# ShenhanQian/GaussianAvatars

Measured on AMD Instinct MI355X. Metric: frames/sec fwd+bwd @100k SH-3 splats 802x550, higher is better.
Workload: dtype f32; 1 GPU; BASELINE configs[2]: 100000 mesh-bound SH-3 splats (synthetic stand-in for media/306), 802x550 (HxW), select_mesh_by_timestep + render + L1-vs-white + backward, no optimiser step; splats=100000, width=550, height=802, sh_degree=3, scene=ellipsoid, splat_order=morton (io.spatial_sort: the loaders' default), num_rendered=2322054, num_binned=1851307, tile_culling=True, binding=fused, parallelism=one process, one GPU, 300 frames in turn; no collective

## Files before the change

### gaussianavatars_amd/_lib.py

```python
from __future__ import annotations

import ctypes as C
import os

_HERE = os.path.dirname(os.path.abspath(__file__))


def raw_stream(dev):
    import torch

    try:
        return torch._C._cuda_getCurrentRawStream(dev.index if dev.index is not None else torch.cuda.current_device())
    except AttributeError:
        return torch.cuda.current_stream(dev).cuda_stream


class _NoCtx:
    def __enter__(self):
        return None

    def __exit__(self, *a):
        return False


# ... 21 lines not shown


class GsrSettings(C.Structure):
    _fields_ = [
        ("image_height", C.c_int32),
        ("image_width", C.c_int32),
        ("tanfovx", C.c_float),
        ("tanfovy", C.c_float),
        ("bg", C.c_void_p),
        ("scale_modifier", C.c_float),
        ("viewmatrix", C.c_void_p),
        ("projmatrix", C.c_void_p),
        ("sh_degree", C.c_int32),
        ("campos", C.c_void_p),
        ("prefiltered", C.c_int32),
        ("debug", C.c_int32),
        ("tile_culling", C.c_int32),
        ("forward_only", C.c_int32),
        ("deterministic", C.c_int32),
        ("exact_scale_grad", C.c_int32),
        ("deferred_count", C.c_int32),
        ("fast_blend", C.c_int32),
    ]


class GsrGeomLayout(C.Structure):
    _fields_ = [(n, C.c_size_t) for n in
                ("depths", "grec", "cov3D", "rect", "tiles_touched", "clamped", "visible", "brec", "acc64", "acc", "total")]


class GsrBinningLayout(C.Structure):
    _fields_ = [(n, C.c_size_t) for n in
                ("keys", "point_list", "qlist", "qpos", "qcount", "qstart", "ranges", "tile_count", "tile_start", "tile_cursor", "tile_order",
                 "block_hist", "dkeys", "dtmp", "order", "bcount", "bstart", "bcursor", "border", "bhist", "qhist", "qprefix", "qmask", "ranks", "rank", "rank_over", "srect", "sspan", "pstat", "tdesc", "obs", "bandcnt", "path", "chunks", "nb", "nbands", "band_rows",
                 "total")]


class GsrBound(C.Structure):
    _fields_ = [("binding", C.c_void_p), ("binding_is_i64", C.c_int32), ("F", C.c_int32), ("face_R", C.c_void_p), ("face_scale", C.c_void_p),
                ("face_center", C.c_void_p), ("face_quat", C.c_void_p), ("slot", C.c_void_p), ("rows", C.c_void_p)]


class GsrImageLayout(C.Structure):
    _fields_ = [(n, C.c_size_t) for n in ("final_T", "n_contrib", "n_contrib_q", "c_final", "ck", "gmax", "units", "total")]


GSR_SYMBOLS = {
    "gsr_abi_version": (C.c_int, []),
    "gsr_last_error": (C.c_char_p, []),
    "gsr_count_slot_read": (C.c_int, [C.c_int32, C.POINTER(C.c_int64), C.POINTER(C.c_int64)]),
    "gsr_count_slot_overflow": (C.c_int, [C.c_int32, C.POINTER(C.c_int64), C.c_int32]),
    "gsr_last_forward_seq": (C.c_int64, []),
    "gsr_count_slot_wait": (C.c_int, [C.c_int32, C.c_int64, C.c_void_p, C.POINTER(C.c_int64)]),
    "gsr_geom_layout": (C.c_int, [C.c_int32, C.POINTER(GsrGeomLayout)]),
    "gsr_binning_layout": (C.c_int, [C.c_int64, C.c_int32, C.c_int32, C.c_int32, C.c_int32, C.POINTER(GsrBinningLayout)]),
    "gsr_image_layout": (C.c_int, [C.c_int32, C.c_int32, C.POINTER(GsrImageLayout)]),
    "gsr_forward": (C.c_int, [C.POINTER(GsrSettings), C.c_int32, C.c_int32] + [C.c_void_p] * 7 +
                    [C.c_void_p, C.c_void_p, C.c_void_p, C.c_void_p, C.c_int64, C.c_void_p,
                     C.POINTER(C.c_int64), C.c_void_p]),
    "gsr_backward": (C.c_int, [C.POINTER(GsrSettings), C.c_int32, C.c_int32] + [C.c_void_p] * 6 +
                     [C.c_void_p, C.c_void_p, C.c_void_p, C.c_int64, C.c_void_p, C.c_int64, C.c_void_p] +
                     [C.c_void_p] * 8 + [C.c_void_p]),
    "gsr_forward_ex": (C.c_int, [C.POINTER(GsrSettings), C.c_int32, C.c_int32] + [C.c_void_p] * 8 +
                       [C.c_void_p, C.c_void_p, C.c_void_p, C.c_void_p, C.c_int64, C.c_void_p,
                        C.POINTER(C.c_int64), C.c_void_p]),
    "gsr_backward_ex": (C.c_int, [C.POINTER(GsrSettings), C.c_int32, C.c_int32] + [C.c_void_p] * 7 +
                        [C.c_void_p, C.c_void_p, C.c_void_p, C.c_int64, C.c_void_p, C.c_int64, C.c_void_p] +
                        [C.c_void_p] * 9 + [C.c_void_p]),
    "gsr_forward_bound": (C.c_int, [C.POINTER(GsrSettings), C.c_int32, C.c_int32, C.POINTER(GsrBound)] + [C.c_void_p] * 6 +
                          [C.c_void_p, C.c_void_p, C.c_void_p, C.c_void_p, C.c_int64, C.c_void_p, C.POINTER(C.c_int64), C.c_void_p]),
    "gsr_backward_bound": (C.c_int, [C.POINTER(GsrSettings), C.c_int32, C.c_int32, C.POINTER(GsrBound)] + [C.c_void_p] * 6 +
                           [C.c_void_p, C.c_void_p, C.c_void_p, C.c_int64, C.c_void_p, C.c_int64, C.c_void_p] +
                           [C.c_void_p] * 8 + [C.c_void_p]),
    "gsr_mark_visible": (C.c_int, [C.c_int32, C.c_void_p, C.c_void_p, C.c_void_p, C.c_void_p, C.c_void_p]),
    "gsr_profile_enable": (C.c_int, [C.c_int]),
    "gsr_profile_read": (C.c_int, [C.POINTER(C.c_double), C.POINTER(C.c_int64)]),
    "gsr_kernel_name": (C.c_char_p, [C.c_int]),
    "gsr_wait_stats": (C.c_int, [C.POINTER(C.c_double), C.POINTER(C.c_int64)]),
}
GSR_NUM_KERNELS = 12


def gsr_profile_enable(on: bool) -> None:
    gsr().gsr_profile_enable(1 if on else 0)


def gsr_profile_read() -> dict:
    ms = (C.c_double * GSR_NUM_KERNELS)()
    n = (C.c_int64 * GSR_NUM_KERNELS)()
    rc = gsr().gsr_profile_read(ms, n)
    if rc != GSR_OK:
        raise RuntimeError(f"gsr_profile_read failed: {gsr().gsr_last_error().decode()}")
    return {gsr().gsr_kernel_name(i).decode(): (ms[i], n[i]) for i in range(GSR_NUM_KERNELS)}

def gsr_wait_stats():
    ms, n = C.c_double(), C.c_int64()
    gsr().gsr_wait_stats(C.byref(ms), C.byref(n))
    return ms.value, n.value


_gsr = None


def _torch_first():
    import torch


def gsr():
    global _gsr
    if _gsr is None:
        if not os.path.exists(GSR_LIB_PATH):
            raise RuntimeError(
                f"{GSR_LIB_PATH} is missing: build it with `python -c 'import __graft_entry__ as g; g.build()'` "
                "(hipcc --offload-arch=gfx950).  There is no CPU fallback."
            )
        _torch_first()
        lib = C.CDLL(GSR_LIB_PATH)
        for name, (res, args) in GSR_SYMBOLS.items():
            fn = getattr(lib, name)
            fn.restype = res
            fn.argtypes = args
        if lib.gsr_abi_version() != GSR_ABI_VERSION:
            raise RuntimeError(f"gsr ABI version {lib.gsr_abi_version()} != {GSR_ABI_VERSION}")
        _gsr = lib
    return _gsr


GAB_LIB_PATH = os.environ.get("GAB_LIB") or os.path.join(_HERE, "libgab_hip.so")
GAB_FLAME_WS_FLOATS = 512
GAB_BIND_ROW_FLOATS = 20
_P = C.c_void_p


class GabRig(C.Structure):
    _fields_ = [("V", C.c_int32), ("n_shape", C.c_int32), ("n_expr", C.c_int32), ("v_template", _P), ("shapedirs", _P),
                ("posedirs", _P), ("J_regressor", _P), ("lbs_weights", _P), ("parents", C.c_int32 * 5)]


GAB_SYMBOLS = {
    "gab_abi_version": (C.c_int, []),
    "gab_last_error": (C.c_char_p, []),
    "gab_flame_forward": (C.c_int, [C.POINTER(GabRig)] + [_P] * 8 + [_P, _P, _P, _P]),
    "gab_flame_backward": (C.c_int, [C.POINTER(GabRig)] + [_P] * 8 + [_P, _P, _P, _P] + [_P] * 8 + [_P] +
                           [C.c_int32, C.POINTER(C.c_void_p), C.POINTER(C.c_int32), _P]),
    "gab_flame_prepared_floats": (C.c_int64, [C.POINTER(GabRig)]),
    "gab_flame_prepare": (C.c_int, [C.POINTER(GabRig), _P, _P, _P, _P]),
    "gab_flame_forward_prepared": (C.c_int, [C.POINTER(GabRig), _P] + [_P] * 6 + [_P, _P, _P, _P]),
    "gab_blend_sequence": (C.c_int, [C.POINTER(GabRig), _P, _P, C.c_int32, _P, _P]),
    "gab_flame_forward_sequence": (C.c_int, [C.POINTER(GabRig), _P, _P] + [_P] * 6 + [_P, _P, _P, _P]),
    "gab_flame_backward_prepared": (C.c_int, [C.POINTER(GabRig), _P] + [_P] * 4 + [_P, _P, _P] + [_P] * 6 + [_P] +
                                    [C.c_int32, C.POINTER(C.c_void_p), C.POINTER(C.c_int32), _P]),
    "gab_mesh_backward_prepared": (C.c_int, [C.POINTER(GabRig), _P] + [_P] * 4 + [_P, _P, _P, _P, _P] + [_P] * 5 + [_P] * 6 + [_P] +
                                   [C.c_int32, C.POINTER(C.c_void_p), C.POINTER(C.c_int32), _P]),
    "gab_face_frames_forward": (C.c_int, [C.c_int32, C.c_int32, _P, _P, C.c_int32, _P, _P, _P, _P, _P, _P]),
    "gab_face_frames_backward": (C.c_int, [C.c_int32, C.c_int32, _P, _P, C.c_int32, _P, _P, _P, _P, _P, C.c_int32, _P]),
    "gab_bind_forward": (C.c_int, [C.c_int32, C.c_int32, _P, _P, _P, _P, C.c_int32, _P, _P, _P, _P, _P, _P, _P, _P, _P, _P]),
    "gab_bind_backward": (C.c_int, [C.c_int32, C.c_int32, _P, _P, _P, _P, C.c_int32, _P, _P, _P, _P, _P, _P, _P, _P, _P, _P, _P, _P, _P, _P, _P]),
    "gab_bind_backward_csr": (C.c_int, [C.c_int32, C.c_int32] + [_P] * 22),
    "gab_bind_backward_faces": (C.c_int, [C.c_int32, _P, _P, _P, _P]),
    "gab_zero_buffers": (C.c_int, [C.c_int32, C.POINTER(C.c_void_p), C.POINTER(C.c_int32), _P]),
    "gab_feed_row": (C.c_int, [_P, C.c_int32, C.c_int32, _P, C.c_int32, _P, _P, _P]),
    "gab_profile_enable": (C.c_int, [C.c_int]),
    "gab_profile_collect": (C.c_int, []),
    "gab_profile_entry": (C.c_int, [C.c_int32, C.POINTER(C.c_char_p), C.POINTER(C.c_double), C.POINTER(C.c_int64)]),
    "gab_profile_reset": (C.c_int, []),
}
GAB_ABI_VERSION = 5

_gab = None


def gab():
    global _gab
    if _gab is None:
        if not os.path.exists(GAB_LIB_PATH):
            raise RuntimeError(f"{GAB_LIB_PATH} is missing: run __graft_entry__.build() (hipcc, gfx950).  There is no CPU fallback.")
        _torch_first()
        lib = C.CDLL(GAB_LIB_PATH)
        for name, (res, args) in GAB_SYMBOLS.items():
            fn = getattr(lib, name)
            fn.restype = res
            fn.argtypes = args
        if lib.gab_abi_version() != GAB_ABI_VERSION:
            raise RuntimeError(f"gab ABI version {lib.gab_abi_version()} != {GAB_ABI_VERSION}")
        _gab = lib
    return _gab


GLS_LIB_PATH = os.path.join(_HERE, "libgls_hip.so")
GLS_SYMBOLS = {
    "gls_abi_version": (C.c_int, []),
    "gls_last_error": (C.c_char_p, []),
    "gls_partial_floats": (C.c_int64, [C.c_int32] * 4),
    "gls_l1_ssim_forward": (C.c_int, [C.c_int32] * 4 + [_P, _P, C.c_float] + [_P] * 4),
    "gls_l1_ssim_backward": (C.c_int, [C.c_int32] * 4 + [_P] * 4 + [C.c_float, _P, _P]),
    "gls_l1_ssim_backward_split": (C.c_int, [C.c_int32] * 4 + [_P] * 5 + [C.c_int32, C.c_float, _P, _P]),
    "gls_l1_forward": (C.c_int, [C.c_int64, _P, _P, C.c_float, _P, _P, _P]),
    "gls_l1_forward_grad": (C.c_int, [C.c_int64, _P, _P, C.c_float, _P, _P, _P, _P]),
    "gls_l1_backward": (C.c_int, [C.c_int64, _P, _P, _P, C.c_float, _P, _P]),
    "gls_densification_stats": (C.c_int, [C.c_int32] + [_P] * 6),
    "gls_add_densification_stats": (C.c_int, [C.c_int32, _P, _P, C.c_int32, _P, _P, _P]),
    "gls_profile_enable": (C.c_int, [C.c_int]),
    "gls_profile_collect": (C.c_int, []),
    "gls_profile_entry": (C.c_int, [C.c_int32, C.POINTER(C.c_char_p), C.POINTER(C.c_double), C.POINTER(C.c_int64)]),
    "gls_profile_reset": (C.c_int, []),
}
GLS_ABI_VERSION = 4

_gls = None


def gls():
    global _gls
    if _gls is None:
        if not os.path.exists(GLS_LIB_PATH):
            raise RuntimeError(f"{GLS_LIB_PATH} is missing: run __graft_entry__.build() (hipcc, gfx950).  There is no CPU fallback.")
        _torch_first()
        lib = C.CDLL(GLS_LIB_PATH)
        for name, (res, args) in GLS_SYMBOLS.items():
            fn = getattr(lib, name)
            fn.restype = res
            fn.argtypes = args
        if lib.gls_abi_version() != GLS_ABI_VERSION:
            raise RuntimeError(f"gls ABI version {lib.gls_abi_version()} != {GLS_ABI_VERSION}")
        _gls = lib
    return _gls


def launch_profile_enable(on: bool) -> None:
    for lib, tag in ((gab(), "gab"), (gls(), "gls")):
        getattr(lib, tag + "_profile_enable")(1 if on else 0)
        if on:
            getattr(lib, tag + "_profile_reset")()


def launch_profile_read() -> dict:
    out = {}
    for lib, tag in ((gab(), "gab"), (gls(), "gls")):
        n = getattr(lib, tag + "_profile_collect")()
        for i in range(n):
            name, ms, k = C.c_char_p(), C.c_double(), C.c_int64()
            if getattr(lib, tag + "_profile_entry")(i, C.byref(name), C.byref(ms), C.byref(k)) == 0:
                out[name.value.decode()] = (ms.value, k.value)
    return out


def gls_error() -> str:
    return gls().gls_last_error().decode("utf-8", "replace")


def gab_error() -> str:
    return gab().gab_last_error().decode("utf-8", "replace")


def gsr_error() -> str:
    return gsr().gsr_last_error().decode("utf-8", "replace")


GMR_LIB_PATH = os.path.join(_HERE, "libgmr_hip.so")
GMR_SYMBOLS = {
    "gmr_abi_version": (C.c_int, []),
    "gmr_last_error": (C.c_char_p, []),
    "gmr_workspace_bytes": (C.c_int64, [C.c_int32, C.c_int32]),
    "gmr_rasterize": (C.c_int, [C.c_int32] * 5 + [_P, _P, _P, _P, _P]),
    "gmr_antialias": (C.c_int, [C.c_int32] * 6 + [_P] * 7),
}
GMR_ABI_VERSION = 1
GMR_MAX_TRIANGLES = (1 << 24) - 1

_gmr = None


def gmr():
    global _gmr
    if _gmr is None:
        if not os.path.exists(GMR_LIB_PATH):
            raise RuntimeError(f"{GMR_LIB_PATH} is missing: run __graft_entry__.build() (hipcc, gfx950).  There is no CPU fallback.")
        _torch_first()
        lib = C.CDLL(GMR_LIB_PATH)
        for name, (res, args) in GMR_SYMBOLS.items():
            fn = getattr(lib, name)
            fn.restype = res
            fn.argtypes = args
        if lib.gmr_abi_version() != GMR_ABI_VERSION:
            raise RuntimeError(f"gmr ABI version {lib.gmr_abi_version()} != {GMR_ABI_VERSION}")
        _gmr = lib
    return _gmr


def gmr_error() -> str:
    return gmr().gmr_last_error().decode("utf-8", "replace")


GOP_LIB_PATH = os.path.join(_HERE, "libgop_hip.so")
GOP_ABI_VERSION = 1
GOP_MAX_TENSORS = 32
GOP_SLAB = 2048


class GopAdamTensor(C.Structure):
    _fields_ = [("param", _P), ("grad", _P), ("exp_avg", _P), ("exp_avg_sq", _P), ("n", C.c_int64), ("step_size", C.c_float),
                ("bias_correction2_sqrt", C.c_float)]


GOP_SYMBOLS = {
    "gop_abi_version": (C.c_int, []),
    "gop_last_error": (C.c_char_p, []),
    "gop_adam_step": (C.c_int, [C.c_int32, C.POINTER(GopAdamTensor), C.c_float, C.c_float, C.c_float, _P]),
    "gop_adam_step_ex": (C.c_int, [C.c_int32, C.POINTER(GopAdamTensor)] + [C.c_float] * 5 + [_P]),
    "gop_profile_enable": (C.c_int, [C.c_int]),
    "gop_profile_collect": (C.c_int, []),
    "gop_profile_entry": (C.c_int, [C.c_int32, C.POINTER(C.c_char_p), C.POINTER(C.c_double), C.POINTER(C.c_int64)]),
    "gop_profile_reset": (C.c_int, []),
}

_gop = None


def gop():
    global _gop
# ... 33 lines not shown
```

### gaussianavatars_amd/binding.py

```python
from __future__ import annotations

import ctypes as C
import os

import torch

from . import _host, _lib


def _p(t):
    return None if t is None else t.data_ptr()


def _stream(dev):
    return _lib.raw_stream(dev)


def _chk(rc, what):
    if rc != 0:
        raise RuntimeError(f"{what} failed ({rc}): {_lib.gab_error()}")


def _need_cuda(t, name):
    if not t.is_cuda:
# ... 51 lines not shown
        head._gab_rig = (key, s)
        r = head._gab_rig
    return r[1]


def _prepared_rig(head, rig, shape_flat, so_flat):
    key = (id(rig), shape_flat.data_ptr(), shape_flat._version, None if so_flat is None else (so_flat.data_ptr(), so_flat._version))
    c = getattr(head, "_gab_prepared", None)
    if c is None or c[0] != key:
        lib = _lib.gab()
        dev = head.v_template.device
        buf = torch.empty(int(lib.gab_flame_prepared_floats(C.byref(rig))), dtype=torch.float32, device=dev)
        with _lib.on_device(dev):
            _chk(lib.gab_flame_prepare(C.byref(rig), _p(shape_flat), _p(so_flat), _p(buf), _stream(dev)), "gab_flame_prepare")
        head._gab_prepared = c = (key, buf, shape_flat, so_flat)
    return c[1]


def _sequence_mode() -> str:
    return os.environ.get("GAA_MESH_SEQUENCE", "off")


def _sequence_table(head, rig, prepared, expr_tab):
    mode = _sequence_mode()
    if mode == "off" or getattr(head, "flame_sequence", True) is False or rig.n_expr <= 0:
        return None
    T = int(expr_tab.shape[0])
    if T < 2 or T * 3 * rig.V * 4 > (1 << 30):
        return None
    key = (prepared.data_ptr(), id(prepared), expr_tab.data_ptr(), expr_tab._version, T)
    c = getattr(head, "_gab_sequence", None)
    if c is not None and c[0] == key:
        if c[1] is not None:
            return c[1]
    elif mode != "eager":
        head._gab_sequence = (key, None, None, None)
        return None
    lib = _lib.gab()
    dev = expr_tab.device
    seq = torch.empty((T, 3 * rig.V), dtype=torch.float32, device=dev)
    with _lib.on_device(dev):
        _chk(lib.gab_blend_sequence(C.byref(rig), _p(prepared), _p(expr_tab), T, _p(seq), _stream(dev)), "gab_blend_sequence")
    head._gab_sequence = (key, seq, prepared, expr_tab)
    return seq


def _use_prepared(head, shape_needs_grad, so_needs_grad) -> bool:
    return not shape_needs_grad and not so_needs_grad and getattr(head, "flame_impl", "prepared") != "classic"


class _FlameForward(torch.autograd.Function):
    @staticmethod
    def forward(ctx, head, shape, expr, rotation, neck, jaw, eyes, translation, static_offset):
        ctx.set_materialize_grads(False)
        lib = _lib.gab()
        rig = _rig_struct(head)
        dev = head.v_template.device
        V = rig.V
        ins = [_f32(t).reshape(-1) for t in (shape, expr, rotation, neck, jaw, eyes, translation)]
        if ins[0].numel() != rig.n_shape or ins[1].numel() != rig.n_expr or ins[5].numel() != 6:
            raise RuntimeError("fused FLAME forward is batch-1: shape (1,n_shape), expr (1,n_expr), eyes (1,6)")
        so = None if static_offset is None else _f32(static_offset).reshape(-1)
        if so is not None and so.numel() != 3 * V:
            raise RuntimeError("static_offset must be (1,V,3)")
        verts = torch.empty((1, V, 3), dtype=torch.float32, device=dev)
        v_shaped = torch.empty((1, V, 3), dtype=torch.float32, device=dev)
        ws = torch.empty(_lib.GAB_FLAME_WS_FLOATS, dtype=torch.float32, device=dev)
        need = ctx.needs_input_grad
        ctx.prepared = _prepared_rig(head, rig, ins[0], so) if _use_prepared(head, need[1], static_offset is not None and need[8]) else None
        with _lib.on_device(dev):
            if ctx.prepared is not None:
                _chk(lib.gab_flame_forward_prepared(C.byref(rig), _p(ctx.prepared), *[_p(t) for t in ins[1:]], _p(verts), _p(v_shaped),
                                                    _p(ws), _stream(dev)), "gab_flame_forward_prepared")
            else:
                _chk(lib.gab_flame_forward(C.byref(rig), *[_p(t) for t in ins], _p(so), _p(verts), _p(v_shaped), _p(ws), _stream(dev)),
                     "gab_flame_forward")
        ctx.head = head
        ctx.has_so = static_offset is not None
        ctx.shapes = [t.shape for t in (shape, expr, rotation, neck, jaw, eyes, translation)]
        ctx.so_shape = None if static_offset is None else static_offset.shape
        ctx.save_for_backward(*ins, *( [so] if so is not None else []), v_shaped, ws)
        return verts, v_shaped

    @staticmethod
    def backward(ctx, g_verts, g_vshaped):
        lib = _lib.gab()
        head = ctx.head
        rig = _rig_struct(head)
        saved = ctx.saved_tensors
        ins = list(saved[:7])
        so = saved[7] if ctx.has_so else None
        v_shaped, ws = saved[-2], saved[-1]
        dev = v_shaped.device
        V = rig.V
        need = ctx.needs_input_grad
        f32 = dict(dtype=torch.float32, device=dev)
        d_shape = torch.empty(rig.n_shape, **f32) if need[1] else None
        d_expr = torch.empty(rig.n_expr, **f32)
        d_rot, d_neck, d_jaw = torch.empty(3, **f32), torch.empty(3, **f32), torch.empty(3, **f32)
        d_eyes, d_trans = torch.empty(6, **f32), torch.empty(3, **f32)
        d_so = torch.empty(3 * V, **f32) if (ctx.has_so and need[8]) else None
        scratch = torch.empty(3 * V, **f32)
        gv = torch.zeros((V, 3), **f32) if g_verts is None else _f32(g_verts)
        gvs = None if g_vshaped is None else _f32(g_vshaped)
        with _lib.on_device(dev):
            if ctx.prepared is not None and gvs is None and d_shape is None and d_so is None:
                _chk(lib.gab_flame_backward_prepared(C.byref(rig), _p(ctx.prepared), *[_p(t) for t in ins[2:6]], _p(v_shaped), _p(ws), _p(gv),
                                                     _p(d_expr), _p(d_rot), _p(d_neck), _p(d_jaw), _p(d_eyes), _p(d_trans), _p(scratch),
                                                     0, None, None, _stream(dev)), "gab_flame_backward_prepared")
            else:
                _chk(lib.gab_flame_backward(C.byref(rig), *[_p(t) for t in ins], _p(so), _p(v_shaped), _p(ws), _p(gv), _p(gvs),
                                            _p(d_shape), _p(d_expr), _p(d_rot), _p(d_neck), _p(d_jaw), _p(d_eyes), _p(d_trans), _p(d_so),
                                            _p(scratch), 0, None, None, _stream(dev)), "gab_flame_backward")
        sh = ctx.shapes
        outs = [None, None if d_shape is None else d_shape.view(sh[0]), d_expr.view(sh[1]), d_rot.view(sh[2]), d_neck.view(sh[3]),
                d_jaw.view(sh[4]), d_eyes.view(sh[5]), d_trans.view(sh[6]), None if d_so is None else d_so.view(ctx.so_shape)]
        return tuple(outs)


def flame_forward(head, shape, expr, rotation, neck, jaw, eyes, translation, static_offset=None):
    return _FlameForward.apply(head, shape, expr, rotation, neck, jaw, eyes, translation, static_offset)


class _FlameForwardTimestep(torch.autograd.Function):

    _ROWS = ("expr", "rotation", "neck_pose", "jaw_pose", "eyes_pose", "translation")

    @staticmethod
    def forward(ctx, head, t, shape, expr, rotation, neck, jaw, eyes, translation, static_offset):
        ctx.set_materialize_grads(False)
        lib = _lib.gab()
        rig = _rig_struct(head)
        dev = head.v_template.device
        V = rig.V
        tabs = [_f32(x) for x in (expr, rotation, neck, jaw, eyes, translation)]
        T = tabs[0].shape[0]
        widths = [int(x.shape[1]) for x in tabs]
        if widths != [rig.n_expr, 3, 3, 3, 6, 3] or any(x.shape[0] != T for x in tabs) or not (0 <= t < T):
            raise RuntimeError("flame_forward_timestep: expected (T,n_expr),(T,3),(T,3),(T,3),(T,6),(T,3) tables and 0 <= t < T")
        sh = _f32(shape).reshape(-1)
        so = None if static_offset is None else _f32(static_offset).reshape(-1)
        rows = [x.data_ptr() + 4 * t * w for x, w in zip(tabs, widths)]
        verts = torch.empty((1, V, 3), dtype=torch.float32, device=dev)
        v_shaped = torch.empty((1, V, 3), dtype=torch.float32, device=dev)
        ws = torch.empty(_lib.GAB_FLAME_WS_FLOATS, dtype=torch.float32, device=dev)
        need = ctx.needs_input_grad
        ctx.prepared = _prepared_rig(head, rig, sh, so) if _use_prepared(head, need[2], so is not None and need[9]) else None
        seq = _sequence_table(head, rig, ctx.prepared, tabs[0]) if (ctx.prepared is not None and not any(need[2:])) else None
        with _lib.on_device(dev):
            if seq is not None:
                _chk(lib.gab_flame_forward_sequence(C.byref(rig), _p(ctx.prepared), seq.data_ptr() + 4 * t * 3 * V, *rows, _p(verts), _p(v_shaped),
                                                    _p(ws), _stream(dev)), "gab_flame_forward_sequence")
            elif ctx.prepared is not None:
                _chk(lib.gab_flame_forward_prepared(C.byref(rig), _p(ctx.prepared), *rows, _p(verts), _p(v_shaped), _p(ws), _stream(dev)),
                     "gab_flame_forward_prepared")
            else:
                _chk(lib.gab_flame_forward(C.byref(rig), _p(sh), *rows, _p(so), _p(verts), _p(v_shaped), _p(ws), _stream(dev)),
                     "gab_flame_forward")
        ctx.head, ctx.t, ctx.T, ctx.widths = head, t, T, widths
        ctx.has_so = so is not None
        ctx.shape_shape = shape.shape
        ctx.so_shape = None if static_offset is None else static_offset.shape
        ctx.keep = _Keep(sh, *tabs, *([so] if so is not None else []), v_shaped, ws)
        return verts, v_shaped

    @staticmethod
    def backward(ctx, g_verts, g_vshaped):
        lib = _lib.gab()
        rig = _rig_struct(ctx.head)
        saved = ctx.keep.get()
        sh, tabs = saved[0], list(saved[1:7])
        so = saved[7] if ctx.has_so else None
        v_shaped, ws = saved[-2], saved[-1]
        dev = v_shaped.device
        V, T, t, widths = rig.V, ctx.T, ctx.t, ctx.widths
        need = ctx.needs_input_grad
        f32 = dict(dtype=torch.float32, device=dev)
        tables = [torch.empty((T, w), **f32) for w in widths]
        ptrs = (C.c_void_p * len(tables))(*[x.data_ptr() for x in tables])
        sizes = (C.c_int32 * len(tables))(*[T * w for w in widths])
        outp = [x.data_ptr() + 4 * t * w for x, w in zip(tables, widths)]
        d_shape = torch.empty(rig.n_shape, **f32) if need[2] else None
        d_so = torch.empty(3 * V, **f32) if (ctx.has_so and need[9]) else None
        scratch = torch.empty(3 * V, **f32)
        gv = torch.zeros((V, 3), **f32) if g_verts is None else _f32(g_verts)
        gvs = None if g_vshaped is None else _f32(g_vshaped)
        rows = [x.data_ptr() + 4 * t * w for x, w in zip(tabs, widths)]
        with _lib.on_device(dev):
            if ctx.prepared is not None and gvs is None and d_shape is None and d_so is None:
                _chk(lib.gab_flame_backward_prepared(C.byref(rig), _p(ctx.prepared), *rows[1:5], _p(v_shaped), _p(ws), _p(gv), *outp,
                                                     _p(scratch), len(tables), ptrs, sizes, _stream(dev)), "gab_flame_backward_prepared")
            else:
                _chk(lib.gab_flame_backward(C.byref(rig), _p(sh), *rows, _p(so), _p(v_shaped), _p(ws), _p(gv), _p(gvs), _p(d_shape),
                                            *outp, _p(d_so), _p(scratch), len(tables), ptrs, sizes, _stream(dev)), "gab_flame_backward")
        grads = [tb if need[3 + i] else None for i, tb in enumerate(tables)]
        return (None, None, None if d_shape is None else d_shape.view(ctx.shape_shape), *grads,
                None if d_so is None else d_so.view(ctx.so_shape))


def flame_forward_timestep(head, flame_param: dict, t: int):
    fp = flame_param
    return _FlameForwardTimestep.apply(head, int(t), fp["shape"], fp["expr"], fp["rotation"], fp["neck_pose"], fp["jaw_pose"],
                                       fp["eyes_pose"], fp["translation"], fp.get("static_offset"))


class _FaceFrames(torch.autograd.Function):
    @staticmethod
    def forward(ctx, verts, faces):
        ctx.set_materialize_grads(False)
        lib = _lib.gab()
        _need_cuda(verts, "verts")
        dev = verts.device
        v = _f32(verts)
        fi, is64 = _idx(faces)
        V, F = v.shape[0], fi.shape[0]
        f32 = dict(dtype=torch.float32, device=dev)
        center, R = torch.empty((F, 3), **f32), torch.empty((F, 3, 3), **f32)
        scale, quat = torch.empty((F, 1), **f32), torch.empty((F, 4), **f32)
        ctx.d_verts = torch.empty((V, 3), **f32) if ctx.needs_input_grad[0] else None
        with _lib.on_device(dev):
            _chk(lib.gab_face_frames_forward(V, F, _p(v), _p(fi), is64, _p(center), _p(R), _p(scale), _p(quat), _p(ctx.d_verts),
                                             _stream(dev)), "gab_face_frames_forward")
        ctx.keep = _Keep(v, fi)
        ctx.is64 = is64
        return center, R, scale, quat

    @staticmethod
    def backward(ctx, g_center, g_R, g_scale, g_quat):
        lib = _lib.gab()
        v, fi = ctx.keep.get()
        dev = v.device
        V, F = v.shape[0], fi.shape[0]
        d_verts, ctx.d_verts = ctx.d_verts, None
        prepared = d_verts is not None
        if not prepared:
            d_verts = torch.empty((V, 3), dtype=torch.float32, device=dev)
        gs = [None if g is None else _f32(g) for g in (g_center, g_R, g_scale, g_quat)]
        with _lib.on_device(dev):
            _chk(lib.gab_face_frames_backward(V, F, _p(v), _p(fi), ctx.is64, _p(gs[0]), _p(gs[1]), _p(gs[2]), _p(gs[3]), _p(d_verts),
                                              1 if prepared else 0, _stream(dev)), "gab_face_frames_backward")
        return d_verts, None


def face_frames(verts, faces):
    return _FaceFrames.apply(verts, faces)


class _SubCtx:

    def __init__(self, needs_input_grad):
        self.needs_input_grad = needs_input_grad

    def set_materialize_grads(self, flag):
        pass


def vertex_corner_csr(faces: torch.Tensor, num_verts: int):
    hit = getattr(faces, "_gaa_vertex_corners", None)
    if hit is not None and hit[0] == faces._version and hit[1] == num_verts:
        return hit[2]
    f = faces.detach().long()
    flat = f.reshape(-1)
    order = torch.sort(flat, stable=True).indices
    fo, co = order // 3, order % 3
    vf_list = torch.cat([(4 * fo + co)[:, None], f[fo]], 1).to(torch.int32).contiguous()
    vf_begin = torch.zeros(num_verts + 1, dtype=torch.int32, device=flat.device)
    vf_begin[1:] = torch.cumsum(torch.bincount(flat, minlength=num_verts), 0).to(torch.int32)
    faces._gaa_vertex_corners = (faces._version, num_verts, (vf_begin, vf_list))
    return vf_begin, vf_list


def _mesh_backward_mode() -> str:
    return os.environ.get("GAA_MESH_BWD", "merged")


class _MeshFramesTimestep(torch.autograd.Function):
    @staticmethod
    def forward(ctx, head, t, faces, shape, expr, rotation, neck, jaw, eyes, translation, static_offset):
        ctx.set_materialize_grads(False)
        need = ctx.needs_input_grad
        c1 = _SubCtx((False, False) + tuple(need[3:]))
        verts, v_shaped = _FlameForwardTimestep.forward(c1, head, t, shape, expr, rotation, neck, jaw, eyes, translation, static_offset)
        ctx.merged = c1.prepared is not None and _mesh_backward_mode() == "merged"
        if ctx.merged and faces.device != verts.device:
            raise RuntimeError(f"select_mesh_by_timestep: faces live on {faces.device}, the vertices on {verts.device}")
        if ctx.merged and any(need):
            ctx.corners = vertex_corner_csr(faces, int(verts.shape[1]))
        c2 = _SubCtx((any(need) and not ctx.merged, False))
        center, R, scale, quat = _FaceFrames.forward(c2, verts[0], faces)
        ctx.c1, ctx.c2 = c1, c2
        ctx.faces = faces
        return verts, v_shaped, center, R, scale, quat

    @staticmethod
    def _backward_merged(ctx, g_verts, g_center, g_R, g_scale, g_quat):
        c1, c2 = ctx.c1, ctx.c2
        lib = _lib.gab()
        rig = _rig_struct(c1.head)
        saved = c1.keep.get()
        tabs = list(saved[1:7])
        v_shaped, ws = saved[-2], saved[-1]
        v, _ = c2.keep.get()
        dev = v.device
        V, T, t, widths = rig.V, c1.T, c1.t, c1.widths
        need = c1.needs_input_grad
        f32 = dict(dtype=torch.float32, device=dev)
        tables = [torch.empty((T, w), **f32) for w in widths]
        ptrs = (C.c_void_p * len(tables))(*[x.data_ptr() for x in tables])
        sizes = (C.c_int32 * len(tables))(*[T * w for w in widths])
        outp = [x.data_ptr() + 4 * t * w for x, w in zip(tables, widths)]
        rows = [x.data_ptr() + 4 * t * w for x, w in zip(tabs, widths)]
        vf_begin, vf_list = ctx.corners
        scratch = torch.empty(3 * V, **f32)
        gs = [None if g is None else _f32(g) for g in (g_center, g_R, g_scale, g_quat)]
        gv = None if g_verts is None else _f32(g_verts)
        with _lib.on_device(dev):
            _chk(lib.gab_mesh_backward_prepared(C.byref(rig), _p(c1.prepared), *rows[1:5], _p(v_shaped), _p(ws), _p(v),
                                                _p(vf_begin), _p(vf_list), _p(gs[0]), _p(gs[1]), _p(gs[2]), _p(gs[3]), _p(gv), *outp,
                                                _p(scratch), len(tables), ptrs, sizes, _stream(dev)), "gab_mesh_backward_prepared")
        grads = [tb if need[3 + i] else None for i, tb in enumerate(tables)]
        return (None, None, None, None, *grads, None)

    @staticmethod
    def backward(ctx, g_verts, g_vshaped, g_center, g_R, g_scale, g_quat):
        if ctx.merged and g_vshaped is None:
            return _MeshFramesTimestep._backward_merged(ctx, g_verts, g_center, g_R, g_scale, g_quat)
        d_verts, _ = _FaceFrames.backward(ctx.c2, g_center, g_R, g_scale, g_quat)
        if g_verts is not None:
            d_verts = d_verts + g_verts.reshape(d_verts.shape)
        grads = _FlameForwardTimestep.backward(ctx.c1, d_verts.view(1, -1, 3), g_vshaped)
        return (None, None, None) + tuple(grads[2:])


_RIG_BUFFERS = ("v_template", "shapedirs", "posedirs", "J_regressor", "lbs_weights")


def _plain(t) -> bool:
    return t.is_cuda and t.dtype is torch.float32 and t.is_contiguous()


def _mesh_plan(H, head, fp: dict, faces):
    shape, so = fp["shape"], fp.get("static_offset")
    bufs = head.__dict__.get("_buffers")
    if bufs is None or any(n not in bufs for n in _RIG_BUFFERS):
        bufs = {n: getattr(head, n) for n in _RIG_BUFFERS}
    env = (os.environ.get("GAA_MESH_BWD"), os.environ.get("GAA_MESH_SEQUENCE"))
    st = head.__dict__.get("_gaa_mesh_plan")
    if st is not None:
        (plan, k_shape, v_shape, k_so, v_so, k_faces, v_faces, k_bufs, k_env, k_flags) = st
        if (k_shape is shape and v_shape == shape._version and k_so is so and (so is None or v_so == so._version) and k_faces is faces and v_faces == faces._version
                and k_env == env and k_flags == (shape.requires_grad, so is not None and so.requires_grad, getattr(head, "flame_impl", "prepared"))
                and all(bufs[n] is b for n, b in zip(_RIG_BUFFERS, k_bufs))):
            return plan
    plan = None
    flags = (shape.requires_grad, so is not None and so.requires_grad, getattr(head, "flame_impl", "prepared"))
    ok = (not flags[0] and not flags[1] and flags[2] != "classic" and _mesh_backward_mode() == "merged" and _sequence_mode() == "off"
          and all(_plain(bufs[n]) for n in _RIG_BUFFERS) and faces.is_cuda and faces.is_contiguous() and faces.dtype in (torch.int32, torch.int64)
          and faces.device == bufs["v_template"].device)
    if ok:
        rig = _rig_struct(head)
        sh = _f32(shape).reshape(-1)
        sof = None if so is None else _f32(so).reshape(-1)
        if sh.numel() == rig.n_shape and (sof is None or sof.numel() == 3 * rig.V):
            prepared = _prepared_rig(head, rig, sh, sof)
            vf_begin, vf_list = vertex_corner_csr(faces, int(rig.V))
            plan = H.make_mesh_plan(*[bufs[n] for n in _RIG_BUFFERS], [int(x) for x in head.parents.tolist()], int(head.n_shape_params), prepared, faces, vf_begin, vf_list)
    head.__dict__["_gaa_mesh_plan"] = (plan, shape, shape._version, so, None if so is None else so._version, faces, faces._version, tuple(bufs[n] for n in _RIG_BUFFERS), env, flags)
    return plan


def mesh_frames_timestep(head, flame_param: dict, t: int, faces):
    fp = flame_param
    H = _host.get()
    if H is not None:
        expr, rot, neck, jaw, eyes, trans = fp["expr"], fp["rotation"], fp["neck_pose"], fp["jaw_pose"], fp["eyes_pose"], fp["translation"]
        if _plain(expr) and _plain(rot) and _plain(neck) and _plain(jaw) and _plain(eyes) and _plain(trans):
            plan = _mesh_plan(H, head, fp, faces)
            if plan is not None:
                return H.mesh_frames(plan, expr, rot, neck, jaw, eyes, trans, int(t))
    return _MeshFramesTimestep.apply(head, int(t), faces, fp["shape"], fp["expr"], fp["rotation"], fp["neck_pose"], fp["jaw_pose"],
                                     fp["eyes_pose"], fp["translation"], fp.get("static_offset"))


def binding_csr(binding: torch.Tensor, num_faces: int):
    b = binding.detach().long()
    order64 = torch.sort(b, stable=True).indices
    order = order64.to(torch.int32).contiguous()
    counts = torch.bincount(b, minlength=num_faces)
    face_begin = torch.zeros(num_faces + 1, dtype=torch.int32, device=b.device)
    face_begin[1:] = torch.cumsum(counts, 0).to(torch.int32)
    slot = torch.empty_like(order)
    slot[order64] = torch.arange(order.numel(), dtype=torch.int32, device=b.device)
    return order, face_begin, b.to(torch.int32).contiguous(), slot


class _BindSplats(torch.autograd.Function):
    @staticmethod
    def forward(ctx, xyz, log_scaling, rotation, binding, face_R, face_scale, face_center, face_quat, csr=None, opacity_logit=None):
        lib = _lib.gab()
        _need_cuda(xyz, "_xyz")
        dev = xyz.device
        x, ls, q = _f32(xyz), _f32(log_scaling), _f32(rotation)
        b, is64 = _idx(binding)
        fR, fs, fc, fq = _f32(face_R), _f32(face_scale), _f32(face_center), _f32(face_quat)
        N, F = x.shape[0], fc.shape[0]
        f32 = dict(dtype=torch.float32, device=dev)
        ox, osc, oq = torch.empty((N, 3), **f32), torch.empty((N, 3), **f32), torch.empty((N, 4), **f32)
        ol = None if opacity_logit is None else _f32(opacity_logit)
        oo = None if ol is None else torch.empty_like(ol)
        with _lib.on_device(dev):
            _chk(lib.gab_bind_forward(N, F, _p(x), _p(ls), _p(q), _p(b), is64, _p(fc), _p(fR), _p(fs), _p(fq), _p(ox), _p(osc), _p(oq),
                                      _p(ol), _p(oo), _stream(dev)), "gab_bind_forward")
        ctx.keep = _Keep(x, ls, q, b, fR, fs, fc, fq, oo)
        ctx.is64 = is64
        if csr is not None and (csr[0].numel() != N or csr[1].numel() != F + 1 or any(t.numel() != N for t in csr[2:4])):
            raise RuntimeError(f"binding CSR does not match this call: {csr[0].numel()} ordered splats / {csr[1].numel() - 1} faces, "
                               f"expected {N} / {F} (rebuild it with binding_csr after the binding changed)")
        ctx.csr = csr
        if oo is None:
            return ox, osc, oq
        return ox, osc, oq, oo

    @staticmethod
    def backward(ctx, g_xyz, g_scaling, g_rot, g_opacity=None):
        lib = _lib.gab()
        x, ls, q, b, fR, fs, fc, fq, oo = ctx.keep.get()
        dev = x.device
        N, F = x.shape[0], fc.shape[0]
        f32 = dict(dtype=torch.float32, device=dev)
        d_x, d_ls, d_q = torch.empty((N, 3), **f32), torch.empty((N, 3), **f32), torch.empty((N, 4), **f32)
        d_face = torch.empty(17 * F, **f32)
        gs = [None if g is None else _f32(g) for g in (g_xyz, g_scaling, g_rot)]
        go = None if (oo is None or g_opacity is None) else _f32(g_opacity)
        d_ol = None if oo is None else torch.empty_like(oo)
        with _lib.on_device(dev):
            if ctx.csr is not None:
                order, face_begin = ctx.csr[0], ctx.csr[1]
                splat_face, slot = (ctx.csr[2], ctx.csr[3]) if len(ctx.csr) >= 4 else (None, None)
                rows = torch.empty(_lib.GAB_BIND_ROW_FLOATS * N, **f32) if slot is not None else None
                _chk(lib.gab_bind_backward_csr(N, F, _p(x), _p(ls), _p(q), _p(fR), _p(fs), _p(fq), _p(gs[0]), _p(gs[1]), _p(gs[2]),
                                               _p(order), _p(face_begin), _p(d_x), _p(d_ls), _p(d_q), _p(d_face), _p(oo), _p(go), _p(d_ol),
                                               _p(splat_face), _p(slot), _p(rows), _stream(dev)), "gab_bind_backward_csr")
            else:
                _chk(lib.gab_bind_backward(N, F, _p(x), _p(ls), _p(q), _p(b), ctx.is64, _p(fc), _p(fR), _p(fs), _p(fq), _p(gs[0]),
                                           _p(gs[1]), _p(gs[2]), _p(d_x), _p(d_ls), _p(d_q), _p(d_face), _p(oo), _p(go), _p(d_ol),
                                           _stream(dev)), "gab_bind_backward")
        return (d_x, d_ls, d_q, None, d_face[3 * F: 12 * F].view(F, 3, 3), d_face[12 * F: 13 * F].view(F, 1), d_face[: 3 * F].view(F, 3),
                d_face[13 * F:].view(F, 4), None, d_ol)


def bind_splats(xyz, log_scaling, rotation, binding, face_R, face_scale, face_center, face_quat, csr=None, opacity_logit=None):
    return _BindSplats.apply(xyz, log_scaling, rotation, binding, face_R, face_scale, face_center, face_quat, csr, opacity_logit)
```

### gaussianavatars_amd/csrc/build_host.py

```python
#!/usr/bin/env python3
import os
import subprocess
import sys
import sysconfig

HERE = os.path.dirname(os.path.abspath(__file__))
OUT = os.path.join(os.path.dirname(HERE), "gaa_host.so")
SRC = os.path.join(HERE, "gaa_host.cpp")
STAMP = OUT + ".stamp"
DEPS = [SRC, __file__] + [os.path.join(HERE, "..", "..", "include", h) for h in ("gsr.h", "gab.h", "gls.h")]


def build_stamp() -> str:
    import torch

    return "torch=%s cxx11abi=%d python=%s soabi=%s" % (torch.__version__, int(torch._C._GLIBCXX_USE_CXX11_ABI), sys.version.split()[0],
                                                       sysconfig.get_config_var("SOABI"))


def stamp_matches() -> bool:
    try:
        return open(STAMP).read().strip() == build_stamp()
    except OSError:
        return False


def up_to_date() -> bool:
    return os.path.exists(OUT) and all(os.path.getmtime(OUT) >= os.path.getmtime(d) for d in DEPS) and stamp_matches()


def main() -> int:
    if up_to_date() and "--force" not in sys.argv:
        return 0
    import torch
    from torch.utils import cpp_extension as ce

    tl = ce.library_paths()[0]
    rocm = os.environ.get("ROCM_PATH", "/opt/rocm")
    cmd = ["g++", "-O2", "-std=c++17", "-fPIC", "-shared", "-Wall", "-Wno-unused-function", "-Wno-sign-compare",
           "-D__HIP_PLATFORM_AMD__=1", "-DUSE_ROCM=1", "-DTORCH_EXTENSION_NAME=gaa_host", "-DTORCH_API_INCLUDE_EXTENSION_H",
           f"-D_GLIBCXX_USE_CXX11_ABI={int(torch._C._GLIBCXX_USE_CXX11_ABI)}"]
    cmd += [f"-I{p}" for p in ce.include_paths()] + [f"-I{rocm}/include", f"-I{sysconfig.get_paths()['include']}"]
    cmd += [SRC, "-o", OUT, f"-L{tl}", "-lc10", "-lc10_hip", "-ltorch_cpu", "-ltorch_hip", "-ltorch", "-ltorch_python", "-ldl", f"-Wl,-rpath,{tl}"]
    print("building gaa_host.so (g++, torch %s) ..." % torch.__version__, flush=True)
    r = subprocess.run(cmd)
    if r.returncode == 0:
        with open(STAMP, "w") as fh:
            fh.write(build_stamp() + "\n")
    return r.returncode


if __name__ == "__main__":
    sys.exit(main())
```

### gaussianavatars_amd/csrc/gaa_host.cpp

```cpp
#include <torch/extension.h>

#include <ATen/hip/impl/HIPGuardImplMasqueradingAsCUDA.h>
#include <c10/hip/HIPStream.h>
#include <dlfcn.h>
#include <torch/csrc/autograd/function.h>
#include <torch/csrc/autograd/functions/utils.h>

#include <atomic>
#include <map>
#include <mutex>
#include <tuple>

#include "../../include/gab.h"
#include "../../include/gls.h"
#include "../../include/gsr.h"

namespace {

using at::Tensor;
using torch::autograd::Node;
using torch::autograd::variable_list;

#define GAA_API(X)                                                                                                                      \
    X(gsr_abi_version) X(gsr_last_error) X(gsr_geom_layout) X(gsr_binning_layout) X(gsr_image_layout) X(gsr_forward_bound)             \
    X(gsr_backward_bound) X(gsr_last_forward_seq) X(gsr_count_slot_wait) X(gsr_count_slot_overflow)                                     \
    X(gab_abi_version) X(gab_last_error) X(gab_flame_forward_prepared) X(gab_face_frames_forward) X(gab_mesh_backward_prepared)         \
    X(gab_bind_backward_faces)                                                                                                           \
    X(gls_abi_version) X(gls_last_error) X(gls_partial_floats) X(gls_l1_forward) X(gls_l1_forward_grad) X(gls_l1_backward)               \
    X(gls_l1_ssim_forward) X(gls_l1_ssim_backward_split)

struct Api {
#define GAA_DECL(name) decltype(&::name) name = nullptr;
    GAA_API(GAA_DECL)
#undef GAA_DECL
    bool ready = false;
} api;

void* open_loaded(const std::string& path)
{
    void* h = dlopen(path.c_str(), RTLD_NOW | RTLD_NOLOAD);
    if (!h) h = dlopen(path.c_str(), RTLD_NOW);
    TORCH_CHECK(h, "gaa_host: cannot open ", path, ": ", dlerror());
    return h;
}

void init(const std::string& gsr_path, const std::string& gab_path, const std::string& gls_path)
{
    void* hs[3] = {open_loaded(gsr_path), open_loaded(gab_path), open_loaded(gls_path)};
#define GAA_LOAD(name)                                                                                       \
    {                                                                                                        \
        void* s = nullptr;                                                                                   \
        for (void* h : hs)                                                                                   \
            if (!s) s = dlsym(h, #name);                                                                     \
        TORCH_CHECK(s, "gaa_host: the libraries do not export ", #name);                                     \
        api.name = reinterpret_cast<decltype(api.name)>(s);                                                  \
    }
    GAA_API(GAA_LOAD)
#undef GAA_LOAD
    TORCH_CHECK(api.gsr_abi_version() == GSR_ABI_VERSION, "gaa_host was built for gsr ABI ", GSR_ABI_VERSION, ", the library is ", api.gsr_abi_version());
    TORCH_CHECK(api.gab_abi_version() == GAB_ABI_VERSION, "gaa_host was built for gab ABI ", GAB_ABI_VERSION, ", the library is ", api.gab_abi_version());
    TORCH_CHECK(api.gls_abi_version() == GLS_ABI_VERSION, "gaa_host was built for gls ABI ", GLS_ABI_VERSION, ", the library is ", api.gls_abi_version());
    api.ready = true;
}

inline void need_api() { TORCH_CHECK(api.ready, "gaa_host.init() has not been called"); }

inline void* cur_stream(const Tensor& t) { return (void*)c10::hip::getCurrentHIPStream(t.device().index()).stream(); }
using DeviceGuard = c10::hip::HIPGuardMasqueradingAsCUDA;

inline const float* fptr(const Tensor& t) { return t.defined() && t.numel() ? t.data_ptr<float>() : nullptr; }
inline float* fptr_mut(Tensor& t) { return t.defined() && t.numel() ? t.data_ptr<float>() : nullptr; }

inline void check_f32(const Tensor& t, const char* name)
{
    TORCH_CHECK(t.defined() && t.is_cuda(), name, " must be a device tensor; the MI355X path has no CPU implementation");
    TORCH_CHECK(t.scalar_type() == at::kFloat && t.is_contiguous(), name, " must be contiguous float32 (the native host does not copy: take the Python entry)");
}

inline Tensor empty_f32(at::IntArrayRef sizes, const Tensor& like) { return at::empty(sizes, like.options().dtype(at::kFloat)); }

inline Tensor grad_f32(const Tensor& g)
{
    if (!g.defined()) return g;
    if (g.scalar_type() == at::kFloat && g.is_contiguous()) return g;
    return g.to(at::kFloat).contiguous();
}

struct Kept {
    Tensor t;
    uint32_t version = 0;
    Kept() = default;
    explicit Kept(const Tensor& x, bool alias = false) : t(x.defined() ? (alias ? x.detach() : x) : x), version(x.defined() ? x._version() : 0) {}
    const Tensor& get(const char* what) const
    {
        TORCH_CHECK(!t.defined() || t._version() == version, "one of the variables needed for gradient computation has been modified by an inplace operation (",
                    what, " saved by the native host is at version ", t.defined() ? t._version() : 0, ", expected ", version, ")");
        return t;
    }
};

inline bool any_requires_grad(std::initializer_list<std::reference_wrapper<const Tensor>> ts)
{
    if (!at::GradMode::is_enabled()) return false;
    for (const Tensor& t : ts)
        if (t.defined() && t.requires_grad()) return true;
    return false;
}

struct MeshPlan {
    GabRig rig{};
    Tensor keep[5];
    Tensor prepared;
    Tensor faces;
    int faces_i64 = 0;
    Tensor vf_begin, vf_list;
    int64_t F = 0;
};

struct MeshNode : public Node {
    std::shared_ptr<MeshPlan> plan;
    Kept tabs[6];
    Kept verts, v_shaped;
    Tensor ws;
    int64_t t = 0, T = 0;
    int64_t widths[6] = {0, 3, 3, 3, 6, 3};

    variable_list apply(variable_list&& grads) override
    {
        std::lock_guard<std::mutex> lock(mutex_);
        need_api();
        TORCH_CHECK(grads.size() == 6, "MeshNode: expected 6 gradients");
        TORCH_CHECK(!grads[1].defined(), "the native mesh node has no path for a gradient w.r.t. verts_cano (v_shaped): take GAA_NATIVE_HOST=0");
        const MeshPlan& p = *plan;
        static const char* names[6] = {"expr", "rotation", "neck_pose", "jaw_pose", "eyes_pose", "translation"};
        const Tensor& v = verts.get("verts");
        const Tensor& vs = v_shaped.get("verts_cano");
        DeviceGuard guard(v.device().index());
        void* stream = cur_stream(v);
        const int V = p.rig.V;
        Tensor tables[6];
        float* zero_ptrs[6];
        int32_t zero_sizes[6];
        float* outp[6];
        const float* rows[6];
        for (int i = 0; i < 6; ++i) {
            const Tensor& tab = tabs[i].get(names[i]);
            tables[i] = empty_f32({T, widths[i]}, v);
            zero_ptrs[i] = tables[i].data_ptr<float>();
            zero_sizes[i] = (int32_t)(T * widths[i]);
            outp[i] = zero_ptrs[i] + t * widths[i];
            rows[i] = tab.data_ptr<float>() + t * widths[i];
        }
        Tensor scratch = empty_f32({3 * (int64_t)V}, v);
        Tensor gc = grad_f32(grads[2]), gR = grad_f32(grads[3]), gs = grad_f32(grads[4]), gq = grad_f32(grads[5]), gv = grad_f32(grads[0]);
        int rc = api.gab_mesh_backward_prepared(&p.rig, p.prepared.data_ptr<float>(), rows[1], rows[2], rows[3], rows[4], vs.data_ptr<float>(), ws.data_ptr<float>(),
                                                v.data_ptr<float>(), p.vf_begin.data_ptr<int32_t>(), p.vf_list.data_ptr<int32_t>(), fptr(gc), fptr(gR), fptr(gs), fptr(gq),
                                                fptr(gv), outp[0], outp[1], outp[2], outp[3], outp[4], outp[5], scratch.data_ptr<float>(), 6, zero_ptrs, zero_sizes, stream);
        TORCH_CHECK(rc == 0, "gab_mesh_backward_prepared failed (", rc, "): ", api.gab_last_error());
        variable_list out(6);
        for (int i = 0; i < 6; ++i)
            if (task_should_compute_output(i)) out[i] = tables[i];
        return out;
    }
    void release_variables() override {}
};

std::vector<Tensor> mesh_frames(const std::shared_ptr<MeshPlan>& plan, const Tensor& expr, const Tensor& rotation, const Tensor& neck, const Tensor& jaw,
                                const Tensor& eyes, const Tensor& translation, int64_t t)
{
    need_api();
    const MeshPlan& p = *plan;
    const Tensor* tabs[6] = {&expr, &rotation, &neck, &jaw, &eyes, &translation};
    const int64_t widths[6] = {p.rig.n_expr, 3, 3, 3, 6, 3};
    static const char* names[6] = {"expr", "rotation", "neck_pose", "jaw_pose", "eyes_pose", "translation"};
    const int64_t T = expr.dim() == 2 ? expr.size(0) : -1;
    TORCH_CHECK(T > 0 && t >= 0 && t < T, "flame_forward_timestep: expected (T,n_expr),(T,3),(T,3),(T,3),(T,6),(T,3) tables and 0 <= t < T");
    for (int i = 0; i < 6; ++i) {
        check_f32(*tabs[i], names[i]);
        TORCH_CHECK(tabs[i]->dim() == 2 && tabs[i]->size(0) == T && tabs[i]->size(1) == widths[i],
                    "flame_forward_timestep: expected (T,n_expr),(T,3),(T,3),(T,3),(T,6),(T,3) tables and 0 <= t < T");
    }
    const Tensor& like = p.prepared;
    DeviceGuard guard(like.device().index());
    void* stream = cur_stream(like);
    const int64_t V = p.rig.V, F = p.F;
    Tensor verts = empty_f32({1, V, 3}, like), v_shaped = empty_f32({1, V, 3}, like), ws = empty_f32({GAB_FLAME_WS_FLOATS}, like);
    Tensor center = empty_f32({F, 3}, like), R = empty_f32({F, 3, 3}, like), scale = empty_f32({F, 1}, like), quat = empty_f32({F, 4}, like);
    const float* rows[6];
    for (int i = 0; i < 6; ++i) rows[i] = tabs[i]->data_ptr<float>() + t * widths[i];
    int rc = api.gab_flame_forward_prepared(&p.rig, p.prepared.data_ptr<float>(), rows[0], rows[1], rows[2], rows[3], rows[4], rows[5], verts.data_ptr<float>(),
                                            v_shaped.data_ptr<float>(), ws.data_ptr<float>(), stream);
    TORCH_CHECK(rc == 0, "gab_flame_forward_prepared failed (", rc, "): ", api.gab_last_error());
    rc = api.gab_face_frames_forward((int32_t)V, (int32_t)F, verts.data_ptr<float>(), p.faces.data_ptr(), p.faces_i64, center.data_ptr<float>(), R.data_ptr<float>(),
                                     scale.data_ptr<float>(), quat.data_ptr<float>(), nullptr , stream);
    TORCH_CHECK(rc == 0, "gab_face_frames_forward failed (", rc, "): ", api.gab_last_error());
    if (any_requires_grad({expr, rotation, neck, jaw, eyes, translation})) {
        auto node = std::shared_ptr<MeshNode>(new MeshNode(), torch::autograd::deleteNode);
        node->set_next_edges(torch::autograd::collect_next_edges(expr, rotation, neck, jaw, eyes, translation));
        node->plan = plan;
        for (int i = 0; i < 6; ++i) {
            node->tabs[i] = Kept(*tabs[i]);
            node->widths[i] = widths[i];
        }
        node->verts = Kept(verts, true);
        node->v_shaped = Kept(v_shaped, true);
        node->ws = ws;
        node->t = t;
        node->T = T;
        torch::autograd::set_history({verts, v_shaped, center, R, scale, quat}, node);
    }
    return {verts, v_shaped, center, R, scale, quat};
}

struct Layouts {
    GsrGeomLayout geom;
    GsrImageLayout img;
};
std::mutex layout_mutex;
std::map<std::tuple<int64_t, int, int>, Layouts> layout_cache;
std::map<std::tuple<int64_t, int, int, int64_t, int>, GsrBinningLayout> binning_cache;

Layouts layouts(int64_t P, int W, int H)
{
    std::lock_guard<std::mutex> lock(layout_mutex);
    auto key = std::make_tuple(P, W, H);
    auto it = layout_cache.find(key);
    if (it == layout_cache.end()) {
        if (layout_cache.size() > 64) layout_cache.clear();
        Layouts l{};
        TORCH_CHECK(api.gsr_geom_layout((int32_t)P, &l.geom) == 0 && api.gsr_image_layout(W, H, &l.img) == 0, "gsr layout: ", api.gsr_last_error());
        it = layout_cache.emplace(key, l).first;
    }
    return it->second;
}
GsrBinningLayout binning_layout(int64_t cap, int W, int H, int64_t P, int mode)
{
    std::lock_guard<std::mutex> lock(layout_mutex);
    auto key = std::make_tuple(cap, W, H, P, mode);
    auto it = binning_cache.find(key);
    if (it == binning_cache.end()) {
        if (binning_cache.size() > 64) binning_cache.clear();
        GsrBinningLayout b{};
        TORCH_CHECK(api.gsr_binning_layout(cap, W, H, (int32_t)P, mode, &b) == 0, "gsr_binning_layout: ", api.gsr_last_error());
        it = binning_cache.emplace(key, b).first;
    }
    return it->second;
}

struct RasterNode : public Node {
    GsrSettings s{};
    Tensor bg, viewmatrix, projmatrix, campos;
    Kept xyz, dc, rest, opacity, scaling, rotation;
    Kept fR, fs, fc, fq;
    Tensor binding, csr_slot, face_begin;
    int binding_i64 = 0;
    Tensor radii, state;
    size_t off_img = 0, off_binning = 0;
    int64_t P = 0, M = 0, F = 0, capacity = 0, num_rendered = 0;
    bool bound = false;

    variable_list apply(variable_list&& grads) override
    {
        std::lock_guard<std::mutex> lock(mutex_);
        need_api();
        variable_list out(11);
        if (grads.empty() || !grads[0].defined()) return out;
        TORCH_CHECK(state.defined(), "the rasterizer state of this frame has been released (backward through the graph a second time without retain_graph)");
        const Tensor& x = xyz.get("_xyz");
        DeviceGuard guard(x.device().index());
        void* stream = cur_stream(x);
        Tensor g = grad_f32(grads[0]);
        TORCH_CHECK(g.is_cuda() && g.numel() == 3 * (int64_t)s.image_height * s.image_width, "grad_out_color must be a (3,H,W) device tensor");
        Tensor g_xyz = empty_f32({P, 3}, x), g_m2 = empty_f32({P, 3}, x), g_dc = empty_f32({P, 1, 3}, x), g_rest = empty_f32({P, M - 1, 3}, x);
        Tensor g_op = empty_f32({P, 1}, x), g_ls = empty_f32({P, 3}, x), g_rot = empty_f32({P, 4}, x);
        GsrBound b{};
        Tensor scratch, d_face;
        if (!bound) {
            scratch = empty_f32({9 * P}, x);
        } else {
            const int64_t rows_at = (9 * P + 3) / 4 * 4;
            scratch = empty_f32({rows_at + (int64_t)GAB_BIND_ROW_FLOATS * P}, x);
            d_face = empty_f32({17 * F}, x);
            b.binding = binding.data_ptr();
            b.binding_is_i64 = binding_i64;
            b.F = (int32_t)F;
            b.face_R = fR.get("face_orien_mat").data_ptr<float>();
            b.face_scale = fs.get("face_scaling").data_ptr<float>();
            b.face_center = fc.get("face_center").data_ptr<float>();
            b.face_quat = fq.get("face_orien_quat").data_ptr<float>();
            b.slot = csr_slot.data_ptr<int32_t>();
            b.rows = scratch.data_ptr<float>() + rows_at;
        }
        GsrSettings sb = s;
        sb.forward_only = 0;
        sb.deferred_count = 0;
        uint8_t* st = state.data_ptr<uint8_t>();
        int rc = api.gsr_backward_bound(&sb, (int32_t)P, (int32_t)M, &b, x.data_ptr<float>(), dc.get("_features_dc").data_ptr<float>(), rest.get("_features_rest").data_ptr<float>(),
                                        opacity.get("_opacity").data_ptr<float>(), scaling.get("_scaling").data_ptr<float>(), rotation.get("_rotation").data_ptr<float>(),
                                        radii.data_ptr<int32_t>(), st, st + off_binning, capacity, st + off_img, num_rendered, g.data_ptr<float>(), g_xyz.data_ptr<float>(),
                                        g_m2.data_ptr<float>(), g_dc.data_ptr<float>(), g_rest.data_ptr<float>(), g_op.data_ptr<float>(), g_ls.data_ptr<float>(),
                                        g_rot.data_ptr<float>(), scratch.data_ptr<float>(), stream);
        TORCH_CHECK(rc == 0, "gsr_backward_bound failed (", rc, "): ", api.gsr_last_error());
        if (bound) {
            rc = api.gab_bind_backward_faces((int32_t)F, face_begin.data_ptr<int32_t>(), b.rows, d_face.data_ptr<float>(), stream);
            TORCH_CHECK(rc == 0, "gab_bind_backward_faces failed (", rc, "): ", api.gab_last_error());
        }
        out[0] = g_xyz, out[1] = g_m2, out[2] = g_dc, out[3] = g_rest, out[4] = g_op, out[5] = g_ls, out[6] = g_rot;
        if (bound) {
            if (task_should_compute_output(7)) out[7] = d_face.as_strided({F, 3, 3}, {9, 3, 1}, 3 * F);
            if (task_should_compute_output(8)) out[8] = d_face.as_strided({F, 1}, {1, 1}, 12 * F);
            if (task_should_compute_output(9)) out[9] = d_face.as_strided({F, 3}, {3, 1}, 0);
            if (task_should_compute_output(10)) out[10] = d_face.as_strided({F, 4}, {4, 1}, 13 * F);
        }
        for (int i = 0; i < 7; ++i)
            if (!task_should_compute_output(i)) out[i] = Tensor();
        return out;
    }
    void release_variables() override
    {
        std::lock_guard<std::mutex> lock(mutex_);
        state = Tensor();
    }
};

struct RasterResult {
    Tensor color, radii, visible, state;
    int64_t num_rendered = 0, capacity = 0, off_binning = 0;
    int forward_only = 0, path = 0, nbands = 0, fitted = 1;
};

RasterResult rasterize_bound(const Tensor& xyz, const Tensor& means2D, const Tensor& dc, const Tensor& rest, const Tensor& opacity, const Tensor& scaling,
                             const Tensor& rotation, const c10::optional<Tensor>& face_R, const c10::optional<Tensor>& face_scale,
                             const c10::optional<Tensor>& face_center, const c10::optional<Tensor>& face_quat, const c10::optional<Tensor>& binding,
                             const c10::optional<Tensor>& csr_slot, const c10::optional<Tensor>& face_begin, const Tensor& bg, const Tensor& viewmatrix,
                             const Tensor& projmatrix, const Tensor& campos, int64_t H, int64_t W, double tanfovx, double tanfovy, double scale_modifier,
                             int64_t sh_degree, int64_t debug, int64_t tile_culling, int64_t exact_scale_grad, int64_t deterministic, int64_t fast_blend,
                             int64_t capacity, int64_t late_slot)
{
    need_api();
    check_f32(xyz, "_xyz"), check_f32(dc, "_features_dc"), check_f32(rest, "_features_rest"), check_f32(opacity, "_opacity");
    check_f32(scaling, "_scaling"), check_f32(rotation, "_rotation");
    check_f32(bg, "bg"), check_f32(viewmatrix, "viewmatrix"), check_f32(projmatrix, "projmatrix"), check_f32(campos, "campos");
    const int64_t P = xyz.size(0);
    TORCH_CHECK(P > 0 && xyz.dim() == 2 && xyz.size(1) == 3, "_xyz must be (P,3) with P > 0");
    TORCH_CHECK(rest.dim() == 3 && rest.size(0) == P && rest.size(1) >= 1 && dc.numel() == 3 * P, "split SH: _features_dc must be (P,1,3) and _features_rest (P,M-1,3)");
    const int64_t M = 1 + rest.size(1);
    const bool bound = binding.has_value() && binding->defined();
    GsrBound b{};
// ... 114 lines not shown
        need_api();
        variable_list out(2);
        if (grads.empty() || !grads[0].defined()) return out;
        Tensor pre = da;
        da = Tensor();
        if (pre.defined()) {
            if (is_unit_seed(grads[0])) {
                g_l1_misses = 0;
                out[0] = pre;
                return out;
            }
            if (++g_l1_misses >= 2) g_l1_emit = 0;
        }
        const Tensor& x = a.get("network_output");
        const Tensor& y = b.get("gt");
        DeviceGuard guard(x.device().index());
        void* stream = cur_stream(x);
        Tensor g = grad_f32(grads[0]);
        const int64_t n = x.numel();
        if (task_should_compute_output(0)) {
            out[0] = at::empty_like(x);
            int rc = api.gls_l1_backward(n, x.data_ptr<float>(), y.data_ptr<float>(), g.data_ptr<float>(), (float)scale, out[0].data_ptr<float>(), stream);
            TORCH_CHECK(rc == 0, "gls_l1_backward failed (", rc, "): ", api.gls_last_error());
        }
        if (task_should_compute_output(1)) {
            out[1] = at::empty_like(y);
            int rc = api.gls_l1_backward(n, y.data_ptr<float>(), x.data_ptr<float>(), g.data_ptr<float>(), (float)scale, out[1].data_ptr<float>(), stream);
            TORCH_CHECK(rc == 0, "gls_l1_backward failed (", rc, "): ", api.gls_last_error());
        }
        return out;
    }
    void release_variables() override
    {
        std::lock_guard<std::mutex> lock(mutex_);
        da = Tensor();
    }
};

Tensor l1_loss(const Tensor& a, const Tensor& b, int64_t emit, bool seeded)
{
    need_api();
    check_f32(a, "network_output"), check_f32(b, "gt");
    TORCH_CHECK(a.numel() == b.numel(), "l1_loss: the two images differ in size");
    DeviceGuard guard(a.device().index());
    void* stream = cur_stream(a);
    const int64_t n = a.numel();
    const double scale = 1.0 / (double)std::max<int64_t>(n, 1);
    Tensor out = empty_f32({}, a), partial = empty_f32({api.gls_partial_floats(1, 1, 1, 1)}, a);
    const bool ga = at::GradMode::is_enabled() && a.requires_grad(), gb = at::GradMode::is_enabled() && b.requires_grad();
    Tensor da;
    const bool want = emit < 0 ? g_l1_emit.load() != 0 : emit != 0;
    if (ga && !gb && seeded && want) {
        da = at::empty_like(a);
        int rc = api.gls_l1_forward_grad(n, a.data_ptr<float>(), b.data_ptr<float>(), (float)scale, out.data_ptr<float>(), partial.data_ptr<float>(), da.data_ptr<float>(), stream);
        TORCH_CHECK(rc == 0, "gls_l1_forward_grad failed (", rc, "): ", api.gls_last_error());
    } else {
        int rc = api.gls_l1_forward(n, a.data_ptr<float>(), b.data_ptr<float>(), (float)scale, out.data_ptr<float>(), partial.data_ptr<float>(), stream);
        TORCH_CHECK(rc == 0, "gls_l1_forward failed (", rc, "): ", api.gls_last_error());
    }
    if (ga || gb) {
        auto node = std::shared_ptr<L1Node>(new L1Node(), torch::autograd::deleteNode);
        node->set_next_edges(torch::autograd::collect_next_edges(a, b));
        node->a = Kept(a), node->b = Kept(b), node->da = da, node->scale = scale;
        torch::autograd::set_history(out, node);
    }
    return out;
}

struct L1SsimNode : public Node {
    Kept img1, img2;
    Tensor maps;
    int C = 0, H = 0, W = 0;
    double scale = 0;
    variable_list apply(variable_list&& grads) override
    {
        std::lock_guard<std::mutex> lock(mutex_);
        need_api();
        variable_list out(2);
        if (grads.size() != 2 || (!grads[0].defined() && !grads[1].defined())) return out;
        TORCH_CHECK(maps.defined(), "the SSIM derivative planes of this frame have been released (backward through the graph a second time without retain_graph)");
        const Tensor& x = img1.get("img1");
        const Tensor& y = img2.get("img2");
        DeviceGuard guard(x.device().index());
        void* stream = cur_stream(x);
        Tensor g1 = grad_f32(grads[0]), g2 = grad_f32(grads[1]);
        out[0] = at::empty_like(x);
        int rc = api.gls_l1_ssim_backward_split(1, C, H, W, x.data_ptr<float>(), y.data_ptr<float>(), maps.data_ptr<float>(), fptr(g1), fptr(g2), 0, (float)scale,
                                                out[0].data_ptr<float>(), stream);
        TORCH_CHECK(rc == 0, "gls_l1_ssim_backward_split failed (", rc, "): ", api.gls_last_error());
        return out;
    }
    void release_variables() override
    {
        std::lock_guard<std::mutex> lock(mutex_);
        maps = Tensor();
    }
};

std::vector<Tensor> l1_ssim(const Tensor& img1, const Tensor& img2)
{
    need_api();
    check_f32(img1, "image"), check_f32(img2, "gt");
    TORCH_CHECK(img1.dim() == 3 && img1.sizes() == img2.sizes(), "the native l1_ssim takes one (C,H,W) pair");
    TORCH_CHECK(!(at::GradMode::is_enabled() && img2.requires_grad()), "the native l1_ssim has no gradient for the second image");
    const int C = (int)img1.size(0), H = (int)img1.size(1), W = (int)img1.size(2);
    DeviceGuard guard(img1.device().index());
    void* stream = cur_stream(img1);
    const bool need = at::GradMode::is_enabled() && img1.requires_grad();
    const double scale = 1.0 / ((double)C * H * W);
    Tensor sums = empty_f32({2}, img1), partial = empty_f32({api.gls_partial_floats(1, C, H, W)}, img1);
    Tensor maps = need ? empty_f32({3, 1, C, H, W}, img1) : Tensor();
    int rc = api.gls_l1_ssim_forward(1, C, H, W, img1.data_ptr<float>(), img2.data_ptr<float>(), (float)scale, sums.data_ptr<float>(), fptr_mut(maps), partial.data_ptr<float>(), stream);
    TORCH_CHECK(rc == 0, "gls_l1_ssim_forward failed (", rc, "): ", api.gls_last_error());
    Tensor l1 = at::empty({0}, sums.options()).set_(sums.storage(), 0, {}, {});
    Tensor ss = at::empty({0}, sums.options()).set_(sums.storage(), 1, {}, {});
    if (need) {
        auto node = std::shared_ptr<L1SsimNode>(new L1SsimNode(), torch::autograd::deleteNode);
        node->set_next_edges(torch::autograd::collect_next_edges(img1, img2));
        node->img1 = Kept(img1), node->img2 = Kept(img2), node->maps = maps;
        node->C = C, node->H = H, node->W = W, node->scale = scale;
        torch::autograd::set_history({l1, ss}, node);
    }
    return {l1, ss};
}

std::shared_ptr<MeshPlan> make_mesh_plan(const Tensor& v_template, const Tensor& shapedirs, const Tensor& posedirs, const Tensor& J_regressor, const Tensor& lbs_weights,
                                         std::vector<int64_t> parents, int64_t n_shape, const Tensor& prepared, const Tensor& faces, const Tensor& vf_begin,
                                         const Tensor& vf_list)
{
    auto p = std::make_shared<MeshPlan>();
    const Tensor* rig[5] = {&v_template, &shapedirs, &posedirs, &J_regressor, &lbs_weights};
    static const char* names[5] = {"v_template", "shapedirs", "posedirs", "J_regressor", "lbs_weights"};
    for (int i = 0; i < 5; ++i) {
        check_f32(*rig[i], names[i]);
        p->keep[i] = *rig[i];
    }
    check_f32(prepared, "prepared rig");
    TORCH_CHECK(parents.size() == GAB_NUM_JOINTS, "the fused FLAME kernels are built for the 5-joint FLAME skeleton");
    p->rig.V = (int32_t)v_template.size(0);
    p->rig.n_shape = (int32_t)n_shape;
    p->rig.n_expr = (int32_t)(shapedirs.size(2) - n_shape);
    p->rig.v_template = v_template.data_ptr<float>(), p->rig.shapedirs = shapedirs.data_ptr<float>(), p->rig.posedirs = posedirs.data_ptr<float>();
    p->rig.J_regressor = J_regressor.data_ptr<float>(), p->rig.lbs_weights = lbs_weights.data_ptr<float>();
    for (int j = 0; j < GAB_NUM_JOINTS; ++j) p->rig.parents[j] = (int32_t)parents[j];
    p->prepared = prepared;
    TORCH_CHECK(faces.is_cuda() && faces.is_contiguous() && faces.dim() == 2 && faces.size(1) == 3 && (faces.scalar_type() == at::kInt || faces.scalar_type() == at::kLong),
                "faces must be a contiguous (F,3) int32 / int64 device tensor");
    TORCH_CHECK(faces.device() == prepared.device(), "select_mesh_by_timestep: faces live on ", faces.device(), ", the vertices on ", prepared.device());
    p->faces = faces, p->faces_i64 = faces.scalar_type() == at::kLong, p->F = faces.size(0);
    TORCH_CHECK(vf_begin.scalar_type() == at::kInt && vf_list.scalar_type() == at::kInt && vf_begin.is_contiguous() && vf_list.is_contiguous() && vf_begin.numel() == p->rig.V + 1 &&
                    vf_list.numel() == 12 * p->F,
                "vertex -> corner table does not match this topology");
    p->vf_begin = vf_begin, p->vf_list = vf_list;
    return p;
}

}

PYBIND11_MODULE(TORCH_EXTENSION_NAME, m)
{
    m.doc() = "compiled host side of gaussianavatars_amd's autograd nodes (include/gsr.h, gab.h, gls.h underneath)";
    m.def("init", &init, "resolve the C ABI from the three loaded libraries");
    py::class_<MeshPlan, std::shared_ptr<MeshPlan>>(m, "MeshPlan");
    m.def("make_mesh_plan", &make_mesh_plan);
    m.def("mesh_frames", &mesh_frames, py::call_guard<py::gil_scoped_release>());
    py::class_<RasterResult>(m, "RasterResult")
        .def_readonly("color", &RasterResult::color)
        .def_readonly("radii", &RasterResult::radii)
        .def_readonly("visible", &RasterResult::visible)
        .def_readonly("state", &RasterResult::state)
        .def_readonly("num_rendered", &RasterResult::num_rendered)
        .def_readonly("capacity", &RasterResult::capacity)
        .def_readonly("off_binning", &RasterResult::off_binning)
        .def_readonly("forward_only", &RasterResult::forward_only)
        .def_readonly("path", &RasterResult::path)
        .def_readonly("nbands", &RasterResult::nbands)
        .def_readonly("fitted", &RasterResult::fitted);
    m.def("rasterize_bound", &rasterize_bound, py::call_guard<py::gil_scoped_release>());
    m.def("set_unit_seed", &set_unit_seed);
    m.def("l1_emit_state", &l1_emit_state);
    m.def("l1_loss", &l1_loss, py::call_guard<py::gil_scoped_release>());
    m.def("l1_ssim", &l1_ssim, py::call_guard<py::gil_scoped_release>());
    m.attr("GSR_ABI") = GSR_ABI_VERSION;
    m.attr("GAB_ABI") = GAB_ABI_VERSION;
    m.attr("GLS_ABI") = GLS_ABI_VERSION;
}
```

### gaussianavatars_amd/csrc/gab_kernels.hip

```cpp
#include <hip/hip_runtime.h>
#include <hip/amd_detail/amd_hip_unsafe_atomics.h>

#include <cstdarg>
#include <cstdio>

#include "../../include/gab.h"
#include "launch_prof.h"
#include "bind_math.h"

namespace gab {

struct Rig {
    int V, n_shape, n_expr;
    const float* __restrict__ v_template;
    const float* __restrict__ shapedirs;
    const float* __restrict__ posedirs;
    const float* __restrict__ J_regressor;
    const float* __restrict__ lbs_weights;
    int parents[GAB_NUM_JOINTS];
};

constexpr int WS_J = 0;
constexpr int WS_R = 16;
constexpr int WS_PF = 64;
constexpr int WS_A = 128;
constexpr int WS_DA = 256;
constexpr int WS_DT = 320;
constexpr int WS_DPF = 324;
constexpr int WS_DJ = 384;

template <int CTRL, int ROW_MASK>
__device__ __forceinline__ float dpp_f(float v)
{
    return __int_as_float(__builtin_amdgcn_update_dpp(0, __float_as_int(v), CTRL, ROW_MASK, 0xf, false));
}
__device__ __forceinline__ float wave_sum_hi(float v)
{
    v += dpp_f<0xB1, 0xf>(v);
    v += dpp_f<0x4E, 0xf>(v);
    v += dpp_f<0x141, 0xf>(v);
    v += dpp_f<0x140, 0xf>(v);
    v += dpp_f<0x142, 0xa>(v);
    v += dpp_f<0x143, 0xc>(v);
    return v;
}

__device__ __forceinline__ float beta_at(const float* shape, const float* expr, int n_shape, int l)
{
    return l < n_shape ? shape[l] : expr[l - n_shape];
}

__global__ __launch_bounds__(256) void k_blend(Rig rig, const float* __restrict__ shape, const float* __restrict__ expr,
                                                const float* __restrict__ static_offset, float* __restrict__ v_shaped)
{
    const int lane = threadIdx.x & 63;
    const int e = blockIdx.x * 4 + (threadIdx.x >> 6);
    const int E = 3 * rig.V;
    if (e >= E) return;
    const int NB = rig.n_shape + rig.n_expr;
    const float* row = rig.shapedirs + (size_t)e * NB;
    float acc = 0.f;
    if ((NB & 3) == 0 && (rig.n_shape & 3) == 0) {
        const float4* row4 = reinterpret_cast<const float4*>(row);
        for (int c = lane; c < NB / 4; c += 64) {
            const float4 r = row4[c];
            const int l = 4 * c;
            const float4 b = l < rig.n_shape ? reinterpret_cast<const float4*>(shape)[c]
                                             : reinterpret_cast<const float4*>(expr)[c - rig.n_shape / 4];
            acc += r.x * b.x + r.y * b.y + r.z * b.z + r.w * b.w;
        }
    } else {
        for (int l = lane; l < NB; l += 64) acc += row[l] * beta_at(shape, expr, rig.n_shape, l);
    }
    acc = wave_sum_hi(acc);
    if (lane == 63) v_shaped[e] = rig.v_template[e] + acc + (static_offset ? static_offset[e] : 0.f);
}

__device__ __forceinline__ void rodrigues(const float* r, float* R )
{
    const float ux = r[0] + 1e-8f, uy = r[1] + 1e-8f, uz = r[2] + 1e-8f;
    const float th = sqrtf(ux * ux + uy * uy + uz * uz);
    const float dx = r[0] / th, dy = r[1] / th, dz = r[2] / th;
    const float s = sinf(th), c = cosf(th);
    const float K[9] = {0.f, -dz, dy, dz, 0.f, -dx, -dy, dx, 0.f};
    float KK[9];
#pragma unroll
    for (int i = 0; i < 3; ++i)
#pragma unroll
        for (int j = 0; j < 3; ++j) KK[3 * i + j] = K[3 * i] * K[j] + K[3 * i + 1] * K[3 + j] + K[3 * i + 2] * K[6 + j];
#pragma unroll
    for (int i = 0; i < 9; ++i) R[i] = ((i % 4) == 0 ? 1.f : 0.f) + s * K[i] + (1.f - c) * KK[i];
}

__device__ __forceinline__ void rodrigues_bwd(const float* r, const float* dR , float* dr )
{
    const float u[3] = {r[0] + 1e-8f, r[1] + 1e-8f, r[2] + 1e-8f};
    const float th = sqrtf(u[0] * u[0] + u[1] * u[1] + u[2] * u[2]);
    const float d[3] = {r[0] / th, r[1] / th, r[2] / th};
    const float s = sinf(th), c = cosf(th);
    const float K[9] = {0.f, -d[2], d[1], d[2], 0.f, -d[0], -d[1], d[0], 0.f};
    float KK[9];
#pragma unroll
    for (int i = 0; i < 3; ++i)
#pragma unroll
        for (int j = 0; j < 3; ++j) KK[3 * i + j] = K[3 * i] * K[j] + K[3 * i + 1] * K[3 + j] + K[3 * i + 2] * K[6 + j];
    float g_s = 0.f, g_c = 0.f;
#pragma unroll
    for (int i = 0; i < 9; ++i) { g_s += dR[i] * K[i]; g_c -= dR[i] * KK[i]; }
    float dK[9];
#pragma unroll
    for (int i = 0; i < 3; ++i)
#pragma unroll
        for (int j = 0; j < 3; ++j) {
            float a = 0.f, b = 0.f;
#pragma unroll
            for (int k = 0; k < 3; ++k) {
                a += dR[3 * i + k] * K[3 * j + k];
                b += K[3 * k + i] * dR[3 * k + j];
            }
            dK[3 * i + j] = s * dR[3 * i + j] + (1.f - c) * (a + b);
        }
    const float gd[3] = {dK[7] - dK[5], dK[2] - dK[6], dK[3] - dK[1]};
    float g_th = g_s * c - g_c * s;
    g_th -= (gd[0] * r[0] + gd[1] * r[1] + gd[2] * r[2]) / (th * th);
#pragma unroll
    for (int k = 0; k < 3; ++k) dr[k] = gd[k] / th + g_th * u[k] / th;
}

__device__ constexpr int kFlameParents[GAB_NUM_JOINTS] = {-1, 0, 1, 1, 1};
template <bool FLAME_TREE>
__device__ __forceinline__ int parent_of(const int* parents, int i) { return FLAME_TREE ? kFlameParents[i] : parents[i]; }

template <bool FLAME_TREE>
__device__ __forceinline__ void chain_forward(const int* parents, const float* R , const float* J , float* Rg ,
                                              float* tg )
{
#pragma unroll
    for (int i = 0; i < GAB_NUM_JOINTS; ++i) {
        if (i == 0) {
#pragma unroll
            for (int k = 0; k < 9; ++k) Rg[k] = R[k];
#pragma unroll
            for (int k = 0; k < 3; ++k) tg[k] = J[k];
            continue;
        }
        const int p = parent_of<FLAME_TREE>(parents, i);
        const float rel[3] = {J[3 * i] - J[3 * p], J[3 * i + 1] - J[3 * p + 1], J[3 * i + 2] - J[3 * p + 2]};
#pragma unroll
        for (int r = 0; r < 3; ++r) {
#pragma unroll
            for (int c = 0; c < 3; ++c)
                Rg[9 * i + 3 * r + c] = Rg[9 * p + 3 * r] * R[9 * i + c] + Rg[9 * p + 3 * r + 1] * R[9 * i + 3 + c] +
                                        Rg[9 * p + 3 * r + 2] * R[9 * i + 6 + c];
            tg[3 * i + r] = Rg[9 * p + 3 * r] * rel[0] + Rg[9 * p + 3 * r + 1] * rel[1] + Rg[9 * p + 3 * r + 2] * rel[2] + tg[3 * p + r];
        }
    }
}

template <bool FLAME_TREE>
__global__ __launch_bounds__(1024) void k_joints_chain(Rig rig, const float* __restrict__ v_shaped, const float* __restrict__ rotation,
                                                        const float* __restrict__ neck, const float* __restrict__ jaw,
                                                        const float* __restrict__ eyes, float* __restrict__ ws)
{
    __shared__ float red[16][16];
    __shared__ float out[WS_DA];
    const int tid = threadIdx.x, lane = tid & 63, wid = tid >> 6;
    if (tid < GAB_FLAME_WS_FLOATS - WS_DA) ws[WS_DA + tid] = 0.f;
    if (tid < WS_DA) out[tid] = 0.f;
    float acc[15];
#pragma unroll
    for (int k = 0; k < 15; ++k) acc[k] = 0.f;
    for (int v = tid; v < rig.V; v += 1024) {
        const float x = v_shaped[3 * v], y = v_shaped[3 * v + 1], z = v_shaped[3 * v + 2];
#pragma unroll
        for (int j = 0; j < GAB_NUM_JOINTS; ++j) {
            const float w = rig.J_regressor[(size_t)j * rig.V + v];
            acc[3 * j] += w * x;
            acc[3 * j + 1] += w * y;
            acc[3 * j + 2] += w * z;
        }
    }
#pragma unroll
    for (int k = 0; k < 15; ++k) {
        const float s = wave_sum_hi(acc[k]);
        if (lane == 63) red[wid][k] = s;
    }
    __syncthreads();
    if (tid < 15) {
        float sum = 0.f;
#pragma unroll
        for (int w = 0; w < 16; ++w) sum += red[w][tid];
        out[WS_J + tid] = sum;
    } else if (tid >= 64 && tid < 64 + GAB_NUM_JOINTS) {
        const int j = tid - 64;
        const float* pj = j == 0 ? rotation : j == 1 ? neck : j == 2 ? jaw : eyes + 3 * (j - 3);
        const float pose[3] = {pj[0], pj[1], pj[2]};
        float R[9];
        rodrigues(pose, R);
#pragma unroll
        for (int k = 0; k < 9; ++k) {
            out[WS_R + 9 * j + k] = R[k];
            if (j >= 1) out[WS_PF + 9 * (j - 1) + k] = R[k] - ((k % 4) == 0 ? 1.f : 0.f);
        }
    }
    __syncthreads();
    if (tid == 0) {
        float J[15], R[45], Rg[45], tg[15];
#pragma unroll
        for (int k = 0; k < 15; ++k) J[k] = out[WS_J + k];
#pragma unroll
        for (int k = 0; k < 45; ++k) R[k] = out[WS_R + k];
        chain_forward<FLAME_TREE>(rig.parents, R, J, Rg, tg);
#pragma unroll
        for (int j = 0; j < GAB_NUM_JOINTS; ++j)
#pragma unroll
            for (int r = 0; r < 3; ++r) {
#pragma unroll
                for (int c = 0; c < 3; ++c) out[WS_A + 12 * j + 4 * r + c] = Rg[9 * j + 3 * r + c];
                out[WS_A + 12 * j + 4 * r + 3] = tg[3 * j + r] - (Rg[9 * j + 3 * r] * J[3 * j] + Rg[9 * j + 3 * r + 1] * J[3 * j + 1] +
                                                                  Rg[9 * j + 3 * r + 2] * J[3 * j + 2]);
            }
    }
    __syncthreads();
    if (tid < WS_DA) ws[tid] = out[tid];
}

template <bool DEEP>
__device__ __forceinline__ void vertex_posed_and_T(const Rig& rig, const float* __restrict__ ws, const float* __restrict__ v_shaped,
                                                   int v, float* vp , float* T )
{
    const int E = 3 * rig.V;
    float po[3] = {0.f, 0.f, 0.f};
    if (DEEP) {
#pragma unroll
        for (int p = 0; p < GAB_POSE_FEATURES; ++p) {
            const float f = ws[WS_PF + p];
            const float* row = rig.posedirs + (size_t)p * E + 3 * v;
            po[0] += f * row[0];
            po[1] += f * row[1];
            po[2] += f * row[2];
        }
    } else {
        for (int p = 0; p < GAB_POSE_FEATURES; ++p) {
            const float f = ws[WS_PF + p];
            const float* row = rig.posedirs + (size_t)p * E + 3 * v;
            po[0] += f * row[0];
            po[1] += f * row[1];
            po[2] += f * row[2];
        }
    }
#pragma unroll
    for (int k = 0; k < 3; ++k) vp[k] = po[k] + v_shaped[3 * v + k];
#pragma unroll
    for (int k = 0; k < 12; ++k) T[k] = 0.f;
#pragma unroll
    for (int j = 0; j < GAB_NUM_JOINTS; ++j) {
        const float w = rig.lbs_weights[(size_t)v * GAB_NUM_JOINTS + j];
#pragma unroll
        for (int k = 0; k < 12; ++k) T[k] += w * ws[WS_A + 12 * j + k];
    }
}

__global__ __launch_bounds__(256) void k_skin(Rig rig, const float* __restrict__ ws, const float* __restrict__ v_shaped,
                                               const float* __restrict__ translation, float* __restrict__ verts)
{
    const int v = blockIdx.x * blockDim.x + threadIdx.x;
    if (v >= rig.V) return;
    float vp[3], T[12];
    vertex_posed_and_T<false>(rig, ws, v_shaped, v, vp, T);
    for (int r = 0; r < 3; ++r)
        verts[3 * v + r] = T[4 * r] * vp[0] + T[4 * r + 1] * vp[1] + T[4 * r + 2] * vp[2] + T[4 * r + 3] + translation[r];
}

__host__ __device__ inline int prep_joint_offset(int V) { return (3 * V + 3) & ~3; }

__global__ __launch_bounds__(256) void k_prep_rows(Rig rig, const float* __restrict__ shape, const float* __restrict__ static_offset,
                                                    float* __restrict__ prepared)
{
    const int lane = threadIdx.x & 63;
    const int e = blockIdx.x * 4 + (threadIdx.x >> 6);
    if (e >= 3 * rig.V) return;
    const float* row = rig.shapedirs + (size_t)e * (rig.n_shape + rig.n_expr);
    float acc = 0.f;
    for (int l = lane; l < rig.n_shape; l += 64) acc += row[l] * shape[l];
    acc = wave_sum_hi(acc);
    if (lane == 63) prepared[e] = rig.v_template[e] + acc + (static_offset ? static_offset[e] : 0.f);
}
__global__ __launch_bounds__(256) void k_prep_joints(Rig rig, float* __restrict__ prepared)
{
    const int lane = threadIdx.x & 63;
    const int o = blockIdx.x * 4 + (threadIdx.x >> 6);
    if (o >= 15 + 15 * rig.n_expr) return;
    const int NB = rig.n_shape + rig.n_expr;
    const int k = o < 15 ? o : (o - 15) / rig.n_expr, l = o < 15 ? 0 : (o - 15) % rig.n_expr;
    const int j = k / 3, c = k - 3 * j;
    float acc = 0.f;
    for (int v = lane; v < rig.V; v += 64) {
        const float w = rig.J_regressor[(size_t)j * rig.V + v];
        if (w != 0.f) acc += w * (o < 15 ? prepared[3 * v + c] : rig.shapedirs[(size_t)(3 * v + c) * NB + rig.n_shape + l]);
    }
    acc = wave_sum_hi(acc);
    const int jo = prep_joint_offset(rig.V);
    if (lane == 63) prepared[o < 15 ? jo + o : jo + 16 + (o - 15)] = acc;
}

#ifndef GAB_FUSED_VERTS
#define GAB_FUSED_VERTS 8
#endif
template <bool FLAME_TREE>
__global__ __launch_bounds__(256) void k_flame_fused(Rig rig, const float* __restrict__ prepared, const float* __restrict__ expr,
                                                      const float* __restrict__ rotation, const float* __restrict__ neck,
                                                      const float* __restrict__ jaw, const float* __restrict__ eyes,
                                                      const float* __restrict__ translation, float* __restrict__ verts,
                                                      float* __restrict__ v_shaped, float* __restrict__ ws, const float* __restrict__ vs_pre)
{
    constexpr int VW = GAB_FUSED_VERTS, ROWS = 3 * VW, PER = ROWS / 8;
    __shared__ float out[WS_DA];
    __shared__ float vs[ROWS];
    __shared__ float po[ROWS];
    const int tid = threadIdx.x, lane = tid & 63, wid = tid >> 6;
    const int E = 3 * rig.V, NB = rig.n_shape + rig.n_expr;
    const int e0 = blockIdx.x * ROWS;
    const int jo = prep_joint_offset(rig.V);
    const int hw = 2 * wid + (lane >> 5), hl = lane & 31;
    const int nq = rig.n_expr >> 2;
    const bool vec = (rig.n_expr & 3) == 0 && (rig.n_shape & 3) == 0 && (NB & 3) == 0 && nq <= 32;
    float acc[PER];
#pragma unroll
    for (int r = 0; r < PER; ++r) acc[r] = 0.f;
    if (vs_pre) {
    } else if (vec) {
        float4 rw[PER];
        const float4 b = hl < nq ? reinterpret_cast<const float4*>(expr)[hl] : make_float4(0.f, 0.f, 0.f, 0.f);
#pragma unroll
        for (int r = 0; r < PER; ++r) {
            const int e = e0 + hw * PER + r;
            rw[r] = (e < E && hl < nq) ? reinterpret_cast<const float4*>(rig.shapedirs + (size_t)e * NB + rig.n_shape)[hl]
                                       : make_float4(0.f, 0.f, 0.f, 0.f);
        }
#pragma unroll
        for (int r = 0; r < PER; ++r) acc[r] = rw[r].x * b.x + rw[r].y * b.y + rw[r].z * b.z + rw[r].w * b.w;
    } else {
#pragma unroll
        for (int r = 0; r < PER; ++r) {
            const int e = e0 + hw * PER + r;
            if (e < E)
                for (int l = hl; l < rig.n_expr; l += 32) acc[r] += rig.shapedirs[(size_t)e * NB + rig.n_shape + l] * expr[l];
        }
    }
    if (tid < WS_DA) out[tid] = 0.f;
    __syncthreads();
    if (tid < 240) {
        const int k = tid >> 4, q = tid & 15;
        const float* mrow = prepared + jo + 16 + (size_t)k * rig.n_expr;
        float a = 0.f;
        for (int l = q; l < rig.n_expr; l += 16) a += mrow[l] * expr[l];
        a += dpp_f<0xB1, 0xf>(a);
        a += dpp_f<0x4E, 0xf>(a);
        a += dpp_f<0x141, 0xf>(a);
        a += dpp_f<0x140, 0xf>(a);
        if (q == 0) out[WS_J + k] = prepared[jo + k] + a;
    } else if (tid < 240 + GAB_NUM_JOINTS) {
        const int j = tid - 240;
        const float* pj = j == 0 ? rotation : j == 1 ? neck : j == 2 ? jaw : eyes + 3 * (j - 3);
        const float pose[3] = {pj[0], pj[1], pj[2]};
        float R[9];
        rodrigues(pose, R);
#pragma unroll
        for (int k = 0; k < 9; ++k) {
            out[WS_R + 9 * j + k] = R[k];
            if (j >= 1) out[WS_PF + 9 * (j - 1) + k] = R[k] - ((k % 4) == 0 ? 1.f : 0.f);
        }
    }
#pragma unroll
    for (int r = 0; r < PER; ++r) {
        float a = acc[r];
        a += dpp_f<0xB1, 0xf>(a);
        a += dpp_f<0x4E, 0xf>(a);
        a += dpp_f<0x141, 0xf>(a);
        a += dpp_f<0x140, 0xf>(a);
        a += dpp_f<0x142, 0xa>(a);
        const int e = e0 + hw * PER + r;
        if (hl == 31 && e < E) {
            const float x = vs_pre ? vs_pre[e] : prepared[e] + a;
            vs[hw * PER + r] = x;
            v_shaped[e] = x;
        }
    }
    __syncthreads();
    if (tid == 0) {
        float J[15], R[45], Rg[45], tg[15];
#pragma unroll
        for (int k = 0; k < 15; ++k) J[k] = out[WS_J + k];
#pragma unroll
        for (int k = 0; k < 45; ++k) R[k] = out[WS_R + k];
        chain_forward<FLAME_TREE>(rig.parents, R, J, Rg, tg);
#pragma unroll
        for (int j = 0; j < GAB_NUM_JOINTS; ++j)
#pragma unroll
            for (int r = 0; r < 3; ++r) {
#pragma unroll
                for (int c = 0; c < 3; ++c) out[WS_A + 12 * j + 4 * r + c] = Rg[9 * j + 3 * r + c];
                out[WS_A + 12 * j + 4 * r + 3] = tg[3 * j + r] - (Rg[9 * j + 3 * r] * J[3 * j] + Rg[9 * j + 3 * r + 1] * J[3 * j + 1] +
                                                                  Rg[9 * j + 3 * r + 2] * J[3 * j + 2]);
            }
    } else if (tid >= 64) {
        for (int vl = (tid - 64) >> 4; vl < VW; vl += 12) {
            const int v = blockIdx.x * VW + vl, q = tid & 15;
            float o[3] = {0.f, 0.f, 0.f};
            if (v < rig.V)
                for (int p = q; p < GAB_POSE_FEATURES; p += 16) {
                    const float f = out[WS_PF + p];
                    const float* row = rig.posedirs + (size_t)p * E + 3 * v;
                    o[0] += f * row[0]; o[1] += f * row[1]; o[2] += f * row[2];
                }
#pragma unroll
            for (int k = 0; k < 3; ++k) {
                float a = o[k];
                a += dpp_f<0xB1, 0xf>(a);
                a += dpp_f<0x4E, 0xf>(a);
                a += dpp_f<0x141, 0xf>(a);
                a += dpp_f<0x140, 0xf>(a);
                if (q == 0) po[3 * vl + k] = a;
            }
        }
    }
    __syncthreads();
    if (blockIdx.x == 0) {
        if (tid < WS_DA) ws[tid] = out[tid];
        for (int k = WS_DA + tid; k < GAB_FLAME_WS_FLOATS; k += 256) ws[k] = 0.f;
    }
    if (tid < VW) {
        const int v = blockIdx.x * VW + tid;
        if (v < rig.V) {
            float T[12];
#pragma unroll
            for (int k = 0; k < 12; ++k) T[k] = 0.f;
#pragma unroll
            for (int j = 0; j < GAB_NUM_JOINTS; ++j) {
                const float w = rig.lbs_weights[(size_t)v * GAB_NUM_JOINTS + j];
#pragma unroll
                for (int k = 0; k < 12; ++k) T[k] += w * out[WS_A + 12 * j + k];
            }
            const float vp[3] = {po[3 * tid] + vs[3 * tid], po[3 * tid + 1] + vs[3 * tid + 1], po[3 * tid + 2] + vs[3 * tid + 2]};
#pragma unroll
            for (int r = 0; r < 3; ++r)
                verts[3 * v + r] = T[4 * r] * vp[0] + T[4 * r + 1] * vp[1] + T[4 * r + 2] * vp[2] + T[4 * r + 3] + translation[r];
        }
    }
}

struct ZeroSpec { float* p[8]; int n[8]; int count; };

__global__ __launch_bounds__(256) void k_skin_bwd(Rig rig, float* __restrict__ ws, const float* __restrict__ v_shaped,
                                                   const float* __restrict__ dL_dverts, float* __restrict__ g_vs , ZeroSpec zero)
{
    __shared__ float red[4][100];
    const int tid = threadIdx.x, lane = tid & 63, wid = tid >> 6;
    const int v = blockIdx.x * blockDim.x + tid;
    for (int b = 0; b < zero.count; ++b)
        for (int i = v; i < zero.n[b]; i += (int)(gridDim.x * blockDim.x)) zero.p[b][i] = 0.f;
    const bool ok = v < rig.V;
    const int E = 3 * rig.V;
    float g[3] = {0.f, 0.f, 0.f}, vp[3] = {0.f, 0.f, 0.f}, T[12], gvp[3] = {0.f, 0.f, 0.f};
    float w[GAB_NUM_JOINTS] = {0.f, 0.f, 0.f, 0.f, 0.f};
    float pf[GAB_POSE_FEATURES];
#pragma unroll
    for (int p = 0; p < GAB_POSE_FEATURES; ++p) pf[p] = 0.f;
    if (ok) {
        vertex_posed_and_T<true>(rig, ws, v_shaped, v, vp, T);
#pragma unroll
        for (int k = 0; k < 3; ++k) g[k] = dL_dverts[3 * v + k];
#pragma unroll
        for (int c = 0; c < 3; ++c) gvp[c] = T[c] * g[0] + T[4 + c] * g[1] + T[8 + c] * g[2];
#pragma unroll
        for (int k = 0; k < 3; ++k) g_vs[3 * v + k] = gvp[k];
#pragma unroll
        for (int j = 0; j < GAB_NUM_JOINTS; ++j) w[j] = rig.lbs_weights[(size_t)v * GAB_NUM_JOINTS + j];
#pragma unroll
        for (int p = 0; p < GAB_POSE_FEATURES; ++p) {
            const float* row = rig.posedirs + (size_t)p * E + 3 * v;
            pf[p] = row[0] * gvp[0] + row[1] * gvp[1] + row[2] * gvp[2];
        }
    }
    const float vph[4] = {vp[0], vp[1], vp[2], ok ? 1.f : 0.f};
#pragma unroll
    for (int j = 0; j < GAB_NUM_JOINTS; ++j)
#pragma unroll
        for (int r = 0; r < 3; ++r)
#pragma unroll
            for (int c = 0; c < 4; ++c) {
                const float s = wave_sum_hi(w[j] * g[r] * vph[c]);
                if (lane == 63) red[wid][12 * j + 4 * r + c] = s;
            }
#pragma unroll
    for (int r = 0; r < 3; ++r) {
        const float s = wave_sum_hi(g[r]);
        if (lane == 63) red[wid][60 + r] = s;
    }
#pragma unroll
    for (int p = 0; p < GAB_POSE_FEATURES; ++p) {
        const float s = wave_sum_hi(pf[p]);
        if (lane == 63) red[wid][63 + p] = s;
    }
    __syncthreads();
    if (tid < 99) {
        const float s = (red[0][tid] + red[1][tid]) + (red[2][tid] + red[3][tid]);
        float* dst = tid < 60 ? &ws[WS_DA + tid] : (tid < 63 ? &ws[WS_DT + tid - 60] : &ws[WS_DPF + tid - 63]);
        unsafeAtomicAdd(dst, s);
    }
}

template <bool FLAME_TREE, int NT>
__device__ __forceinline__ void chain_bwd_body(Rig rig, float* __restrict__ ws, const float* __restrict__ rotation, const float* __restrict__ neck,
                            const float* __restrict__ jaw, const float* __restrict__ eyes, float* __restrict__ d_rotation,
                            float* __restrict__ d_neck, float* __restrict__ d_jaw, float* __restrict__ d_eyes,
                            float* __restrict__ d_translation, float* __restrict__ d_expr, float* __restrict__ d_shape,
                            const float* __restrict__ Mmat)
{
    __shared__ float sw[GAB_FLAME_WS_FLOATS];
    __shared__ float sdJ[16];
    for (int kk = threadIdx.x; kk < GAB_FLAME_WS_FLOATS; kk += NT) sw[kk] = ws[kk];
    __syncthreads();
    for (int kk = WS_DA + (int)threadIdx.x; kk < WS_DJ; kk += NT) ws[kk] = 0.f;
    if (!Mmat) {
        for (int kk = threadIdx.x; kk < rig.n_expr; kk += NT) d_expr[kk] = 0.f;
        if (d_shape)
            for (int kk = threadIdx.x; kk < rig.n_shape; kk += NT) d_shape[kk] = 0.f;
    }
    __shared__ float sdR[45];
    if (threadIdx.x == 0) {
    float J[15], R[45], Rg[45], tg[15];
#pragma unroll
    for (int k = 0; k < 15; ++k) J[k] = sw[WS_J + k];
#pragma unroll
    for (int k = 0; k < 45; ++k) R[k] = sw[WS_R + k];
    chain_forward<FLAME_TREE>(rig.parents, R, J, Rg, tg);
    float dRg[45], dtg[15], dJ[15], dR[45];
#pragma unroll
    for (int k = 0; k < 45; ++k) { dRg[k] = 0.f; dR[k] = 0.f; }
#pragma unroll
    for (int k = 0; k < 15; ++k) { dtg[k] = 0.f; dJ[k] = 0.f; }
#pragma unroll
    for (int i = 0; i < GAB_NUM_JOINTS; ++i) {
        const float* dA = sw + WS_DA + 12 * i;
#pragma unroll
        for (int r = 0; r < 3; ++r) {
            const float dAt = dA[4 * r + 3];
#pragma unroll
            for (int c = 0; c < 3; ++c) {
                dRg[9 * i + 3 * r + c] += dA[4 * r + c] - dAt * J[3 * i + c];
                dJ[3 * i + c] -= Rg[9 * i + 3 * r + c] * dAt;
            }
            dtg[3 * i + r] += dAt;
        }
    }
#pragma unroll
    for (int i = GAB_NUM_JOINTS - 1; i >= 1; --i) {
        const int p = parent_of<FLAME_TREE>(rig.parents, i);
        const float rel[3] = {J[3 * i] - J[3 * p], J[3 * i + 1] - J[3 * p + 1], J[3 * i + 2] - J[3 * p + 2]};
        float drel[3] = {0.f, 0.f, 0.f};
#pragma unroll
        for (int r = 0; r < 3; ++r) {
#pragma unroll
            for (int c = 0; c < 3; ++c) {
                dRg[9 * p + 3 * r + c] += dtg[3 * i + r] * rel[c];
                drel[c] += Rg[9 * p + 3 * r + c] * dtg[3 * i + r];
            }
            dtg[3 * p + r] += dtg[3 * i + r];
        }
#pragma unroll
        for (int c = 0; c < 3; ++c) { dJ[3 * i + c] += drel[c]; dJ[3 * p + c] -= drel[c]; }
#pragma unroll
        for (int r = 0; r < 3; ++r)
#pragma unroll
            for (int c = 0; c < 3; ++c) {
                float a = 0.f, b = 0.f;
#pragma unroll
                for (int k = 0; k < 3; ++k) {
                    a += dRg[9 * i + 3 * r + k] * R[9 * i + 3 * c + k];
                    b += Rg[9 * p + 3 * k + r] * dRg[9 * i + 3 * k + c];
                }
                dRg[9 * p + 3 * r + c] += a;
                dR[9 * i + 3 * r + c] += b;
            }
    }
#pragma unroll
    for (int k = 0; k < 9; ++k) dR[k] += dRg[k];
#pragma unroll
    for (int c = 0; c < 3; ++c) dJ[c] += dtg[c];
#pragma unroll
    for (int j = 1; j < GAB_NUM_JOINTS; ++j)
#pragma unroll
        for (int k = 0; k < 9; ++k) dR[9 * j + k] += sw[WS_DPF + 9 * (j - 1) + k];
#pragma unroll
    for (int k = 0; k < 45; ++k) sdR[k] = dR[k];
#pragma unroll
    for (int k = 0; k < 15; ++k) { ws[WS_DJ + k] = dJ[k]; sdJ[k] = dJ[k]; }
    }
    __syncthreads();
    if (Mmat)
        for (int l = threadIdx.x; l < rig.n_expr; l += NT) {
            float a = 0.f;
#pragma unroll
            for (int k = 0; k < 15; ++k) a += Mmat[(size_t)k * rig.n_expr + l] * sdJ[k];
            unsafeAtomicAdd(&d_expr[l], a);
        }
    const int j = threadIdx.x;
    if (j < GAB_NUM_JOINTS) {
        const float* pj = j == 0 ? rotation : j == 1 ? neck : j == 2 ? jaw : eyes + 3 * (j - 3);
        float* dj = j == 0 ? d_rotation : j == 1 ? d_neck : j == 2 ? d_jaw : d_eyes + 3 * (j - 3);
        const float pose[3] = {pj[0], pj[1], pj[2]};
        float dRj[9], dpose[3];
#pragma unroll
        for (int k = 0; k < 9; ++k) dRj[k] = sdR[9 * j + k];
        rodrigues_bwd(pose, dRj, dpose);
        dj[0] = dpose[0]; dj[1] = dpose[1]; dj[2] = dpose[2];
    } else if (j >= 8 && j < 11) {
        d_translation[j - 8] = sw[WS_DT + j - 8];
    }
}
template <bool FLAME_TREE>
__global__ __launch_bounds__(64) void k_chain_bwd(Rig rig, float* __restrict__ ws, const float* __restrict__ rotation, const float* __restrict__ neck,
                            const float* __restrict__ jaw, const float* __restrict__ eyes, float* __restrict__ d_rotation,
                            float* __restrict__ d_neck, float* __restrict__ d_jaw, float* __restrict__ d_eyes,
                            float* __restrict__ d_translation, float* __restrict__ d_expr, float* __restrict__ d_shape)
{
    chain_bwd_body<FLAME_TREE, 64>(rig, ws, rotation, neck, jaw, eyes, d_rotation, d_neck, d_jaw, d_eyes, d_translation, d_expr, d_shape, nullptr);
}

#define GAB_BLEND_BWD_ROWS 128
__device__ __forceinline__ void blend_bwd_body(Rig rig, const float* __restrict__ ws, const float* __restrict__ g_vs,
                                               const float* __restrict__ dL_dv_shaped, float* __restrict__ d_static_offset,
                                               float* __restrict__ d_shape, float* __restrict__ d_expr, int block)
{
    __shared__ float g[GAB_BLEND_BWD_ROWS];
    const int tid = threadIdx.x;
    const int E = 3 * rig.V;
    const int e0 = block * GAB_BLEND_BWD_ROWS;
    if (tid < GAB_BLEND_BWD_ROWS) {
        const int e = e0 + tid;
        float x = 0.f;
        if (e < E) {
            const int v = e / 3, k = e - 3 * v;
            x = g_vs[e];
            if (ws)
                for (int j = 0; j < GAB_NUM_JOINTS; ++j) x += rig.J_regressor[(size_t)j * rig.V + v] * ws[WS_DJ + 3 * j + k];
            if (dL_dv_shaped) x += dL_dv_shaped[e];
            if (d_static_offset) d_static_offset[e] = x;
        }
        g[tid] = x;
    }
    __syncthreads();
    const int NB = rig.n_shape + rig.n_expr;
    const int rows = min(GAB_BLEND_BWD_ROWS, E - e0);
    const int c0 = d_shape ? 0 : rig.n_shape, nC = NB - c0;
    __shared__ float part[128];
    const int cl = tid & 127, half = tid >> 7;
    const int r0 = half * (GAB_BLEND_BWD_ROWS / 2), r1 = min(rows, r0 + GAB_BLEND_BWD_ROWS / 2);
    for (int cb = 0; cb < nC; cb += 128) {
        const int c = cb + cl;
        float acc = 0.f;
        if (c < nC) {
            const float* col = rig.shapedirs + (size_t)e0 * NB + c0 + c;
            int r = r0;
            for (; r + 8 <= r1; r += 8) {
                float x[8];
#pragma unroll
                for (int k = 0; k < 8; ++k) x[k] = col[(size_t)(r + k) * NB];
#pragma unroll
                for (int k = 0; k < 8; ++k) acc += x[k] * g[r + k];
            }
            for (; r < r1; ++r) acc += col[(size_t)r * NB] * g[r];
        }
        if (half == 1) part[cl] = acc;
        __syncthreads();
        if (half == 0 && c < nC) {
            const int l = c0 + c;
            float* dst = l < rig.n_shape ? d_shape + l : d_expr + (l - rig.n_shape);
            unsafeAtomicAdd(dst, acc + part[cl]);
        }
        __syncthreads();
    }
}
__global__ __launch_bounds__(256) void k_blend_bwd(Rig rig, const float* __restrict__ ws, const float* __restrict__ g_vs,
                                                    const float* __restrict__ dL_dv_shaped, float* __restrict__ d_static_offset,
                                                    float* __restrict__ d_shape, float* __restrict__ d_expr)
{
    blend_bwd_body(rig, ws, g_vs, dL_dv_shaped, d_static_offset, d_shape, d_expr, (int)blockIdx.x);
}
template <bool FLAME_TREE>
__global__ __launch_bounds__(256) void k_chain_blend_bwd(Rig rig, float* __restrict__ ws, const float* __restrict__ g_vs, const float* __restrict__ Mmat,
                                                          const float* __restrict__ rotation, const float* __restrict__ neck,
                                                          const float* __restrict__ jaw, const float* __restrict__ eyes,
                                                          float* __restrict__ d_rotation, float* __restrict__ d_neck, float* __restrict__ d_jaw,
                                                          float* __restrict__ d_eyes, float* __restrict__ d_translation, float* __restrict__ d_expr)
{
    if (blockIdx.x == 0)
        chain_bwd_body<FLAME_TREE, 256>(rig, ws, rotation, neck, jaw, eyes, d_rotation, d_neck, d_jaw, d_eyes, d_translation, d_expr, nullptr, Mmat);
    else
        blend_bwd_body(rig, nullptr, g_vs, nullptr, nullptr, nullptr, d_expr, (int)blockIdx.x - 1);
}

struct Vec3 { float x, y, z; };
__device__ __forceinline__ Vec3 operator-(Vec3 a, Vec3 b) { return {a.x - b.x, a.y - b.y, a.z - b.z}; }
__device__ __forceinline__ Vec3 operator+(Vec3 a, Vec3 b) { return {a.x + b.x, a.y + b.y, a.z + b.z}; }
__device__ __forceinline__ Vec3 operator*(Vec3 a, float s) { return {a.x * s, a.y * s, a.z * s}; }
__device__ __forceinline__ float dot(Vec3 a, Vec3 b) { return a.x * b.x + a.y * b.y + a.z * b.z; }
__device__ __forceinline__ Vec3 cross(Vec3 a, Vec3 b) { return {a.y * b.z - a.z * b.y, a.z * b.x - a.x * b.z, a.x * b.y - a.y * b.x}; }
__device__ __forceinline__ Vec3 ld3(const float* p, long long i) { return {p[3 * i], p[3 * i + 1], p[3 * i + 2]}; }

__device__ __forceinline__ long long index_at(const void* idx, int is64, long long i)
{
    return is64 ? ((const long long*)idx)[i] : (long long)((const int*)idx)[i];
}

struct Frame {
    Vec3 e1, e2, a0, a1, a2, n, m;
    float l1, ln, lm, d;
    bool c1, cn, cm;
};
__device__ __forceinline__ Frame make_frame(Vec3 v0, Vec3 v1, Vec3 v2)
{
    Frame f;
    const float eps = 1e-20f;
    f.e1 = v1 - v0;
    f.e2 = v2 - v0;
    float q = dot(f.e1, f.e1);
    f.c1 = q < eps; f.l1 = sqrtf(f.c1 ? eps : q);
    f.a0 = f.e1 * (1.f / f.l1);
    f.n = cross(f.a0, f.e2);
    q = dot(f.n, f.n);
    f.cn = q < eps; f.ln = sqrtf(f.cn ? eps : q);
    f.a1 = f.n * (1.f / f.ln);
    f.m = cross(f.a1, f.a0);
    q = dot(f.m, f.m);
    f.cm = q < eps; f.lm = sqrtf(f.cm ? eps : q);
    f.a2 = f.m * (-1.f / f.lm);
    f.d = dot(f.a2, f.e2);
    return f;
}

__device__ __forceinline__ int quat_raw(const float* R, float* q)
{
    const float tr = R[0] + R[4] + R[8];
    const float dec[4] = {R[0], R[4], R[8], tr};
    int c = 0;
    for (int k = 1; k < 4; ++k) if (dec[k] > dec[c]) c = k;
    if (c < 3) {
        const int i = c, j = (i + 1) % 3, k = (j + 1) % 3;
        q[i] = 1.f - tr + 2.f * R[4 * i];
        q[j] = R[3 * j + i] + R[3 * i + j];
        q[k] = R[3 * k + i] + R[3 * i + k];
        q[3] = R[3 * k + j] - R[3 * j + k];
    } else {
        q[0] = R[7] - R[5];
        q[1] = R[2] - R[6];
        q[2] = R[3] - R[1];
        q[3] = 1.f + tr;
    }
    return c;
}

__global__ __launch_bounds__(256) void k_face_frames(int F, const float* __restrict__ verts, const void* __restrict__ faces, int is64,
                                                      float* __restrict__ center, float* __restrict__ Rm, float* __restrict__ scaling,
                                                      float* __restrict__ quat, float* __restrict__ zero_fill, int zero_count)
{
    const int f = blockIdx.x * blockDim.x + threadIdx.x;
    if (zero_fill)
        for (int k = f; k < zero_count; k += (int)(gridDim.x * blockDim.x)) zero_fill[k] = 0.f;
    if (f >= F) return;
    const Vec3 v0 = ld3(verts, index_at(faces, is64, 3ll * f)), v1 = ld3(verts, index_at(faces, is64, 3ll * f + 1)),
               v2 = ld3(verts, index_at(faces, is64, 3ll * f + 2));
    const Frame fr = make_frame(v0, v1, v2);
    const Vec3 c = (v0 + v1 + v2) * (1.f / 3.f);
    center[3 * f] = c.x; center[3 * f + 1] = c.y; center[3 * f + 2] = c.z;
    const float R[9] = {fr.a0.x, fr.a1.x, fr.a2.x, fr.a0.y, fr.a1.y, fr.a2.y, fr.a0.z, fr.a1.z, fr.a2.z};
    for (int k = 0; k < 9; ++k) Rm[9 * f + k] = R[k];
    scaling[f] = (fr.l1 + fabsf(fr.d)) * 0.5f;
    float q[4];
    quat_raw(R, q);
    const float inv = 1.f / sqrtf(q[0] * q[0] + q[1] * q[1] + q[2] * q[2] + q[3] * q[3]);
    quat[4 * f] = q[3] * inv;
    quat[4 * f + 1] = q[0] * inv;
    quat[4 * f + 2] = q[1] * inv;
    quat[4 * f + 3] = q[2] * inv;
}

__device__ __forceinline__ Vec3 unit_bwd(Vec3 g_unit, Vec3 unit, float len, bool clamped)
{
    if (clamped) return g_unit * (1.f / len);
    return (g_unit - unit * dot(unit, g_unit)) * (1.f / len);
}

__device__ __forceinline__ void face_frame_bwd(int f, Vec3 v0, Vec3 v1, Vec3 v2, const float* __restrict__ d_center, const float* __restrict__ d_R,
                                               const float* __restrict__ d_scaling, const float* __restrict__ d_quat, Vec3& g0, Vec3& g1, Vec3& g2)
{
    const Frame fr = make_frame(v0, v1, v2);
    const float R[9] = {fr.a0.x, fr.a1.x, fr.a2.x, fr.a0.y, fr.a1.y, fr.a2.y, fr.a0.z, fr.a1.z, fr.a2.z};
    float gR[9];
    for (int k = 0; k < 9; ++k) gR[k] = d_R ? d_R[9 * f + k] : 0.f;
    if (d_quat) {
        float q[4];
        const int c = quat_raw(R, q);
        const float len = sqrtf(q[0] * q[0] + q[1] * q[1] + q[2] * q[2] + q[3] * q[3]);
        const float qn[4] = {q[0] / len, q[1] / len, q[2] / len, q[3] / len};
        const float g[4] = {d_quat[4 * f + 1], d_quat[4 * f + 2], d_quat[4 * f + 3], d_quat[4 * f]};
        const float gd = qn[0] * g[0] + qn[1] * g[1] + qn[2] * g[2] + qn[3] * g[3];
        float gq[4];
        for (int k = 0; k < 4; ++k) gq[k] = (g[k] - qn[k] * gd) / len;
        if (c < 3) {
            const int i = c, j = (i + 1) % 3, k = (j + 1) % 3;
            gR[0] -= gq[i]; gR[4] -= gq[i]; gR[8] -= gq[i];
            gR[4 * i] += 2.f * gq[i];
            gR[3 * j + i] += gq[j]; gR[3 * i + j] += gq[j];
            gR[3 * k + i] += gq[k]; gR[3 * i + k] += gq[k];
            gR[3 * k + j] += gq[3]; gR[3 * j + k] -= gq[3];
        } else {
            gR[7] += gq[0]; gR[5] -= gq[0];
            gR[2] += gq[1]; gR[6] -= gq[1];
            gR[3] += gq[2]; gR[1] -= gq[2];
            gR[0] += gq[3]; gR[4] += gq[3]; gR[8] += gq[3];
        }
    }
    Vec3 g_a0 = {gR[0], gR[3], gR[6]}, g_a1 = {gR[1], gR[4], gR[7]}, g_a2 = {gR[2], gR[5], gR[8]};
    Vec3 g_e2 = {0.f, 0.f, 0.f};
    float g_l1 = 0.f;
    if (d_scaling) {
        const float gs = d_scaling[f] * 0.5f;
        g_l1 = gs;
        const float sg = fr.d > 0.f ? 1.f : (fr.d < 0.f ? -1.f : 0.f);
        g_a2 = g_a2 + fr.e2 * (gs * sg);
        g_e2 = g_e2 + fr.a2 * (gs * sg);
    }
    const Vec3 u = fr.a2 * -1.f;
    const Vec3 g_m = unit_bwd(g_a2 * -1.f, u, fr.lm, fr.cm);
    g_a1 = g_a1 + cross(fr.a0, g_m);
    g_a0 = g_a0 + cross(g_m, fr.a1);
    const Vec3 g_n = unit_bwd(g_a1, fr.a1, fr.ln, fr.cn);
    g_a0 = g_a0 + cross(fr.e2, g_n);
    g_e2 = g_e2 + cross(g_n, fr.a0);
    Vec3 g_e1 = unit_bwd(g_a0, fr.a0, fr.l1, fr.c1);
    if (!fr.c1) g_e1 = g_e1 + fr.a0 * g_l1;
    Vec3 gc = {0.f, 0.f, 0.f};
    if (d_center) gc = Vec3{d_center[3 * f], d_center[3 * f + 1], d_center[3 * f + 2]} * (1.f / 3.f);
    g0 = gc - g_e1 - g_e2; g1 = gc + g_e1; g2 = gc + g_e2;
}

__global__ __launch_bounds__(256) void k_face_frames_bwd(int F, const float* __restrict__ verts, const void* __restrict__ faces, int is64,
                                                          const float* __restrict__ d_center, const float* __restrict__ d_R,
                                                          const float* __restrict__ d_scaling, const float* __restrict__ d_quat,
                                                          float* __restrict__ d_verts)
{
    const int f = blockIdx.x * blockDim.x + threadIdx.x;
    if (f >= F) return;
    const long long i0 = index_at(faces, is64, 3ll * f), i1 = index_at(faces, is64, 3ll * f + 1), i2 = index_at(faces, is64, 3ll * f + 2);
    Vec3 g0, g1, g2;
    face_frame_bwd(f, ld3(verts, i0), ld3(verts, i1), ld3(verts, i2), d_center, d_R, d_scaling, d_quat, g0, g1, g2);
    unsafeAtomicAdd(&d_verts[3 * i0], g0.x); unsafeAtomicAdd(&d_verts[3 * i0 + 1], g0.y); unsafeAtomicAdd(&d_verts[3 * i0 + 2], g0.z);
    unsafeAtomicAdd(&d_verts[3 * i1], g1.x); unsafeAtomicAdd(&d_verts[3 * i1 + 1], g1.y); unsafeAtomicAdd(&d_verts[3 * i1 + 2], g1.z);
    unsafeAtomicAdd(&d_verts[3 * i2], g2.x); unsafeAtomicAdd(&d_verts[3 * i2 + 1], g2.y); unsafeAtomicAdd(&d_verts[3 * i2 + 2], g2.z);
}

#ifndef GAB_MESH_VPB
#define GAB_MESH_VPB 32
#endif
struct GatherSkinArgs {
    const float* v_shaped; float* ws;
    const float* verts;
    const int* vf_begin; const int4* vf_list;
    const float* d_center; const float* d_R; const float* d_scaling; const float* d_quat;
    const float* g_verts;
    float* g_vs;
};
__global__ __launch_bounds__(256) void k_gather_skin_bwd(Rig rig, GatherSkinArgs a, ZeroSpec zero)
{
    constexpr int VPB = GAB_MESH_VPB, ROWS = 3 * VPB;
    static_assert(VPB == 16 || VPB == 32 || VPB == 64, "a wave holds the workgroup's vertices");
    __shared__ float gv[ROWS];
    __shared__ float red[100];
    constexpr int PDN = GAB_POSE_FEATURES * ROWS, PDK = (PDN + 255) / 256;
    __shared__ float pd[GAB_POSE_FEATURES][ROWS];
    const int tid = threadIdx.x, lane = tid & 63, wid = __builtin_amdgcn_readfirstlane(tid >> 6);
    const int gid = blockIdx.x * 256 + tid;
    for (int b = 0; b < zero.count; ++b)
        for (int i = gid; i < zero.n[b]; i += (int)(gridDim.x * 256)) zero.p[b][i] = 0.f;
    const int vbase = blockIdx.x * VPB, vend = min(vbase + VPB, rig.V);
    const int E = 3 * rig.V;
    const int p0 = a.vf_begin[vbase], p1 = a.vf_begin[vend];
    float pdr[PDK];
#pragma unroll
    for (int i = 0; i < PDK; ++i) {
        const int k = tid + 256 * i, p = k / ROWS, c = k - p * ROWS;
        pdr[i] = (k < PDN && 3 * vbase + c < E) ? rig.posedirs[(size_t)p * E + 3 * vbase + c] : 0.f;
    }
    const int v = vbase + lane;
    const bool ok = lane < VPB && v < rig.V;
    float vs[3] = {0.f, 0.f, 0.f}, gx[3] = {0.f, 0.f, 0.f};
    float w[GAB_NUM_JOINTS] = {0.f, 0.f, 0.f, 0.f, 0.f};
    if (ok) {
#pragma unroll
        for (int k = 0; k < 3; ++k) { vs[k] = a.v_shaped[3 * v + k]; gx[k] = a.g_verts ? a.g_verts[3 * v + k] : 0.f; }
#pragma unroll
        for (int j = 0; j < GAB_NUM_JOINTS; ++j) w[j] = rig.lbs_weights[(size_t)v * GAB_NUM_JOINTS + j];
    }
    for (int k = tid; k < ROWS; k += 256) gv[k] = 0.f;
    __syncthreads();
    float tc[3] = {0.f, 0.f, 0.f};
    for (int p = p0 + tid; p < p1; p += 256) {
        const int4 e = a.vf_list[p];
        const int f = e.x >> 2, c = e.x & 3;
        Vec3 g0, g1, g2;
        face_frame_bwd(f, ld3(a.verts, e.y), ld3(a.verts, e.z), ld3(a.verts, e.w), a.d_center, a.d_R, a.d_scaling, a.d_quat, g0, g1, g2);
        const Vec3 g = c == 0 ? g0 : (c == 1 ? g1 : g2);
        const int vl = (c == 0 ? e.y : (c == 1 ? e.z : e.w)) - vbase;
        atomicAdd(&gv[3 * vl], g.x); atomicAdd(&gv[3 * vl + 1], g.y); atomicAdd(&gv[3 * vl + 2], g.z);
        if (a.d_center) {
#pragma unroll
            for (int r = 0; r < 3; ++r) tc[r] += a.d_center[3 * f + r] * (1.0f / 3.0f);
        }
    }
    __shared__ float tcs[4][3];
#pragma unroll
    for (int r = 0; r < 3; ++r) {
        const float s = wave_sum_hi(tc[r]);
        if (lane == 63) tcs[wid][r] = s;
    }
#pragma unroll
    for (int i = 0; i < PDK; ++i) {
        const int k = tid + 256 * i;
        if (k < PDN) (&pd[0][0])[k] = pdr[i];
    }
    __syncthreads();
    float g[3] = {0.f, 0.f, 0.f}, vp[3] = {0.f, 0.f, 0.f}, T[12], gvp[3] = {0.f, 0.f, 0.f};
    float pf[GAB_POSE_FEATURES];
#pragma unroll
    for (int p = 0; p < GAB_POSE_FEATURES; ++p) pf[p] = 0.f;
    if (ok) {
        float po[3] = {0.f, 0.f, 0.f};
#pragma unroll
        for (int p = 0; p < GAB_POSE_FEATURES; ++p) {
            const float f = a.ws[WS_PF + p];
            po[0] += f * pd[p][3 * lane]; po[1] += f * pd[p][3 * lane + 1]; po[2] += f * pd[p][3 * lane + 2];
        }
#pragma unroll
        for (int k = 0; k < 3; ++k) vp[k] = po[k] + vs[k];
#pragma unroll
        for (int k = 0; k < 12; ++k) T[k] = 0.f;
#pragma unroll
        for (int j = 0; j < GAB_NUM_JOINTS; ++j)
#pragma unroll
            for (int k = 0; k < 12; ++k) T[k] += w[j] * a.ws[WS_A + 12 * j + k];
#pragma unroll
        for (int k = 0; k < 3; ++k) g[k] = gv[3 * lane + k] + gx[k];
#pragma unroll
        for (int c = 0; c < 3; ++c) gvp[c] = T[c] * g[0] + T[4 + c] * g[1] + T[8 + c] * g[2];
#pragma unroll
        for (int p = 0; p < GAB_POSE_FEATURES; ++p) pf[p] = pd[p][3 * lane] * gvp[0] + pd[p][3 * lane + 1] * gvp[1] + pd[p][3 * lane + 2] * gvp[2];
        if (wid == 0) { a.g_vs[3 * v] = gvp[0]; a.g_vs[3 * v + 1] = gvp[1]; a.g_vs[3 * v + 2] = gvp[2]; }
    }
    const float vph[4] = {vp[0], vp[1], vp[2], ok ? 1.f : 0.f};
#pragma unroll
    for (int j = 0; j < GAB_NUM_JOINTS; ++j) {
        if (wid != (j >> 1)) continue;
#pragma unroll
        for (int r = 0; r < 3; ++r)
#pragma unroll
            for (int c = 0; c < 4; ++c) {
                const float s = wave_sum_hi(w[j] * g[r] * vph[c]);
                if (lane == 63) red[12 * j + 4 * r + c] = s;
            }
    }
    if (wid == 2) {
#pragma unroll
        for (int r = 0; r < 3; ++r) {
            const float s = wave_sum_hi(gx[r]);
            if (lane == 63) red[60 + r] = s + ((tcs[0][r] + tcs[1][r]) + (tcs[2][r] + tcs[3][r]));
        }
    }
#pragma unroll
    for (int p = 0; p < GAB_POSE_FEATURES; ++p) {
        if (wid != (p < 9 ? 2 : 3)) continue;
        const float s = wave_sum_hi(pf[p]);
        if (lane == 63) red[63 + p] = s;
    }
    __syncthreads();
    if (tid < 99) {
        float* dst = tid < 60 ? &a.ws[WS_DA + tid] : (tid < 63 ? &a.ws[WS_DT + tid - 60] : &a.ws[WS_DPF + tid - 63]);
        unsafeAtomicAdd(dst, red[tid]);
    }
}

using bindm::qmul;
using bindm::qconj;
using bindm::qnorm_clamped;

__global__ __launch_bounds__(256) void k_bind(int N, const float* __restrict__ xyz, const float* __restrict__ log_scaling,
                                               const float* __restrict__ rotation, const void* __restrict__ binding, int is64,
                                               const float* __restrict__ fc, const float* __restrict__ fR, const float* __restrict__ fs,
                                               const float* __restrict__ fq, float* __restrict__ out_xyz, float* __restrict__ out_scaling,
                                               float* __restrict__ out_rotation, const float* __restrict__ opacity_logit,
                                               float* __restrict__ out_opacity)
{
    const int i = blockIdx.x * blockDim.x + threadIdx.x;
    if (i >= N) return;
    if (opacity_logit) out_opacity[i] = bindm::sigmoid(opacity_logit[i]);
    const long long f = index_at(binding, is64, i);
    const float s = fs[f];
    float w[3];
    bindm::world_xyz(fR + 9 * f, s, fc + 3 * f, xyz[3 * i], xyz[3 * i + 1], xyz[3 * i + 2], w);
    for (int r = 0; r < 3; ++r) out_xyz[3 * i + r] = w[r];
    for (int k = 0; k < 3; ++k) out_scaling[3 * i + k] = bindm::world_scaling(log_scaling[3 * i + k], s);
    reinterpret_cast<float4*>(out_rotation)[i] = bindm::world_rotation(reinterpret_cast<const float4*>(fq)[f], reinterpret_cast<const float4*>(rotation)[i]);
}

__global__ __launch_bounds__(256) void k_bind_bwd(int N, const float* __restrict__ xyz, const float* __restrict__ log_scaling,
                                                   const float* __restrict__ rotation, const void* __restrict__ binding, int is64,
                                                   const float* __restrict__ fR, const float* __restrict__ fs, const float* __restrict__ fq,
                                                   const float* __restrict__ g_xyz, const float* __restrict__ g_scaling,
                                                   const float* __restrict__ g_rot, float* __restrict__ d_xyz,
                                                   float* __restrict__ d_log_scaling, float* __restrict__ d_rotation, float* __restrict__ d_face, int F,
                                                   const float* __restrict__ out_opacity, const float* __restrict__ g_opacity,
                                                   float* __restrict__ d_opacity_logit)
{
    const int i = blockIdx.x * blockDim.x + threadIdx.x;
    if (i >= N) return;
    if (d_opacity_logit) {
        const float o = out_opacity[i];
        d_opacity_logit[i] = (g_opacity ? g_opacity[i] : 0.f) * o * (1.f - o);
    }
    const long long f = index_at(binding, is64, i);
    const float s = fs[f];
    const float* R = fR + 9 * f;
    float* dfc = d_face + 3 * f;
    float* dfR = d_face + (size_t)3 * F + 9 * f;
    float* dfs = d_face + (size_t)12 * F + f;
    float* dfq = d_face + (size_t)13 * F + 4 * f;
    float ds = 0.f;
    const float x[3] = {xyz[3 * i], xyz[3 * i + 1], xyz[3 * i + 2]};
    const float gx[3] = {g_xyz ? g_xyz[3 * i] : 0.f, g_xyz ? g_xyz[3 * i + 1] : 0.f, g_xyz ? g_xyz[3 * i + 2] : 0.f};
    for (int c = 0; c < 3; ++c) d_xyz[3 * i + c] = s * (R[c] * gx[0] + R[3 + c] * gx[1] + R[6 + c] * gx[2]);
    if (g_xyz) {
        for (int r = 0; r < 3; ++r) {
            unsafeAtomicAdd(&dfc[r], gx[r]);
            const float rx = R[3 * r] * x[0] + R[3 * r + 1] * x[1] + R[3 * r + 2] * x[2];
            ds += gx[r] * rx;
            for (int c = 0; c < 3; ++c) unsafeAtomicAdd(&dfR[3 * r + c], s * gx[r] * x[c]);
        }
    }
    for (int k = 0; k < 3; ++k) {
        const float e = expf(log_scaling[3 * i + k]);
        const float g = g_scaling ? g_scaling[3 * i + k] : 0.f;
        d_log_scaling[3 * i + k] = g * e * s;
        ds += g * e;
    }
    unsafeAtomicAdd(dfs, ds);
    const float4 qf = reinterpret_cast<const float4*>(fq)[f];
    const float4 q = reinterpret_cast<const float4*>(rotation)[i];
    const float na = qnorm_clamped(qf), nb = qnorm_clamped(q);
    const float4 a = make_float4(qf.x / na, qf.y / na, qf.z / na, qf.w / na);
    const float4 b = make_float4(q.x / nb, q.y / nb, q.z / nb, q.w / nb);
    const float4 g = g_rot ? reinterpret_cast<const float4*>(g_rot)[i] : make_float4(0.f, 0.f, 0.f, 0.f);
    const float4 da = qmul(g, qconj(b));
    const float4 db = qmul(qconj(a), g);
    const float ada = a.x * da.x + a.y * da.y + a.z * da.z + a.w * da.w;
    const float bdb = b.x * db.x + b.y * db.y + b.z * db.z + b.w * db.w;
    reinterpret_cast<float4*>(d_rotation)[i] = make_float4((db.x - b.x * bdb) / nb, (db.y - b.y * bdb) / nb, (db.z - b.z * bdb) / nb, (db.w - b.w * bdb) / nb);
    if (g_rot) {
        unsafeAtomicAdd(&dfq[0], (da.x - a.x * ada) / na);
        unsafeAtomicAdd(&dfq[1], (da.y - a.y * ada) / na);
        unsafeAtomicAdd(&dfq[2], (da.z - a.z * ada) / na);
        unsafeAtomicAdd(&dfq[3], (da.w - a.w * ada) / na);
    }
}

__global__ __launch_bounds__(256) void k_bind_bwd_csr(int F, const float* __restrict__ xyz, const float* __restrict__ log_scaling,
                                                       const float* __restrict__ rotation, const float* __restrict__ fR,
                                                       const float* __restrict__ fs, const float* __restrict__ fq,
                                                       const float* __restrict__ g_xyz, const float* __restrict__ g_scaling,
                                                       const float* __restrict__ g_rot, const int* __restrict__ order,
                                                       const int* __restrict__ face_begin, float* __restrict__ d_xyz,
                                                       float* __restrict__ d_log_scaling, float* __restrict__ d_rotation,
                                                       float* __restrict__ d_face, const float* __restrict__ out_opacity,
                                                       const float* __restrict__ g_opacity, float* __restrict__ d_opacity_logit)
{
    const int gtid = blockIdx.x * blockDim.x + threadIdx.x;
    const int f = gtid >> 4, sub = gtid & 15;
    const bool okf = f < F;
    float acc[17];
#pragma unroll
    for (int k = 0; k < 17; ++k) acc[k] = 0.f;
    if (okf) {
        const float s = fs[f];
        float R[9];
#pragma unroll
        for (int k = 0; k < 9; ++k) R[k] = fR[9 * f + k];
        const float4 qf = reinterpret_cast<const float4*>(fq)[f];
        const float na = qnorm_clamped(qf);
        const float4 a = make_float4(qf.x / na, qf.y / na, qf.z / na, qf.w / na);
        const int b0 = face_begin[f], b1 = face_begin[f + 1];
        for (int j = b0 + sub; j < b1; j += 16) {
            const int i = order[j];
            if (d_opacity_logit) {
                const float o = out_opacity[i];
                d_opacity_logit[i] = (g_opacity ? g_opacity[i] : 0.f) * o * (1.f - o);
            }
            const float x[3] = {xyz[3 * i], xyz[3 * i + 1], xyz[3 * i + 2]};
            const float gx[3] = {g_xyz ? g_xyz[3 * i] : 0.f, g_xyz ? g_xyz[3 * i + 1] : 0.f, g_xyz ? g_xyz[3 * i + 2] : 0.f};
#pragma unroll
            for (int c = 0; c < 3; ++c) d_xyz[3 * i + c] = s * (R[c] * gx[0] + R[3 + c] * gx[1] + R[6 + c] * gx[2]);
#pragma unroll
            for (int r = 0; r < 3; ++r) {
                acc[r] += gx[r];
                acc[12] += gx[r] * (R[3 * r] * x[0] + R[3 * r + 1] * x[1] + R[3 * r + 2] * x[2]);
#pragma unroll
                for (int c = 0; c < 3; ++c) acc[3 + 3 * r + c] += s * gx[r] * x[c];
            }
#pragma unroll
            for (int k = 0; k < 3; ++k) {
                const float e = expf(log_scaling[3 * i + k]);
                const float g = g_scaling ? g_scaling[3 * i + k] : 0.f;
                d_log_scaling[3 * i + k] = g * e * s;
                acc[12] += g * e;
            }
            const float4 q = reinterpret_cast<const float4*>(rotation)[i];
            const float nb = qnorm_clamped(q);
            const float4 b = make_float4(q.x / nb, q.y / nb, q.z / nb, q.w / nb);
            const float4 g = g_rot ? reinterpret_cast<const float4*>(g_rot)[i] : make_float4(0.f, 0.f, 0.f, 0.f);
            const float4 da = qmul(g, qconj(b));
            const float4 db = qmul(qconj(a), g);
            const float ada = a.x * da.x + a.y * da.y + a.z * da.z + a.w * da.w;
            const float bdb = b.x * db.x + b.y * db.y + b.z * db.z + b.w * db.w;
            reinterpret_cast<float4*>(d_rotation)[i] =
                make_float4((db.x - b.x * bdb) / nb, (db.y - b.y * bdb) / nb, (db.z - b.z * bdb) / nb, (db.w - b.w * bdb) / nb);
            acc[13] += (da.x - a.x * ada) / na;
            acc[14] += (da.y - a.y * ada) / na;
            acc[15] += (da.z - a.z * ada) / na;
            acc[16] += (da.w - a.w * ada) / na;
        }
    }
#pragma unroll
    for (int k = 0; k < 17; ++k) {
// ... 231 lines not shown
    const unsigned period = schedule ? (unsigned)n_sched : (unsigned)T;
    int t = schedule ? schedule[c % period] : (int)c;
    t = (int)((unsigned)t % (unsigned)T);
    for (int k = threadIdx.x; k < width; k += 256) row[k] = packed[(size_t)t * width + k];
    __syncthreads();
    if (threadIdx.x == 0) *cursor = (int)((c + 1u) % period);
}

__global__ __launch_bounds__(256) void k_zero_many(ZeroSpec z)
{
    const int b = blockIdx.y;
    if (b >= z.count) return;
    float* p = z.p[b];
    for (int i = blockIdx.x * blockDim.x + threadIdx.x; i < z.n[b]; i += gridDim.x * blockDim.x) p[i] = 0.f;
}

}

namespace {
thread_local char g_err[512] = "";
int fail(int code, const char* fmt, ...)
{
    va_list ap;
    va_start(ap, fmt);
    vsnprintf(g_err, sizeof(g_err), fmt, ap);
    va_end(ap);
    return code;
}
#define HIP_TRY(expr)                                                                                    \
    do {                                                                                                 \
        hipError_t e_ = (expr);                                                                          \
        if (e_ != hipSuccess) return fail(GAB_E_HIP, "%s failed: %s", #expr, hipGetErrorString(e_));     \
    } while (0)
#define LAUNCH_CHECK(name)                                                                               \
    do {                                                                                                 \
        hipError_t e_ = hipGetLastError();                                                               \
        if (e_ != hipSuccess) return fail(GAB_E_HIP, "launch of %s failed: %s", name, hipGetErrorString(e_)); \
    } while (0)

int to_rig(const GabRig* r, gab::Rig* o)
{
    if (!r) return fail(GAB_E_ARG, "rig is NULL");
    if (r->V <= 0 || r->n_shape < 0 || r->n_expr < 0 || r->n_shape + r->n_expr <= 0) return fail(GAB_E_ARG, "bad rig sizes");
    if (!r->v_template || !r->shapedirs || !r->posedirs || !r->J_regressor || !r->lbs_weights) return fail(GAB_E_ARG, "NULL rig buffer");
    if (r->parents[0] != -1) return fail(GAB_E_ARG, "parents[0] must be -1");
    for (int i = 1; i < GAB_NUM_JOINTS; ++i)
        if (r->parents[i] < 0 || r->parents[i] >= i) return fail(GAB_E_ARG, "parents must be topologically ordered");
    o->V = r->V; o->n_shape = r->n_shape; o->n_expr = r->n_expr;
    o->v_template = r->v_template; o->shapedirs = r->shapedirs; o->posedirs = r->posedirs;
    o->J_regressor = r->J_regressor; o->lbs_weights = r->lbs_weights;
    for (int i = 0; i < GAB_NUM_JOINTS; ++i) o->parents[i] = r->parents[i];
    return 0;
}
}

extern "C" {

int gab_abi_version(void) { return GAB_ABI_VERSION; }
const char* gab_last_error(void) { return g_err; }

int gab_flame_forward(const GabRig* rig_, const float* shape, const float* expr, const float* rotation, const float* neck,
                      const float* jaw, const float* eyes, const float* translation, const float* static_offset, float* verts,
                      float* v_shaped, float* ws, void* stream_)
{
    gab::Rig rig;
    if (int rc = to_rig(rig_, &rig)) return rc;
    if ((rig.n_shape && !shape) || (rig.n_expr && !expr) || !rotation || !neck || !jaw || !eyes || !translation || !verts || !v_shaped || !ws)
        return fail(GAB_E_ARG, "gab_flame_forward: NULL buffer");
    hipStream_t st = (hipStream_t)stream_;
    const int E = 3 * rig.V;
    PROF_LAUNCH(gab::k_blend, dim3((E + 3) / 4), dim3(256), 0, st, rig, shape, expr, static_offset, v_shaped);
    LAUNCH_CHECK("k_blend");
    const bool flame_tree = rig.parents[1] == 0 && rig.parents[2] == 1 && rig.parents[3] == 1 && rig.parents[4] == 1;
    if (flame_tree)
        PROF_LAUNCH(gab::k_joints_chain<true>, dim3(1), dim3(1024), 0, st, rig, (const float*)v_shaped, rotation, neck, jaw, eyes, ws);
    else
        PROF_LAUNCH(gab::k_joints_chain<false>, dim3(1), dim3(1024), 0, st, rig, (const float*)v_shaped, rotation, neck, jaw, eyes, ws);
    LAUNCH_CHECK("k_joints_chain");
    PROF_LAUNCH(gab::k_skin, dim3((rig.V + 255) / 256), dim3(256), 0, st, rig, (const float*)ws, (const float*)v_shaped, translation, verts);
    LAUNCH_CHECK("k_skin");
    return GAB_OK;
}

int gab_flame_backward(const GabRig* rig_, const float* shape, const float* expr, const float* rotation, const float* neck,
                       const float* jaw, const float* eyes, const float* translation, const float* static_offset,
                       const float* v_shaped, float* ws, const float* dL_dverts, const float* dL_dv_shaped, float* d_shape,
                       float* d_expr, float* d_rotation, float* d_neck, float* d_jaw, float* d_eyes, float* d_translation,
                       float* d_static_offset, float* scratch, int32_t zero_count, float* const* zero_buffers_host,
                       const int32_t* zero_sizes_host, void* stream_)
{
    (void)shape; (void)expr; (void)translation; (void)static_offset;
    if (zero_count < 0 || zero_count > 8 || (zero_count > 0 && (!zero_buffers_host || !zero_sizes_host)))
        return fail(GAB_E_ARG, "gab_flame_backward: 0..8 zero-fill buffers");
    gab::ZeroSpec zs;
    zs.count = zero_count;
    for (int i = 0; i < 8; ++i) {
        zs.p[i] = i < zero_count ? zero_buffers_host[i] : nullptr;
        zs.n[i] = i < zero_count ? zero_sizes_host[i] : 0;
        if (i < zero_count && (zs.n[i] < 0 || (zs.n[i] > 0 && !zs.p[i]))) return fail(GAB_E_ARG, "gab_flame_backward: bad zero-fill buffer %d", i);
    }
    gab::Rig rig;
    if (int rc = to_rig(rig_, &rig)) return rc;
    if (!rotation || !neck || !jaw || !eyes || !v_shaped || !ws || !dL_dverts || !d_expr || !d_rotation || !d_neck || !d_jaw || !d_eyes ||
        !d_translation || !scratch)
        return fail(GAB_E_ARG, "gab_flame_backward: NULL buffer");
    hipStream_t st = (hipStream_t)stream_;
    const int E = 3 * rig.V;
    PROF_LAUNCH(gab::k_skin_bwd, dim3((rig.V + 255) / 256), dim3(256), 0, st, rig, ws, v_shaped, dL_dverts, scratch, zs);
    LAUNCH_CHECK("k_skin_bwd");
    const bool flame_tree = rig.parents[1] == 0 && rig.parents[2] == 1 && rig.parents[3] == 1 && rig.parents[4] == 1;
    if (flame_tree)
        PROF_LAUNCH(gab::k_chain_bwd<true>, dim3(1), dim3(64), 0, st, rig, ws, rotation, neck, jaw, eyes, d_rotation, d_neck, d_jaw, d_eyes, d_translation, d_expr, d_shape);
    else
        PROF_LAUNCH(gab::k_chain_bwd<false>, dim3(1), dim3(64), 0, st, rig, ws, rotation, neck, jaw, eyes, d_rotation, d_neck, d_jaw, d_eyes, d_translation, d_expr, d_shape);
    LAUNCH_CHECK("k_chain_bwd");
    PROF_LAUNCH(gab::k_blend_bwd, dim3((E + GAB_BLEND_BWD_ROWS - 1) / GAB_BLEND_BWD_ROWS), dim3(256), 0, st, rig, (const float*)ws,
                       (const float*)scratch, dL_dv_shaped, d_static_offset, d_shape, d_expr);
    LAUNCH_CHECK("k_blend_bwd");
    return GAB_OK;
}

int64_t gab_flame_prepared_floats(const GabRig* rig_)
{
    if (!rig_ || rig_->V <= 0 || rig_->n_expr < 0) return -1;
    return (int64_t)gab::prep_joint_offset(rig_->V) + 16 + 15 * (int64_t)rig_->n_expr;
}

int gab_flame_prepare(const GabRig* rig_, const float* shape, const float* static_offset, float* prepared, void* stream_)
{
    gab::Rig rig;
    if (int rc = to_rig(rig_, &rig)) return rc;
    if ((rig.n_shape && !shape) || !prepared) return fail(GAB_E_ARG, "gab_flame_prepare: NULL buffer");
    hipStream_t st = (hipStream_t)stream_;
    const int E = 3 * rig.V, outs = 15 + 15 * rig.n_expr;
    PROF_LAUNCH(gab::k_prep_rows, dim3((E + 3) / 4), dim3(256), 0, st, rig, shape, static_offset, prepared);
    LAUNCH_CHECK("k_prep_rows");
    PROF_LAUNCH(gab::k_prep_joints, dim3((outs + 3) / 4), dim3(256), 0, st, rig, prepared);
    LAUNCH_CHECK("k_prep_joints");
    return GAB_OK;
}

int gab_flame_forward_prepared(const GabRig* rig_, const float* prepared, const float* expr, const float* rotation, const float* neck,
                               const float* jaw, const float* eyes, const float* translation, float* verts, float* v_shaped, float* ws,
                               void* stream_)
{
    gab::Rig rig;
    if (int rc = to_rig(rig_, &rig)) return rc;
    if (!prepared || (rig.n_expr && !expr) || !rotation || !neck || !jaw || !eyes || !translation || !verts || !v_shaped || !ws)
        return fail(GAB_E_ARG, "gab_flame_forward_prepared: NULL buffer");
    hipStream_t st = (hipStream_t)stream_;
    const int blocks = (rig.V + GAB_FUSED_VERTS - 1) / GAB_FUSED_VERTS;
    const bool flame_tree = rig.parents[1] == 0 && rig.parents[2] == 1 && rig.parents[3] == 1 && rig.parents[4] == 1;
    if (flame_tree)
        PROF_LAUNCH(gab::k_flame_fused<true>, dim3(blocks), dim3(256), 0, st, rig, prepared, expr, rotation, neck, jaw, eyes, translation, verts, v_shaped, ws, (const float*)nullptr);
    else
        PROF_LAUNCH(gab::k_flame_fused<false>, dim3(blocks), dim3(256), 0, st, rig, prepared, expr, rotation, neck, jaw, eyes, translation, verts, v_shaped, ws, (const float*)nullptr);
    LAUNCH_CHECK("k_flame_fused");
    return GAB_OK;
}

int gab_blend_sequence(const GabRig* rig_, const float* prepared, const float* expr_table, int32_t T, float* v_shaped_seq, void* stream_)
{
    gab::Rig rig;
    if (int rc = to_rig(rig_, &rig)) return rc;
    if (T < 0 || (T > 0 && (!prepared || !expr_table || !v_shaped_seq))) return fail(GAB_E_ARG, "gab_blend_sequence: bad arguments");
    if (T == 0) return GAB_OK;
    if (rig.n_expr <= 0) return fail(GAB_E_ARG, "gab_blend_sequence: the rig has no expression block");
    const int E = 3 * rig.V;
    const int gx = ((E + 31) / 32 + 3) / 4, mtiles = (T + 31) / 32;
    const int MT = std::min(16, std::max(1, (mtiles * gx + 511) / 512));
    dim3 grid((unsigned)gx, (unsigned)((mtiles + MT - 1) / MT));
    PROF_LAUNCH(gab::k_blend_seq_mfma, grid, dim3(256), 0, (hipStream_t)stream_, rig, prepared, expr_table, (int)T, MT, v_shaped_seq);
    LAUNCH_CHECK("k_blend_seq_mfma");
    return GAB_OK;
}

int gab_flame_forward_sequence(const GabRig* rig_, const float* prepared, const float* v_shaped_row, const float* expr, const float* rotation,
                               const float* neck, const float* jaw, const float* eyes, const float* translation, float* verts, float* v_shaped,
                               float* ws, void* stream_)
{
    gab::Rig rig;
    if (int rc = to_rig(rig_, &rig)) return rc;
    if (!prepared || !v_shaped_row || (rig.n_expr && !expr) || !rotation || !neck || !jaw || !eyes || !translation || !verts || !v_shaped || !ws)
        return fail(GAB_E_ARG, "gab_flame_forward_sequence: NULL buffer");
    hipStream_t st = (hipStream_t)stream_;
    const int blocks = (rig.V + GAB_FUSED_VERTS - 1) / GAB_FUSED_VERTS;
    const bool flame_tree = rig.parents[1] == 0 && rig.parents[2] == 1 && rig.parents[3] == 1 && rig.parents[4] == 1;
    if (flame_tree)
        PROF_LAUNCH(gab::k_flame_fused<true>, dim3(blocks), dim3(256), 0, st, rig, prepared, expr, rotation, neck, jaw, eyes, translation, verts, v_shaped, ws, v_shaped_row);
    else
        PROF_LAUNCH(gab::k_flame_fused<false>, dim3(blocks), dim3(256), 0, st, rig, prepared, expr, rotation, neck, jaw, eyes, translation, verts, v_shaped, ws, v_shaped_row);
    LAUNCH_CHECK("k_flame_fused");
    return GAB_OK;
}

int gab_flame_backward_prepared(const GabRig* rig_, const float* prepared, const float* rotation, const float* neck, const float* jaw,
                                const float* eyes, const float* v_shaped, float* ws, const float* dL_dverts, float* d_expr,
                                float* d_rotation, float* d_neck, float* d_jaw, float* d_eyes, float* d_translation, float* scratch,
                                int32_t zero_count, float* const* zero_buffers_host, const int32_t* zero_sizes_host, void* stream_)
{
    if (zero_count < 0 || zero_count > 7 || (zero_count > 0 && (!zero_buffers_host || !zero_sizes_host)))
        return fail(GAB_E_ARG, "gab_flame_backward_prepared: 0..7 zero-fill buffers");
    gab::Rig rig;
    if (int rc = to_rig(rig_, &rig)) return rc;
    if (!prepared || !rotation || !neck || !jaw || !eyes || !v_shaped || !ws || !dL_dverts || !d_expr || !d_rotation || !d_neck || !d_jaw ||
        !d_eyes || !d_translation || !scratch)
        return fail(GAB_E_ARG, "gab_flame_backward_prepared: NULL buffer");
    gab::ZeroSpec zs;
    bool covers_expr = false;
    for (int i = 0; i < 8; ++i) {
        zs.p[i] = i < zero_count ? zero_buffers_host[i] : nullptr;
        zs.n[i] = i < zero_count ? zero_sizes_host[i] : 0;
        if (i < zero_count && (zs.n[i] < 0 || (zs.n[i] > 0 && !zs.p[i]))) return fail(GAB_E_ARG, "gab_flame_backward_prepared: bad zero-fill buffer %d", i);
        if (i < zero_count && d_expr >= zs.p[i] && d_expr + rig.n_expr <= zs.p[i] + zs.n[i]) covers_expr = true;
    }
    zs.count = zero_count;
    if (!covers_expr) { zs.p[zs.count] = d_expr; zs.n[zs.count] = rig.n_expr; ++zs.count; }
    hipStream_t st = (hipStream_t)stream_;
    const int E = 3 * rig.V;
    PROF_LAUNCH(gab::k_skin_bwd, dim3((rig.V + 255) / 256), dim3(256), 0, st, rig, ws, v_shaped, dL_dverts, scratch, zs);
    LAUNCH_CHECK("k_skin_bwd");
    const float* Mmat = prepared + gab::prep_joint_offset(rig.V) + 16;
    const int blocks = 1 + (E + GAB_BLEND_BWD_ROWS - 1) / GAB_BLEND_BWD_ROWS;
    const bool flame_tree = rig.parents[1] == 0 && rig.parents[2] == 1 && rig.parents[3] == 1 && rig.parents[4] == 1;
    if (flame_tree)
        PROF_LAUNCH(gab::k_chain_blend_bwd<true>, dim3(blocks), dim3(256), 0, st, rig, ws, (const float*)scratch, Mmat, rotation, neck, jaw, eyes,
                           d_rotation, d_neck, d_jaw, d_eyes, d_translation, d_expr);
    else
        PROF_LAUNCH(gab::k_chain_blend_bwd<false>, dim3(blocks), dim3(256), 0, st, rig, ws, (const float*)scratch, Mmat, rotation, neck, jaw, eyes,
                           d_rotation, d_neck, d_jaw, d_eyes, d_translation, d_expr);
    LAUNCH_CHECK("k_chain_blend_bwd");
    return GAB_OK;
}

int gab_mesh_backward_prepared(const GabRig* rig_, const float* prepared, const float* rotation, const float* neck, const float* jaw,
                               const float* eyes, const float* v_shaped, float* ws, const float* verts, const int32_t* vf_begin,
                               const int32_t* vf_list, const float* d_center, const float* d_orien_mat, const float* d_scaling,
                               const float* d_orien_quat, const float* dL_dverts, float* d_expr, float* d_rotation, float* d_neck,
                               float* d_jaw, float* d_eyes, float* d_translation, float* scratch, int32_t zero_count,
                               float* const* zero_buffers_host, const int32_t* zero_sizes_host, void* stream_)
{
    if (zero_count < 0 || zero_count > 7 || (zero_count > 0 && (!zero_buffers_host || !zero_sizes_host)))
        return fail(GAB_E_ARG, "gab_mesh_backward_prepared: 0..7 zero-fill buffers");
    gab::Rig rig;
    if (int rc = to_rig(rig_, &rig)) return rc;
    if (!prepared || !rotation || !neck || !jaw || !eyes || !v_shaped || !ws || !verts || !vf_begin || !vf_list || !d_expr || !d_rotation ||
        !d_neck || !d_jaw || !d_eyes || !d_translation || !scratch)
        return fail(GAB_E_ARG, "gab_mesh_backward_prepared: NULL buffer");
    gab::ZeroSpec zs;
    bool covers_expr = false;
    for (int i = 0; i < 8; ++i) {
        zs.p[i] = i < zero_count ? zero_buffers_host[i] : nullptr;
        zs.n[i] = i < zero_count ? zero_sizes_host[i] : 0;
        if (i < zero_count && (zs.n[i] < 0 || (zs.n[i] > 0 && !zs.p[i]))) return fail(GAB_E_ARG, "gab_mesh_backward_prepared: bad zero-fill buffer %d", i);
        if (i < zero_count && d_expr >= zs.p[i] && d_expr + rig.n_expr <= zs.p[i] + zs.n[i]) covers_expr = true;
    }
    zs.count = zero_count;
    if (!covers_expr) { zs.p[zs.count] = d_expr; zs.n[zs.count] = rig.n_expr; ++zs.count; }
    gab::GatherSkinArgs a;
    a.v_shaped = v_shaped; a.ws = ws; a.verts = verts;
    a.vf_begin = vf_begin; a.vf_list = reinterpret_cast<const int4*>(vf_list);
    a.d_center = d_center; a.d_R = d_orien_mat; a.d_scaling = d_scaling; a.d_quat = d_orien_quat; a.g_verts = dL_dverts;
    a.g_vs = scratch;
    hipStream_t st = (hipStream_t)stream_;
    PROF_LAUNCH(gab::k_gather_skin_bwd, dim3((rig.V + GAB_MESH_VPB - 1) / GAB_MESH_VPB), dim3(256), 0, st, rig, a, zs);
    LAUNCH_CHECK("k_gather_skin_bwd");
    const int E = 3 * rig.V;
    const float* Mmat = prepared + gab::prep_joint_offset(rig.V) + 16;
    const int blocks = 1 + (E + GAB_BLEND_BWD_ROWS - 1) / GAB_BLEND_BWD_ROWS;
    const bool flame_tree = rig.parents[1] == 0 && rig.parents[2] == 1 && rig.parents[3] == 1 && rig.parents[4] == 1;
    if (flame_tree)
        PROF_LAUNCH(gab::k_chain_blend_bwd<true>, dim3(blocks), dim3(256), 0, st, rig, ws, (const float*)scratch, Mmat, rotation, neck, jaw, eyes,
                           d_rotation, d_neck, d_jaw, d_eyes, d_translation, d_expr);
    else
        PROF_LAUNCH(gab::k_chain_blend_bwd<false>, dim3(blocks), dim3(256), 0, st, rig, ws, (const float*)scratch, Mmat, rotation, neck, jaw, eyes,
                           d_rotation, d_neck, d_jaw, d_eyes, d_translation, d_expr);
    LAUNCH_CHECK("k_chain_blend_bwd");
    return GAB_OK;
}

int gab_face_frames_forward(int32_t V, int32_t F, const float* verts, const void* faces, int32_t is64, float* center, float* orien_mat,
                            float* scaling, float* orien_quat, float* d_verts_zeroed, void* stream_)
{
    if (V <= 0 || F < 0) return fail(GAB_E_ARG, "bad sizes");
    if (F == 0) {
        if (d_verts_zeroed) HIP_TRY(hipMemsetAsync(d_verts_zeroed, 0, (size_t)V * 3 * sizeof(float), (hipStream_t)stream_));
        return GAB_OK;
    }
    if (!verts || !faces || !center || !orien_mat || !scaling || !orien_quat) return fail(GAB_E_ARG, "gab_face_frames_forward: NULL buffer");
    PROF_LAUNCH(gab::k_face_frames, dim3((F + 255) / 256), dim3(256), 0, (hipStream_t)stream_, F, verts, faces, is64, center, orien_mat,
                       scaling, orien_quat, d_verts_zeroed, 3 * V);
    LAUNCH_CHECK("k_face_frames");
    return GAB_OK;
}

int gab_face_frames_backward(int32_t V, int32_t F, const float* verts, const void* faces, int32_t is64, const float* d_center,
                             const float* d_orien_mat, const float* d_scaling, const float* d_orien_quat, float* d_verts,
                             int32_t d_verts_is_zero, void* stream_)
{
    if (V <= 0 || F < 0) return fail(GAB_E_ARG, "bad sizes");
    if (!d_verts) return fail(GAB_E_ARG, "d_verts is NULL");
    hipStream_t st = (hipStream_t)stream_;
    if (!d_verts_is_zero) HIP_TRY(hipMemsetAsync(d_verts, 0, (size_t)V * 3 * sizeof(float), st));
    if (F == 0) return GAB_OK;
    if (!verts || !faces) return fail(GAB_E_ARG, "gab_face_frames_backward: NULL buffer");
    PROF_LAUNCH(gab::k_face_frames_bwd, dim3((F + 255) / 256), dim3(256), 0, st, F, verts, faces, is64, d_center, d_orien_mat, d_scaling,
                       d_orien_quat, d_verts);
    LAUNCH_CHECK("k_face_frames_bwd");
    return GAB_OK;
}

int gab_bind_forward(int32_t N, int32_t F, const float* xyz, const float* log_scaling, const float* rotation, const void* binding,
                     int32_t is64, const float* face_center, const float* face_orien_mat, const float* face_scaling,
                     const float* face_orien_quat, float* out_xyz, float* out_scaling, float* out_rotation, const float* opacity_logit,
                     float* out_opacity, void* stream_)
{
    if (N < 0 || F <= 0) return fail(GAB_E_ARG, "bad sizes");
    if (N == 0) return GAB_OK;
    if ((opacity_logit == nullptr) != (out_opacity == nullptr)) return fail(GAB_E_ARG, "opacity_logit and out_opacity go together");
    if (!xyz || !log_scaling || !rotation || !binding || !face_center || !face_orien_mat || !face_scaling || !face_orien_quat || !out_xyz ||
        !out_scaling || !out_rotation)
        return fail(GAB_E_ARG, "gab_bind_forward: NULL buffer");
    PROF_LAUNCH(gab::k_bind, dim3((N + 255) / 256), dim3(256), 0, (hipStream_t)stream_, N, xyz, log_scaling, rotation, binding, is64,
                       face_center, face_orien_mat, face_scaling, face_orien_quat, out_xyz, out_scaling, out_rotation, opacity_logit, out_opacity);
    LAUNCH_CHECK("k_bind");
    return GAB_OK;
}

int gab_bind_backward(int32_t N, int32_t F, const float* xyz, const float* log_scaling, const float* rotation, const void* binding,
                      int32_t is64, const float* face_center, const float* face_orien_mat, const float* face_scaling,
                      const float* face_orien_quat, const float* d_out_xyz, const float* d_out_scaling, const float* d_out_rotation,
                      float* d_xyz, float* d_log_scaling, float* d_rotation, float* d_face, const float* out_opacity,
                      const float* d_out_opacity, float* d_opacity_logit, void* stream_)
{
    (void)face_center;
    if (d_opacity_logit && !out_opacity) return fail(GAB_E_ARG, "d_opacity_logit needs out_opacity");
    if (N < 0 || F <= 0) return fail(GAB_E_ARG, "bad sizes");
    if (!d_face) return fail(GAB_E_ARG, "d_face is NULL");
    hipStream_t st = (hipStream_t)stream_;
    HIP_TRY(hipMemsetAsync(d_face, 0, (size_t)F * 17 * sizeof(float), st));
    if (N == 0) return GAB_OK;
    if (!xyz || !log_scaling || !rotation || !binding || !face_orien_mat || !face_scaling || !face_orien_quat || !d_xyz || !d_log_scaling ||
        !d_rotation)
        return fail(GAB_E_ARG, "gab_bind_backward: NULL buffer");
    PROF_LAUNCH(gab::k_bind_bwd, dim3((N + 255) / 256), dim3(256), 0, st, N, xyz, log_scaling, rotation, binding, is64, face_orien_mat,
                       face_scaling, face_orien_quat, d_out_xyz, d_out_scaling, d_out_rotation, d_xyz, d_log_scaling, d_rotation, d_face, F,
                       out_opacity, d_out_opacity, d_opacity_logit);
    LAUNCH_CHECK("k_bind_bwd");
    return GAB_OK;
}

int gab_bind_backward_csr(int32_t N, int32_t F, const float* xyz, const float* log_scaling, const float* rotation,
                          const float* face_orien_mat, const float* face_scaling, const float* face_orien_quat,
                          const float* d_out_xyz, const float* d_out_scaling, const float* d_out_rotation, const int32_t* order,
                          const int32_t* face_begin, float* d_xyz, float* d_log_scaling, float* d_rotation, float* d_face,
                          const float* out_opacity, const float* d_out_opacity, float* d_opacity_logit,
                          const int32_t* splat_face, const int32_t* slot, float* rows, void* stream_)
{
    if (d_opacity_logit && !out_opacity) return fail(GAB_E_ARG, "d_opacity_logit needs out_opacity");
    if (N < 0 || F <= 0) return fail(GAB_E_ARG, "bad sizes");
    if (!d_face || !order || !face_begin) return fail(GAB_E_ARG, "gab_bind_backward_csr: NULL buffer");
    if (N > 0 && (!xyz || !log_scaling || !rotation || !face_orien_mat || !face_scaling || !face_orien_quat || !d_xyz || !d_log_scaling ||
                  !d_rotation))
        return fail(GAB_E_ARG, "gab_bind_backward_csr: NULL buffer");
    const long long threads = 16ll * F;
    if (splat_face && slot && rows) {
        if (N > 0) {
            PROF_LAUNCH(gab::k_bind_bwd_rows, dim3((unsigned)((N + 255) / 256)), dim3(256), 0, (hipStream_t)stream_, N, xyz, log_scaling,
                               rotation, splat_face, slot, face_orien_mat, face_scaling, face_orien_quat, d_out_xyz, d_out_scaling,
                               d_out_rotation, d_xyz, d_log_scaling, d_rotation, rows, out_opacity, d_out_opacity, d_opacity_logit);
            LAUNCH_CHECK("k_bind_bwd_rows");
        }
        PROF_LAUNCH(gab::k_bind_bwd_faces, dim3((unsigned)((threads + 255) / 256)), dim3(256), 0, (hipStream_t)stream_, F, face_begin,
                           (const float*)rows, d_face);
        LAUNCH_CHECK("k_bind_bwd_faces");
        return GAB_OK;
    }
    PROF_LAUNCH(gab::k_bind_bwd_csr, dim3((unsigned)((threads + 255) / 256)), dim3(256), 0, (hipStream_t)stream_, F, xyz, log_scaling,
                       rotation, face_orien_mat, face_scaling, face_orien_quat, d_out_xyz, d_out_scaling, d_out_rotation, order, face_begin,
                       d_xyz, d_log_scaling, d_rotation, d_face, out_opacity, d_out_opacity, d_opacity_logit);
    LAUNCH_CHECK("k_bind_bwd_csr");
    return GAB_OK;
}

int gab_bind_backward_faces(int32_t F, const int32_t* face_begin, const float* rows, float* d_face, void* stream_)
{
    if (F <= 0 || !face_begin || !rows || !d_face) return fail(GAB_E_ARG, "gab_bind_backward_faces: bad arguments");
    const long long threads = 16ll * F;
    PROF_LAUNCH(gab::k_bind_bwd_faces, dim3((unsigned)((threads + 255) / 256)), dim3(256), 0, (hipStream_t)stream_, F, face_begin, rows, d_face);
    LAUNCH_CHECK("k_bind_bwd_faces");
    return GAB_OK;
}

int gab_feed_row(const float* packed, int32_t T, int32_t width, const int32_t* schedule, int32_t n_sched, int32_t* cursor, float* row,
                 void* stream_)
{
    if (T <= 0 || width <= 0 || !packed || !cursor || !row || (schedule && n_sched <= 0)) return fail(GAB_E_ARG, "gab_feed_row: bad arguments");
    PROF_LAUNCH(gab::k_feed_row, dim3(1), dim3(256), 0, (hipStream_t)stream_, packed, T, width, schedule, n_sched, cursor, row);
    LAUNCH_CHECK("k_feed_row");
    return GAB_OK;
}

int gab_zero_buffers(int32_t count, float* const* buffers_host, const int32_t* sizes_host, void* stream_)
{
    if (count < 0 || count > 8 || (count > 0 && (!buffers_host || !sizes_host))) return fail(GAB_E_ARG, "gab_zero_buffers: 0..8 buffers");
    if (count == 0) return GAB_OK;
    gab::ZeroSpec z;
    z.count = count;
    int mx = 0;
    for (int i = 0; i < 8; ++i) {
        z.p[i] = i < count ? buffers_host[i] : nullptr;
        z.n[i] = i < count ? sizes_host[i] : 0;
        if (i < count && (sizes_host[i] < 0 || (sizes_host[i] > 0 && !buffers_host[i]))) return fail(GAB_E_ARG, "gab_zero_buffers: bad buffer %d", i);
        if (z.n[i] > mx) mx = z.n[i];
    }
    int bx = (mx + 255) / 256;
    if (bx < 1) bx = 1;
    if (bx > 64) bx = 64;
    PROF_LAUNCH(gab::k_zero_many, dim3(bx, count), dim3(256), 0, (hipStream_t)stream_, z);
    LAUNCH_CHECK("k_zero_many");
    return GAB_OK;
}

int gab_profile_enable(int on)
{
    lprof::g.on.store(on ? 1 : 0);
    return 0;
}
int gab_profile_collect(void) { return lprof::collect(); }
int gab_profile_entry(int32_t index, const char** name, double* total_ms, int64_t* launches)
// ... 14 lines not shown
```

### include/gab.h

```cpp
#ifndef GAB_H
#define GAB_H

#include <stddef.h>
#include <stdint.h>

#ifdef __cplusplus
extern "C" {
#endif

#define GAB_ABI_VERSION 5
#define GAB_OK 0
#define GAB_E_ARG (-1)
#define GAB_E_HIP (-2)

#define GAB_NUM_JOINTS 5
#define GAB_POSE_FEATURES 36
#define GAB_FLAME_WS_FLOATS 512

typedef struct GabRig {
    int32_t V;
    int32_t n_shape;
    int32_t n_expr;
    const float* v_template;
    const float* shapedirs;
    const float* posedirs;
    const float* J_regressor;
    const float* lbs_weights;
    int32_t parents[GAB_NUM_JOINTS];
} GabRig;

int gab_abi_version(void);
const char* gab_last_error(void);

int gab_flame_forward(const GabRig* rig, const float* shape, const float* expr, const float* rotation,
                      const float* neck, const float* jaw, const float* eyes , const float* translation,
                      const float* static_offset ,
                      float* verts , float* v_shaped , float* ws , void* stream);

int gab_flame_backward(const GabRig* rig, const float* shape, const float* expr, const float* rotation,
                       const float* neck, const float* jaw, const float* eyes, const float* translation,
                       const float* static_offset, const float* v_shaped, float* ws,
                       const float* dL_dverts, const float* dL_dv_shaped,
                       float* d_shape, float* d_expr, float* d_rotation, float* d_neck, float* d_jaw, float* d_eyes,
                       float* d_translation, float* d_static_offset, float* scratch,
                       int32_t zero_count, float* const* zero_buffers_host, const int32_t* zero_sizes_host, void* stream);

int64_t gab_flame_prepared_floats(const GabRig* rig);
int gab_flame_prepare(const GabRig* rig, const float* shape, const float* static_offset , float* prepared, void* stream);
int gab_flame_forward_prepared(const GabRig* rig, const float* prepared, const float* expr, const float* rotation, const float* neck,
                               const float* jaw, const float* eyes , const float* translation,
                               float* verts , float* v_shaped , float* ws , void* stream);
int gab_blend_sequence(const GabRig* rig, const float* prepared, const float* expr_table , int32_t T,
                       float* v_shaped_seq , void* stream);
int gab_flame_forward_sequence(const GabRig* rig, const float* prepared, const float* v_shaped_row , const float* expr,
                               const float* rotation, const float* neck, const float* jaw, const float* eyes , const float* translation,
                               float* verts , float* v_shaped , float* ws , void* stream);
int gab_flame_backward_prepared(const GabRig* rig, const float* prepared, const float* rotation, const float* neck, const float* jaw,
                                const float* eyes, const float* v_shaped, float* ws, const float* dL_dverts,
                                float* d_expr, float* d_rotation, float* d_neck, float* d_jaw, float* d_eyes, float* d_translation,
                                float* scratch, int32_t zero_count, float* const* zero_buffers_host, const int32_t* zero_sizes_host,
                                void* stream);

int gab_mesh_backward_prepared(const GabRig* rig, const float* prepared, const float* rotation, const float* neck, const float* jaw,
                               const float* eyes, const float* v_shaped, float* ws, const float* verts ,
                               const int32_t* vf_begin, const int32_t* vf_list, const float* d_center, const float* d_orien_mat,
                               const float* d_scaling, const float* d_orien_quat, const float* dL_dverts ,
                               float* d_expr, float* d_rotation, float* d_neck, float* d_jaw, float* d_eyes, float* d_translation,
                               float* scratch, int32_t zero_count, float* const* zero_buffers_host, const int32_t* zero_sizes_host,
                               void* stream);

int gab_face_frames_forward(int32_t V, int32_t F, const float* verts, const void* faces , int32_t index_is_i64,
                            float* center , float* orien_mat , float* scaling ,
                            float* orien_quat , float* d_verts_zeroed, void* stream);
int gab_face_frames_backward(int32_t V, int32_t F, const float* verts, const void* faces, int32_t index_is_i64,
                             const float* d_center, const float* d_orien_mat, const float* d_scaling, const float* d_orien_quat,
                             float* d_verts, int32_t d_verts_is_zero, void* stream);

int gab_bind_forward(int32_t N, int32_t F, const float* xyz, const float* log_scaling, const float* rotation,
                     const void* binding, int32_t index_is_i64, const float* face_center, const float* face_orien_mat,
                     const float* face_scaling, const float* face_orien_quat,
                     float* out_xyz, float* out_scaling, float* out_rotation,
                     const float* opacity_logit, float* out_opacity, void* stream);
int gab_bind_backward(int32_t N, int32_t F, const float* xyz, const float* log_scaling, const float* rotation,
                      const void* binding, int32_t index_is_i64, const float* face_center, const float* face_orien_mat,
                      const float* face_scaling, const float* face_orien_quat,
                      const float* d_out_xyz, const float* d_out_scaling, const float* d_out_rotation,
                      float* d_xyz, float* d_log_scaling, float* d_rotation, float* d_face ,
                      const float* out_opacity, const float* d_out_opacity, float* d_opacity_logit, void* stream);

#define GAB_BIND_ROW_FLOATS 20
int gab_bind_backward_csr(int32_t N, int32_t F, const float* xyz, const float* log_scaling, const float* rotation,
                          const float* face_orien_mat, const float* face_scaling, const float* face_orien_quat,
                          const float* d_out_xyz, const float* d_out_scaling, const float* d_out_rotation,
                          const int32_t* order, const int32_t* face_begin,
                          float* d_xyz, float* d_log_scaling, float* d_rotation, float* d_face ,
                          const float* out_opacity, const float* d_out_opacity, float* d_opacity_logit,
                          const int32_t* splat_face, const int32_t* slot, float* rows, void* stream);

int gab_bind_backward_faces(int32_t F, const int32_t* face_begin, const float* rows, float* d_face , void* stream);

int gab_zero_buffers(int32_t count, float* const* buffers_host, const int32_t* sizes_host, void* stream);

int gab_feed_row(const float* packed, int32_t T, int32_t width, const int32_t* schedule, int32_t n_sched, int32_t* cursor, float* row,
                 void* stream);

int gab_profile_enable(int on);
int gab_profile_collect(void);
int gab_profile_entry(int32_t index, const char** name, double* total_ms, int64_t* launches);
int gab_profile_reset(void);

#ifdef __cplusplus
}
#endif
#endif
```

Baseline: 3831 frames/s.

## Fuse face-frame computation into skinning kernel and single-launch mesh backward via counters

Adds a fused mesh forward where the FLAME skinning kernel computes per-face frames once all of a face's vertices are written, tracked by per-face arrival counters. It also adds a fused backward that merges the gather/skin backward with the joint-chain backward through a ticket counter and an accumulator buffer. Per-stream counter tensors are cached, and the path is skipped during graph capture. The aim is to cut kernel launches and intermediate traffic in the mesh stage, at the cost of atomics and cross-block ordering that depend on counters being reset correctly between calls.

```diff
diff --git a/gaussianavatars_amd/_lib.py b/gaussianavatars_amd/_lib.py
--- a/gaussianavatars_amd/_lib.py
+++ b/gaussianavatars_amd/_lib.py
@@ -197,6 +197,11 @@
                                     [C.c_int32, C.POINTER(C.c_void_p), C.POINTER(C.c_int32), _P]),
     "gab_mesh_backward_prepared": (C.c_int, [C.POINTER(GabRig), _P] + [_P] * 4 + [_P, _P, _P, _P, _P] + [_P] * 5 + [_P] * 6 + [_P] +
                                    [C.c_int32, C.POINTER(C.c_void_p), C.POINTER(C.c_int32), _P]),
+    "gab_mesh_counter_words": (C.c_int64, [C.POINTER(GabRig), C.c_int32]),
+    "gab_stream_is_capturing": (C.c_int, [_P]),
+    "gab_mesh_forward_prepared": (C.c_int, [C.POINTER(GabRig), _P] + [_P] * 6 + [_P, _P, _P] + [C.c_int32, _P, _P] + [_P] * 4 + [_P, _P]),
+    "gab_mesh_backward_fused": (C.c_int, [C.POINTER(GabRig), _P] + [_P] * 4 + [_P, _P, _P, C.c_int32, _P, _P] + [_P] * 5 + [_P] * 6 + [_P] +
+                                [C.c_int32, C.POINTER(C.c_void_p), C.POINTER(C.c_int32), _P, _P]),
     "gab_face_frames_forward": (C.c_int, [C.c_int32, C.c_int32, _P, _P, C.c_int32, _P, _P, _P, _P, _P, _P]),
     "gab_face_frames_backward": (C.c_int, [C.c_int32, C.c_int32, _P, _P, C.c_int32, _P, _P, _P, _P, _P, C.c_int32, _P]),
     "gab_bind_forward": (C.c_int, [C.c_int32, C.c_int32, _P, _P, _P, _P, C.c_int32, _P, _P, _P, _P, _P, _P, _P, _P, _P, _P]),
@@ -210,7 +215,7 @@
     "gab_profile_entry": (C.c_int, [C.c_int32, C.POINTER(C.c_char_p), C.POINTER(C.c_double), C.POINTER(C.c_int64)]),
     "gab_profile_reset": (C.c_int, []),
 }
-GAB_ABI_VERSION = 5
+GAB_ABI_VERSION = 6
 
 _gab = None
 
diff --git a/gaussianavatars_amd/binding.py b/gaussianavatars_amd/binding.py
--- a/gaussianavatars_amd/binding.py
+++ b/gaussianavatars_amd/binding.py
@@ -227,8 +227,19 @@
                 _chk(lib.gab_flame_forward_sequence(C.byref(rig), _p(ctx.prepared), seq.data_ptr() + 4 * t * 3 * V, *rows, _p(verts), _p(v_shaped),
                                                     _p(ws), _stream(dev)), "gab_flame_forward_sequence")
             elif ctx.prepared is not None:
-                _chk(lib.gab_flame_forward_prepared(C.byref(rig), _p(ctx.prepared), *rows, _p(verts), _p(v_shaped), _p(ws), _stream(dev)),
-                     "gab_flame_forward_prepared")
+                fr = getattr(ctx, "frames_request", None)
+                cnt = None if fr is None else mesh_counters(fr, rig, dev)
+                if cnt is not None:
+                    F = int(fr.shape[0])
+                    vf_begin, vf_list = vertex_corner_csr(fr, V)
+                    f32 = dict(dtype=torch.float32, device=dev)
+                    frames = (torch.empty((F, 3), **f32), torch.empty((F, 3, 3), **f32), torch.empty((F, 1), **f32), torch.empty((F, 4), **f32))
+                    _chk(lib.gab_mesh_forward_prepared(C.byref(rig), _p(ctx.prepared), *rows, _p(verts), _p(v_shaped), _p(ws), F, _p(vf_begin),
+                                                       _p(vf_list), *[_p(x) for x in frames], _p(cnt), _stream(dev)), "gab_mesh_forward_prepared")
+                    ctx.frames = frames
+                else:
+                    _chk(lib.gab_flame_forward_prepared(C.byref(rig), _p(ctx.prepared), *rows, _p(verts), _p(v_shaped), _p(ws), _stream(dev)),
+                         "gab_flame_forward_prepared")
             else:
                 _chk(lib.gab_flame_forward(C.byref(rig), _p(sh), *rows, _p(so), _p(verts), _p(v_shaped), _p(ws), _stream(dev)),
                      "gab_flame_forward")
@@ -345,6 +356,25 @@
     return vf_begin, vf_list
 
 
+def mesh_counters(faces: torch.Tensor, rig, dev):
+    if os.environ.get("GAA_MESH_FUSED", "1") == "0" or faces.shape[0] == 0 or faces.device != dev:
+        return None
+    lib = _lib.gab()
+    words = int(lib.gab_mesh_counter_words(C.byref(rig), int(faces.shape[0])))
+    stream = _stream(dev)
+    table = getattr(faces, "_gaa_mesh_counters", None)
+    if table is None:
+        table = faces._gaa_mesh_counters = {}
+    key = (int(stream or 0), words)
+    hit = table.get(key)
+    if hit is None:
+        if lib.gab_stream_is_capturing(stream) != 0:
+            return None
+        with torch.cuda.device(dev):
+            hit = table[key] = torch.zeros(words, dtype=torch.int32, device=dev)
+    return hit
+
+
 def _mesh_backward_mode() -> str:
     return os.environ.get("GAA_MESH_BWD", "merged")
 
@@ -355,6 +385,8 @@
         ctx.set_materialize_grads(False)
         need = ctx.needs_input_grad
         c1 = _SubCtx((False, False) + tuple(need[3:]))
+        if _mesh_backward_mode() == "merged" and faces.is_cuda and faces.is_contiguous() and faces.dtype in (torch.int32, torch.int64):
+            c1.frames_request = faces
         verts, v_shaped = _FlameForwardTimestep.forward(c1, head, t, shape, expr, rotation, neck, jaw, eyes, translation, static_offset)
         ctx.merged = c1.prepared is not None and _mesh_backward_mode() == "merged"
         if ctx.merged and faces.device != verts.device:
@@ -362,7 +394,13 @@
         if ctx.merged and any(need):
             ctx.corners = vertex_corner_csr(faces, int(verts.shape[1]))
         c2 = _SubCtx((any(need) and not ctx.merged, False))
-        center, R, scale, quat = _FaceFrames.forward(c2, verts[0], faces)
+        if getattr(c1, "frames", None) is not None:
+            center, R, scale, quat = c1.frames
+            fi, c2.is64 = _idx(faces)
+            c2.d_verts = None
+            c2.keep = _Keep(verts[0], fi)
+        else:
+            center, R, scale, quat = _FaceFrames.forward(c2, verts[0], faces)
         ctx.c1, ctx.c2 = c1, c2
         ctx.faces = faces
         return verts, v_shaped, center, R, scale, quat
@@ -386,9 +424,18 @@
         outp = [x.data_ptr() + 4 * t * w for x, w in zip(tables, widths)]
         rows = [x.data_ptr() + 4 * t * w for x, w in zip(tabs, widths)]
         vf_begin, vf_list = ctx.corners
-        scratch = torch.empty(3 * V, **f32)
         gs = [None if g is None else _f32(g) for g in (g_center, g_R, g_scale, g_quat)]
         gv = None if g_verts is None else _f32(g_verts)
+        with _lib.on_device(dev):
+            cnt = mesh_counters(ctx.faces, rig, dev)
+        if cnt is not None:
+            with _lib.on_device(dev):
+                _chk(lib.gab_mesh_backward_fused(C.byref(rig), _p(c1.prepared), *rows[1:5], _p(v_shaped), _p(ws), _p(v), int(ctx.faces.shape[0]),
+                                                 _p(vf_begin), _p(vf_list), _p(gs[0]), _p(gs[1]), _p(gs[2]), _p(gs[3]), _p(gv), *outp,
+                                                 None, len(tables), ptrs, sizes, _p(cnt), _stream(dev)), "gab_mesh_backward_fused")
+            grads = [tb if need[3 + i] else None for i, tb in enumerate(tables)]
+            return (None, None, None, None, *grads, None)
+        scratch = torch.empty(3 * V, **f32)
         with _lib.on_device(dev):
             _chk(lib.gab_mesh_backward_prepared(C.byref(rig), _p(c1.prepared), *rows[1:5], _p(v_shaped), _p(ws), _p(v),
                                                 _p(vf_begin), _p(vf_list), _p(gs[0]), _p(gs[1]), _p(gs[2]), _p(gs[3]), _p(gv), *outp,
diff --git a/gaussianavatars_amd/csrc/build_host.py b/gaussianavatars_amd/csrc/build_host.py
--- a/gaussianavatars_amd/csrc/build_host.py
+++ b/gaussianavatars_amd/csrc/build_host.py
@@ -8,7 +8,7 @@
 OUT = os.path.join(os.path.dirname(HERE), "gaa_host.so")
 SRC = os.path.join(HERE, "gaa_host.cpp")
 STAMP = OUT + ".stamp"
-DEPS = [SRC, __file__] + [os.path.join(HERE, "..", "..", "include", h) for h in ("gsr.h", "gab.h", "gls.h")]
+DEPS = [SRC, __file__] + [os.path.join(HERE, "..", "..", "include", h) for h in ("gsr.h", "gab.h", "gab_mesh.h", "gls.h")]
 
 
 def build_stamp() -> str:
diff --git a/gaussianavatars_amd/csrc/gaa_host.cpp b/gaussianavatars_amd/csrc/gaa_host.cpp
--- a/gaussianavatars_amd/csrc/gaa_host.cpp
+++ b/gaussianavatars_amd/csrc/gaa_host.cpp
@@ -25,7 +25,8 @@
     X(gsr_abi_version) X(gsr_last_error) X(gsr_geom_layout) X(gsr_binning_layout) X(gsr_image_layout) X(gsr_forward_bound)             \
     X(gsr_backward_bound) X(gsr_last_forward_seq) X(gsr_count_slot_wait) X(gsr_count_slot_overflow)                                     \
     X(gab_abi_version) X(gab_last_error) X(gab_flame_forward_prepared) X(gab_face_frames_forward) X(gab_mesh_backward_prepared)         \
-    X(gab_bind_backward_faces)                                                                                                           \
+    X(gab_bind_backward_faces) X(gab_mesh_forward_prepared) X(gab_mesh_backward_fused) X(gab_mesh_counter_words)                         \
+    X(gab_stream_is_capturing)                                                                                                           \
     X(gls_abi_version) X(gls_last_error) X(gls_partial_floats) X(gls_l1_forward) X(gls_l1_forward_grad) X(gls_l1_backward)               \
     X(gls_l1_ssim_forward) X(gls_l1_ssim_backward_split)
 
@@ -115,6 +116,20 @@
     int faces_i64 = 0;
     Tensor vf_begin, vf_list;
     int64_t F = 0;
+    bool one_launch = true;
+    std::mutex counter_mutex;
+    std::map<void*, Tensor> counters;
+    Tensor counters_for(void* stream)
+    {
+        if (!one_launch || F == 0) return Tensor();
+        std::lock_guard<std::mutex> lock(counter_mutex);
+        auto it = counters.find(stream);
+        if (it != counters.end()) return it->second;
+        if (api.gab_stream_is_capturing(stream) != 0) return Tensor();
+        Tensor c = at::zeros({api.gab_mesh_counter_words(&rig, (int32_t)F)}, prepared.options().dtype(at::kInt));
+        counters.emplace(stream, c);
+        return c;
+    }
 };
 
 struct MeshNode : public Node {
@@ -131,7 +146,7 @@
         need_api();
         TORCH_CHECK(grads.size() == 6, "MeshNode: expected 6 gradients");
         TORCH_CHECK(!grads[1].defined(), "the native mesh node has no path for a gradient w.r.t. verts_cano (v_shaped): take GAA_NATIVE_HOST=0");
-        const MeshPlan& p = *plan;
+        MeshPlan& p = *plan;
         static const char* names[6] = {"expr", "rotation", "neck_pose", "jaw_pose", "eyes_pose", "translation"};
         const Tensor& v = verts.get("verts");
         const Tensor& vs = v_shaped.get("verts_cano");
@@ -151,12 +166,21 @@
             outp[i] = zero_ptrs[i] + t * widths[i];
             rows[i] = tab.data_ptr<float>() + t * widths[i];
         }
-        Tensor scratch = empty_f32({3 * (int64_t)V}, v);
         Tensor gc = grad_f32(grads[2]), gR = grad_f32(grads[3]), gs = grad_f32(grads[4]), gq = grad_f32(grads[5]), gv = grad_f32(grads[0]);
-        int rc = api.gab_mesh_backward_prepared(&p.rig, p.prepared.data_ptr<float>(), rows[1], rows[2], rows[3], rows[4], vs.data_ptr<float>(), ws.data_ptr<float>(),
-                                                v.data_ptr<float>(), p.vf_begin.data_ptr<int32_t>(), p.vf_list.data_ptr<int32_t>(), fptr(gc), fptr(gR), fptr(gs), fptr(gq),
-                                                fptr(gv), outp[0], outp[1], outp[2], outp[3], outp[4], outp[5], scratch.data_ptr<float>(), 6, zero_ptrs, zero_sizes, stream);
-        TORCH_CHECK(rc == 0, "gab_mesh_backward_prepared failed (", rc, "): ", api.gab_last_error());
+        Tensor cnt = p.counters_for(stream);
+        if (cnt.defined()) {
+            int rc = api.gab_mesh_backward_fused(&p.rig, p.prepared.data_ptr<float>(), rows[1], rows[2], rows[3], rows[4], vs.data_ptr<float>(), ws.data_ptr<float>(),
+                                                 v.data_ptr<float>(), (int32_t)p.F, p.vf_begin.data_ptr<int32_t>(), p.vf_list.data_ptr<int32_t>(), fptr(gc), fptr(gR), fptr(gs),
+                                                 fptr(gq), fptr(gv), outp[0], outp[1], outp[2], outp[3], outp[4], outp[5], nullptr, 6, zero_ptrs, zero_sizes,
+                                                 cnt.data_ptr<int32_t>(), stream);
+            TORCH_CHECK(rc == 0, "gab_mesh_backward_fused failed (", rc, "): ", api.gab_last_error());
+        } else {
+            Tensor scratch = empty_f32({3 * (int64_t)V}, v);
+            int rc = api.gab_mesh_backward_prepared(&p.rig, p.prepared.data_ptr<float>(), rows[1], rows[2], rows[3], rows[4], vs.data_ptr<float>(), ws.data_ptr<float>(),
+                                                    v.data_ptr<float>(), p.vf_begin.data_ptr<int32_t>(), p.vf_list.data_ptr<int32_t>(), fptr(gc), fptr(gR), fptr(gs), fptr(gq),
+                                                    fptr(gv), outp[0], outp[1], outp[2], outp[3], outp[4], outp[5], scratch.data_ptr<float>(), 6, zero_ptrs, zero_sizes, stream);
+            TORCH_CHECK(rc == 0, "gab_mesh_backward_prepared failed (", rc, "): ", api.gab_last_error());
+        }
         variable_list out(6);
         for (int i = 0; i < 6; ++i)
             if (task_should_compute_output(i)) out[i] = tables[i];
@@ -169,7 +193,7 @@
                                 const Tensor& eyes, const Tensor& translation, int64_t t)
 {
     need_api();
-    const MeshPlan& p = *plan;
+    MeshPlan& p = *plan;
     const Tensor* tabs[6] = {&expr, &rotation, &neck, &jaw, &eyes, &translation};
     const int64_t widths[6] = {p.rig.n_expr, 3, 3, 3, 6, 3};
     static const char* names[6] = {"expr", "rotation", "neck_pose", "jaw_pose", "eyes_pose", "translation"};
@@ -188,12 +212,20 @@
     Tensor center = empty_f32({F, 3}, like), R = empty_f32({F, 3, 3}, like), scale = empty_f32({F, 1}, like), quat = empty_f32({F, 4}, like);
     const float* rows[6];
     for (int i = 0; i < 6; ++i) rows[i] = tabs[i]->data_ptr<float>() + t * widths[i];
-    int rc = api.gab_flame_forward_prepared(&p.rig, p.prepared.data_ptr<float>(), rows[0], rows[1], rows[2], rows[3], rows[4], rows[5], verts.data_ptr<float>(),
-                                            v_shaped.data_ptr<float>(), ws.data_ptr<float>(), stream);
-    TORCH_CHECK(rc == 0, "gab_flame_forward_prepared failed (", rc, "): ", api.gab_last_error());
-    rc = api.gab_face_frames_forward((int32_t)V, (int32_t)F, verts.data_ptr<float>(), p.faces.data_ptr(), p.faces_i64, center.data_ptr<float>(), R.data_ptr<float>(),
-                                     scale.data_ptr<float>(), quat.data_ptr<float>(), nullptr , stream);
-    TORCH_CHECK(rc == 0, "gab_face_frames_forward failed (", rc, "): ", api.gab_last_error());
+    Tensor cnt = p.counters_for(stream);
+    if (cnt.defined()) {
+        int rc = api.gab_mesh_forward_prepared(&p.rig, p.prepared.data_ptr<float>(), rows[0], rows[1], rows[2], rows[3], rows[4], rows[5], verts.data_ptr<float>(),
+                                               v_shaped.data_ptr<float>(), ws.data_ptr<float>(), (int32_t)F, p.vf_begin.data_ptr<int32_t>(), p.vf_list.data_ptr<int32_t>(),
+                                               center.data_ptr<float>(), R.data_ptr<float>(), scale.data_ptr<float>(), quat.data_ptr<float>(), cnt.data_ptr<int32_t>(), stream);
+        TORCH_CHECK(rc == 0, "gab_mesh_forward_prepared failed (", rc, "): ", api.gab_last_error());
+    } else {
+        int rc = api.gab_flame_forward_prepared(&p.rig, p.prepared.data_ptr<float>(), rows[0], rows[1], rows[2], rows[3], rows[4], rows[5], verts.data_ptr<float>(),
+                                                v_shaped.data_ptr<float>(), ws.data_ptr<float>(), stream);
+        TORCH_CHECK(rc == 0, "gab_flame_forward_prepared failed (", rc, "): ", api.gab_last_error());
+        rc = api.gab_face_frames_forward((int32_t)V, (int32_t)F, verts.data_ptr<float>(), p.faces.data_ptr(), p.faces_i64, center.data_ptr<float>(), R.data_ptr<float>(),
+                                         scale.data_ptr<float>(), quat.data_ptr<float>(), nullptr , stream);
+        TORCH_CHECK(rc == 0, "gab_face_frames_forward failed (", rc, "): ", api.gab_last_error());
+    }
     if (any_requires_grad({expr, rotation, neck, jaw, eyes, translation})) {
         auto node = std::shared_ptr<MeshNode>(new MeshNode(), torch::autograd::deleteNode);
         node->set_next_edges(torch::autograd::collect_next_edges(expr, rotation, neck, jaw, eyes, translation));
@@ -614,6 +646,8 @@
                     vf_list.numel() == 12 * p->F,
                 "vertex -> corner table does not match this topology");
     p->vf_begin = vf_begin, p->vf_list = vf_list;
+    const char* e = getenv("GAA_MESH_FUSED");
+    p->one_launch = !(e && e[0] == '0');
     return p;
 }
 
diff --git a/gaussianavatars_amd/csrc/gab_kernels.hip b/gaussianavatars_amd/csrc/gab_kernels.hip
--- a/gaussianavatars_amd/csrc/gab_kernels.hip
+++ b/gaussianavatars_amd/csrc/gab_kernels.hip
@@ -44,6 +44,9 @@
     v += dpp_f<0x143, 0xc>(v);
     return v;
 }
+
+__device__ __forceinline__ float ld_agent(const float* p) { return __hip_atomic_load(p, __ATOMIC_RELAXED, __HIP_MEMORY_SCOPE_AGENT); }
+__device__ __forceinline__ void st_agent(float* p, float x) { __hip_atomic_store(p, x, __ATOMIC_RELAXED, __HIP_MEMORY_SCOPE_AGENT); }
 
 __device__ __forceinline__ float beta_at(const float* shape, const float* expr, int n_shape, int l)
 {
@@ -304,16 +307,24 @@
     if (lane == 63) prepared[o < 15 ? jo + o : jo + 16 + (o - 15)] = acc;
 }
 
+struct FrameOut {
+    const int* vf_begin; const int4* vf_list;
+    int* cnt;
+    float* center; float* Rm; float* scaling; float* quat;
+};
+__device__ __forceinline__ void frames_on_arrival(const FrameOut& fo, int vbase, int vend, const float* verts);
+
 #ifndef GAB_FUSED_VERTS
 #define GAB_FUSED_VERTS 8
 #endif
-template <bool FLAME_TREE>
+template <int KIND>
 __global__ __launch_bounds__(256) void k_flame_fused(Rig rig, const float* __restrict__ prepared, const float* __restrict__ expr,
                                                       const float* __restrict__ rotation, const float* __restrict__ neck,
                                                       const float* __restrict__ jaw, const float* __restrict__ eyes,
                                                       const float* __restrict__ translation, float* __restrict__ verts,
-                                                      float* __restrict__ v_shaped, float* __restrict__ ws, const float* __restrict__ vs_pre)
-{
+                                                      float* __restrict__ v_shaped, float* __restrict__ ws, const float* __restrict__ vs_pre, FrameOut fo)
+{
+    constexpr bool FLAME_TREE = (KIND & 1) != 0, FRAMES = (KIND & 2) != 0;
     constexpr int VW = GAB_FUSED_VERTS, ROWS = 3 * VW, PER = ROWS / 8;
     __shared__ float out[WS_DA];
     __shared__ float vs[ROWS];
@@ -448,6 +459,10 @@
                 verts[3 * v + r] = T[4 * r] * vp[0] + T[4 * r + 1] * vp[1] + T[4 * r + 2] * vp[2] + T[4 * r + 3] + translation[r];
         }
     }
+    if constexpr (FRAMES) {
+        __syncthreads();
+        frames_on_arrival(fo, blockIdx.x * VW, min((int)blockIdx.x * VW + VW, rig.V), verts);
+    }
 }
 
 struct ZeroSpec { float* p[8]; int n[8]; int count; };
@@ -511,18 +526,20 @@
     }
 }
 
-template <bool FLAME_TREE, int NT>
+template <bool FLAME_TREE, int NT, bool LAST = false>
 __device__ __forceinline__ void chain_bwd_body(Rig rig, float* __restrict__ ws, const float* __restrict__ rotation, const float* __restrict__ neck,
                             const float* __restrict__ jaw, const float* __restrict__ eyes, float* __restrict__ d_rotation,
                             float* __restrict__ d_neck, float* __restrict__ d_jaw, float* __restrict__ d_eyes,
                             float* __restrict__ d_translation, float* __restrict__ d_expr, float* __restrict__ d_shape,
-                            const float* __restrict__ Mmat)
+                            const float* __restrict__ Mmat, float* expr_acc = nullptr)
 {
     __shared__ float sw[GAB_FLAME_WS_FLOATS];
     __shared__ float sdJ[16];
-    for (int kk = threadIdx.x; kk < GAB_FLAME_WS_FLOATS; kk += NT) sw[kk] = ws[kk];
+    for (int kk = threadIdx.x; kk < GAB_FLAME_WS_FLOATS; kk += NT) sw[kk] = LAST ? ld_agent(ws + kk) : ws[kk];
     __syncthreads();
-    for (int kk = WS_DA + (int)threadIdx.x; kk < WS_DJ; kk += NT) ws[kk] = 0.f;
+    for (int kk = WS_DA + (int)threadIdx.x; kk < WS_DJ; kk += NT) {
+        if (LAST) st_agent(ws + kk, 0.f); else ws[kk] = 0.f;
+    }
     if (!Mmat) {
         for (int kk = threadIdx.x; kk < rig.n_expr; kk += NT) d_expr[kk] = 0.f;
         if (d_shape)
@@ -604,7 +621,11 @@
             float a = 0.f;
 #pragma unroll
             for (int k = 0; k < 15; ++k) a += Mmat[(size_t)k * rig.n_expr + l] * sdJ[k];
-            unsafeAtomicAdd(&d_expr[l], a);
+            if (LAST) {
+                st_agent(&d_expr[l], ld_agent(&expr_acc[l]) + a);
+                st_agent(&expr_acc[l], 0.f);
+            } else
+                unsafeAtomicAdd(&d_expr[l], a);
         }
     const int j = threadIdx.x;
     if (j < GAB_NUM_JOINTS) {
@@ -615,9 +636,10 @@
 #pragma unroll
         for (int k = 0; k < 9; ++k) dRj[k] = sdR[9 * j + k];
         rodrigues_bwd(pose, dRj, dpose);
-        dj[0] = dpose[0]; dj[1] = dpose[1]; dj[2] = dpose[2];
+        if (LAST) { st_agent(dj, dpose[0]); st_agent(dj + 1, dpose[1]); st_agent(dj + 2, dpose[2]); }
+        else { dj[0] = dpose[0]; dj[1] = dpose[1]; dj[2] = dpose[2]; }
     } else if (j >= 8 && j < 11) {
-        d_translation[j - 8] = sw[WS_DT + j - 8];
+        if (LAST) st_agent(&d_translation[j - 8], sw[WS_DT + j - 8]); else d_translation[j - 8] = sw[WS_DT + j - 8];
     }
 }
 template <bool FLAME_TREE>
@@ -762,16 +784,9 @@
     return c;
 }
 
-__global__ __launch_bounds__(256) void k_face_frames(int F, const float* __restrict__ verts, const void* __restrict__ faces, int is64,
-                                                      float* __restrict__ center, float* __restrict__ Rm, float* __restrict__ scaling,
-                                                      float* __restrict__ quat, float* __restrict__ zero_fill, int zero_count)
-{
-    const int f = blockIdx.x * blockDim.x + threadIdx.x;
-    if (zero_fill)
-        for (int k = f; k < zero_count; k += (int)(gridDim.x * blockDim.x)) zero_fill[k] = 0.f;
-    if (f >= F) return;
-    const Vec3 v0 = ld3(verts, index_at(faces, is64, 3ll * f)), v1 = ld3(verts, index_at(faces, is64, 3ll * f + 1)),
-               v2 = ld3(verts, index_at(faces, is64, 3ll * f + 2));
+__device__ __forceinline__ void face_frame_store(int f, Vec3 v0, Vec3 v1, Vec3 v2, float* __restrict__ center, float* __restrict__ Rm,
+                                                 float* __restrict__ scaling, float* __restrict__ quat)
+{
     const Frame fr = make_frame(v0, v1, v2);
     const Vec3 c = (v0 + v1 + v2) * (1.f / 3.f);
     center[3 * f] = c.x; center[3 * f + 1] = c.y; center[3 * f + 2] = c.z;
@@ -785,6 +800,35 @@
     quat[4 * f + 1] = q[0] * inv;
     quat[4 * f + 2] = q[1] * inv;
     quat[4 * f + 3] = q[2] * inv;
+}
+
+__global__ __launch_bounds__(256) void k_face_frames(int F, const float* __restrict__ verts, const void* __restrict__ faces, int is64,
+                                                      float* __restrict__ center, float* __restrict__ Rm, float* __restrict__ scaling,
+                                                      float* __restrict__ quat, float* __restrict__ zero_fill, int zero_count)
+{
+    const int f = blockIdx.x * blockDim.x + threadIdx.x;
+    if (zero_fill)
+        for (int k = f; k < zero_count; k += (int)(gridDim.x * blockDim.x)) zero_fill[k] = 0.f;
+    if (f >= F) return;
+    const Vec3 v0 = ld3(verts, index_at(faces, is64, 3ll * f)), v1 = ld3(verts, index_at(faces, is64, 3ll * f + 1)),
+               v2 = ld3(verts, index_at(faces, is64, 3ll * f + 2));
+    face_frame_store(f, v0, v1, v2, center, Rm, scaling, quat);
+}
+
+__device__ __forceinline__ Vec3 ld3_agent(const float* p, long long i) { return {ld_agent(p + 3 * i), ld_agent(p + 3 * i + 1), ld_agent(p + 3 * i + 2)}; }
+
+__device__ __forceinline__ void frames_on_arrival(const FrameOut& fo, int vbase, int vend, const float* verts)
+{
+    const int p0 = fo.vf_begin[vbase], p1 = fo.vf_begin[vend];
+    for (int p = p0 + (int)threadIdx.x; p < p1; p += (int)blockDim.x) {
+        const int4 e = fo.vf_list[p];
+        const int f = e.x >> 2;
+        __threadfence();
+        if (atomicAdd(&fo.cnt[f], 1) != 2) continue;
+        __threadfence();
+        __hip_atomic_store(&fo.cnt[f], 0, __ATOMIC_RELAXED, __HIP_MEMORY_SCOPE_AGENT);
+        face_frame_store(f, ld3_agent(verts, e.y), ld3_agent(verts, e.z), ld3_agent(verts, e.w), fo.center, fo.Rm, fo.scaling, fo.quat);
+    }
 }
 
 __device__ __forceinline__ Vec3 unit_bwd(Vec3 g_unit, Vec3 unit, float len, bool clamped)
@@ -873,9 +917,18 @@
     const float* g_verts;
     float* g_vs;
 };
-__global__ __launch_bounds__(256) void k_gather_skin_bwd(Rig rig, GatherSkinArgs a, ZeroSpec zero)
-{
+struct ChainArgs {
+    const float* Mmat; const float* rotation; const float* neck; const float* jaw; const float* eyes;
+    float* d_rotation; float* d_neck; float* d_jaw; float* d_eyes; float* d_translation; float* d_expr;
+    int* ticket; float* acc;
+};
+#define GAB_FOLD_MAXR 12
+template <int KIND>
+__global__ __launch_bounds__(256) void k_gather_skin_bwd(Rig rig, GatherSkinArgs a, ZeroSpec zero, ChainArgs ch)
+{
+    constexpr bool FUSED = (KIND & 2) != 0;
     constexpr int VPB = GAB_MESH_VPB, ROWS = 3 * VPB;
+    static_assert(!FUSED || (ROWS + 7) / 8 <= GAB_FOLD_MAXR, "a thread's share of the expression block");
     static_assert(VPB == 16 || VPB == 32 || VPB == 64, "a wave holds the workgroup's vertices");
     __shared__ float gv[ROWS];
     __shared__ float red[100];
@@ -904,7 +957,24 @@
 #pragma unroll
         for (int j = 0; j < GAB_NUM_JOINTS; ++j) w[j] = rig.lbs_weights[(size_t)v * GAB_NUM_JOINTS + j];
     }
-    for (int k = tid; k < ROWS; k += 256) gv[k] = 0.f;
+    const int NB = rig.n_shape + rig.n_expr, nq = rig.n_expr >> 2;
+    const bool vec = FUSED && (rig.n_expr & 3) == 0 && (rig.n_shape & 3) == 0 && nq >= 1 && nq <= 32;
+    const int NG = vec ? min(256 / nq, 16) : 1, fg = vec ? tid / nq : 0, fq = vec ? tid - fg * nq : 0;
+    float4 bw[FUSED ? GAB_FOLD_MAXR : 1];
+    if constexpr (FUSED) {
+#pragma unroll
+        for (int i = 0; i < GAB_FOLD_MAXR; ++i) {
+            const int r = fg + NG * i;
+            bw[i] = (vec && fg < NG && r < ROWS && 3 * vbase + r < E)
+                        ? reinterpret_cast<const float4*>(rig.shapedirs + (size_t)(3 * vbase + r) * NB + rig.n_shape)[fq]
+                        : make_float4(0.f, 0.f, 0.f, 0.f);
+        }
+    }
+    __shared__ float gvs[FUSED ? ROWS : 1];
+    for (int k = tid; k < ROWS; k += 256) {
+        gv[k] = 0.f;
+        if (FUSED) gvs[k] = 0.f;
+    }
     __syncthreads();
     float tc[3] = {0.f, 0.f, 0.f};
     for (int p = p0 + tid; p < p1; p += 256) {
@@ -957,7 +1027,10 @@
         for (int c = 0; c < 3; ++c) gvp[c] = T[c] * g[0] + T[4 + c] * g[1] + T[8 + c] * g[2];
 #pragma unroll
         for (int p = 0; p < GAB_POSE_FEATURES; ++p) pf[p] = pd[p][3 * lane] * gvp[0] + pd[p][3 * lane + 1] * gvp[1] + pd[p][3 * lane + 2] * gvp[2];
-        if (wid == 0) { a.g_vs[3 * v] = gvp[0]; a.g_vs[3 * v + 1] = gvp[1]; a.g_vs[3 * v + 2] = gvp[2]; }
+        if (wid == 0) {
+            if (!FUSED || a.g_vs) { a.g_vs[3 * v] = gvp[0]; a.g_vs[3 * v + 1] = gvp[1]; a.g_vs[3 * v + 2] = gvp[2]; }
+            if (FUSED) { gvs[3 * lane] = gvp[0]; gvs[3 * lane + 1] = gvp[1]; gvs[3 * lane + 2] = gvp[2]; }
+        }
     }
     const float vph[4] = {vp[0], vp[1], vp[2], ok ? 1.f : 0.f};
 #pragma unroll
@@ -988,6 +1061,44 @@
     if (tid < 99) {
         float* dst = tid < 60 ? &a.ws[WS_DA + tid] : (tid < 63 ? &a.ws[WS_DT + tid - 60] : &a.ws[WS_DPF + tid - 63]);
         unsafeAtomicAdd(dst, red[tid]);
+    }
+    if constexpr (FUSED) {
+        __shared__ float part[16][128];
+        if (vec) {
+            float4 s4 = make_float4(0.f, 0.f, 0.f, 0.f);
+#pragma unroll
+            for (int i = 0; i < GAB_FOLD_MAXR; ++i) {
+                const int r = fg + NG * i;
+                const float gr = r < ROWS ? gvs[r] : 0.f;
+                s4.x += bw[i].x * gr; s4.y += bw[i].y * gr; s4.z += bw[i].z * gr; s4.w += bw[i].w * gr;
+            }
+            if (fg < NG) { part[fg][4 * fq] = s4.x; part[fg][4 * fq + 1] = s4.y; part[fg][4 * fq + 2] = s4.z; part[fg][4 * fq + 3] = s4.w; }
+            __syncthreads();
+            if (tid < rig.n_expr) {
+                float s = 0.f;
+                for (int g2 = 0; g2 < NG; ++g2) s += part[g2][tid];
+                unsafeAtomicAdd(&ch.acc[tid], s);
+            }
+        } else {
+            const int rows = min(ROWS, E - 3 * vbase);
+            for (int l = tid; l < rig.n_expr; l += 256) {
+                float s = 0.f;
+                for (int r = 0; r < rows; ++r) s += rig.shapedirs[(size_t)(3 * vbase + r) * NB + rig.n_shape + l] * gvs[r];
+                unsafeAtomicAdd(&ch.acc[l], s);
+            }
+        }
+        __shared__ int last;
+        __syncthreads();
+        if (tid == 0) {
+            __threadfence();
+            last = atomicAdd(ch.ticket, 1) == (int)gridDim.x - 1;
+        }
+        __syncthreads();
+        if (!last) return;
+        __threadfence();
+        if (tid == 0) __hip_atomic_store(ch.ticket, 0, __ATOMIC_RELAXED, __HIP_MEMORY_SCOPE_AGENT);
+        chain_bwd_body<(KIND & 1) != 0, 256, true>(rig, a.ws, ch.rotation, ch.neck, ch.jaw, ch.eyes, ch.d_rotation, ch.d_neck, ch.d_jaw, ch.d_eyes,
+                                                   ch.d_translation, ch.d_expr, nullptr, ch.Mmat, ch.acc);
     }
 }
 
@@ -1525,9 +1636,9 @@
     const int blocks = (rig.V + GAB_FUSED_VERTS - 1) / GAB_FUSED_VERTS;
     const bool flame_tree = rig.parents[1] == 0 && rig.parents[2] == 1 && rig.parents[3] == 1 && rig.parents[4] == 1;
     if (flame_tree)
-        PROF_LAUNCH(gab::k_flame_fused<true>, dim3(blocks), dim3(256), 0, st, rig, prepared, expr, rotation, neck, jaw, eyes, translation, verts, v_shaped, ws, (const float*)nullptr);
+        PROF_LAUNCH(gab::k_flame_fused<1>, dim3(blocks), dim3(256), 0, st, rig, prepared, expr, rotation, neck, jaw, eyes, translation, verts, v_shaped, ws, (const float*)nullptr, gab::FrameOut{});
     else
-        PROF_LAUNCH(gab::k_flame_fused<false>, dim3(blocks), dim3(256), 0, st, rig, prepared, expr, rotation, neck, jaw, eyes, translation, verts, v_shaped, ws, (const float*)nullptr);
+        PROF_LAUNCH(gab::k_flame_fused<0>, dim3(blocks), dim3(256), 0, st, rig, prepared, expr, rotation, neck, jaw, eyes, translation, verts, v_shaped, ws, (const float*)nullptr, gab::FrameOut{});
     LAUNCH_CHECK("k_flame_fused");
     return GAB_OK;
 }
@@ -1560,9 +1671,9 @@
     const int blocks = (rig.V + GAB_FUSED_VERTS - 1) / GAB_FUSED_VERTS;
     const bool flame_tree = rig.parents[1] == 0 && rig.parents[2] == 1 && rig.parents[3] == 1 && rig.parents[4] == 1;
     if (flame_tree)
-        PROF_LAUNCH(gab::k_flame_fused<true>, dim3(blocks), dim3(256), 0, st, rig, prepared, expr, rotation, neck, jaw, eyes, translation, verts, v_shaped, ws, v_shaped_row);
+        PROF_LAUNCH(gab::k_flame_fused<1>, dim3(blocks), dim3(256), 0, st, rig, prepared, expr, rotation, neck, jaw, eyes, translation, verts, v_shaped, ws, v_shaped_row, gab::FrameOut{});
     else
-        PROF_LAUNCH(gab::k_flame_fused<false>, dim3(blocks), dim3(256), 0, st, rig, prepared, expr, rotation, neck, jaw, eyes, translation, verts, v_shaped, ws, v_shaped_row);
+        PROF_LAUNCH(gab::k_flame_fused<0>, dim3(blocks), dim3(256), 0, st, rig, prepared, expr, rotation, neck, jaw, eyes, translation, verts, v_shaped, ws, v_shaped_row, gab::FrameOut{});
     LAUNCH_CHECK("k_flame_fused");
     return GAB_OK;
 }
@@ -1636,7 +1747,7 @@
     a.d_center = d_center; a.d_R = d_orien_mat; a.d_scaling = d_scaling; a.d_quat = d_orien_quat; a.g_verts = dL_dverts;
     a.g_vs = scratch;
     hipStream_t st = (hipStream_t)stream_;
-    PROF_LAUNCH(gab::k_gather_skin_bwd, dim3((rig.V + GAB_MESH_VPB - 1) / GAB_MESH_VPB), dim3(256), 0, st, rig, a, zs);
+    PROF_LAUNCH(gab::k_gather_skin_bwd<0>, dim3((rig.V + GAB_MESH_VPB - 1) / GAB_MESH_VPB), dim3(256), 0, st, rig, a, zs, gab::ChainArgs{});
     LAUNCH_CHECK("k_gather_skin_bwd");
     const int E = 3 * rig.V;
     const float* Mmat = prepared + gab::prep_joint_offset(rig.V) + 16;
@@ -1649,6 +1760,95 @@
         PROF_LAUNCH(gab::k_chain_blend_bwd<false>, dim3(blocks), dim3(256), 0, st, rig, ws, (const float*)scratch, Mmat, rotation, neck, jaw, eyes,
                            d_rotation, d_neck, d_jaw, d_eyes, d_translation, d_expr);
     LAUNCH_CHECK("k_chain_blend_bwd");
+    return GAB_OK;
+}
+
+int64_t gab_mesh_counter_words(const GabRig* rig_, int32_t F)
+{
+    if (!rig_ || rig_->n_expr < 0 || F < 0) return -1;
+    return (int64_t)F + 1 + rig_->n_expr;
+}
+
+int gab_stream_is_capturing(void* stream_)
+{
+    hipStreamCaptureStatus cs = hipStreamCaptureStatusNone;
+    if (hipStreamIsCapturing((hipStream_t)stream_, &cs) != hipSuccess) return fail(GAB_E_HIP, "hipStreamIsCapturing failed");
+    return cs != hipStreamCaptureStatusNone ? 1 : 0;
+}
+
+int gab_mesh_forward_prepared(const GabRig* rig_, const float* prepared, const float* expr, const float* rotation, const float* neck,
+                              const float* jaw, const float* eyes, const float* translation, float* verts, float* v_shaped, float* ws,
+                              int32_t F, const int32_t* vf_begin, const int32_t* vf_list, float* center, float* orien_mat, float* scaling,
+                              float* orien_quat, int32_t* counters, void* stream_)
+{
+    gab::Rig rig;
+    if (int rc = to_rig(rig_, &rig)) return rc;
+    if (F < 0) return fail(GAB_E_ARG, "bad sizes");
+    if (!prepared || (rig.n_expr && !expr) || !rotation || !neck || !jaw || !eyes || !translation || !verts || !v_shaped || !ws)
+        return fail(GAB_E_ARG, "gab_mesh_forward_prepared: NULL buffer");
+    if (F > 0 && (!vf_begin || !vf_list || !center || !orien_mat || !scaling || !orien_quat || !counters))
+        return fail(GAB_E_ARG, "gab_mesh_forward_prepared: NULL buffer");
+    if (((uintptr_t)vf_list) & 15) return fail(GAB_E_ARG, "gab_mesh_forward_prepared: vf_list must be 16-byte aligned");
+    hipStream_t st = (hipStream_t)stream_;
+    const int blocks = (rig.V + GAB_FUSED_VERTS - 1) / GAB_FUSED_VERTS;
+    const bool flame_tree = rig.parents[1] == 0 && rig.parents[2] == 1 && rig.parents[3] == 1 && rig.parents[4] == 1;
+    gab::FrameOut fo;
+    fo.vf_begin = vf_begin; fo.vf_list = reinterpret_cast<const int4*>(vf_list); fo.cnt = counters;
+    fo.center = center; fo.Rm = orien_mat; fo.scaling = scaling; fo.quat = orien_quat;
+    if (F == 0) {
+        if (flame_tree)
+            PROF_LAUNCH(gab::k_flame_fused<1>, dim3(blocks), dim3(256), 0, st, rig, prepared, expr, rotation, neck, jaw, eyes, translation, verts, v_shaped, ws, (const float*)nullptr, fo);
+        else
+            PROF_LAUNCH(gab::k_flame_fused<0>, dim3(blocks), dim3(256), 0, st, rig, prepared, expr, rotation, neck, jaw, eyes, translation, verts, v_shaped, ws, (const float*)nullptr, fo);
+    } else if (flame_tree)
+        PROF_LAUNCH(gab::k_flame_fused<3>, dim3(blocks), dim3(256), 0, st, rig, prepared, expr, rotation, neck, jaw, eyes, translation, verts, v_shaped, ws, (const float*)nullptr, fo);
+    else
+        PROF_LAUNCH(gab::k_flame_fused<2>, dim3(blocks), dim3(256), 0, st, rig, prepared, expr, rotation, neck, jaw, eyes, translation, verts, v_shaped, ws, (const float*)nullptr, fo);
+    LAUNCH_CHECK("k_flame_fused");
+    return GAB_OK;
+}
+
+int gab_mesh_backward_fused(const GabRig* rig_, const float* prepared, const float* rotation, const float* neck, const float* jaw,
+                            const float* eyes, const float* v_shaped, float* ws, const float* verts, int32_t F, const int32_t* vf_begin,
+                            const int32_t* vf_list, const float* d_center, const float* d_orien_mat, const float* d_scaling,
+                            const float* d_orien_quat, const float* dL_dverts, float* d_expr, float* d_rotation, float* d_neck,
+                            float* d_jaw, float* d_eyes, float* d_translation, float* g_vs, int32_t zero_count,
+                            float* const* zero_buffers_host, const int32_t* zero_sizes_host, int32_t* counters, void* stream_)
+{
+    if (zero_count < 0 || zero_count > 8 || (zero_count > 0 && (!zero_buffers_host || !zero_sizes_host)))
+        return fail(GAB_E_ARG, "gab_mesh_backward_fused: 0..8 zero-fill buffers");
+    gab::Rig rig;
+    if (int rc = to_rig(rig_, &rig)) return rc;
+    if (F < 0) return fail(GAB_E_ARG, "bad sizes");
+    if (!prepared || !rotation || !neck || !jaw || !eyes || !v_shaped || !ws || !verts || !vf_begin || !vf_list || !d_expr || !d_rotation ||
+        !d_neck || !d_jaw || !d_eyes || !d_translation || !counters)
+        return fail(GAB_E_ARG, "gab_mesh_backward_fused: NULL buffer");
+    if (((uintptr_t)vf_list) & 15) return fail(GAB_E_ARG, "gab_mesh_backward_fused: vf_list must be 16-byte aligned");
+    gab::ZeroSpec zs;
+    for (int i = 0; i < 8; ++i) {
+        zs.p[i] = i < zero_count ? zero_buffers_host[i] : nullptr;
+        zs.n[i] = i < zero_count ? zero_sizes_host[i] : 0;
+        if (i < zero_count && (zs.n[i] < 0 || (zs.n[i] > 0 && !zs.p[i]))) return fail(GAB_E_ARG, "gab_mesh_backward_fused: bad zero-fill buffer %d", i);
+    }
+    zs.count = zero_count;
+    gab::GatherSkinArgs a;
+    a.v_shaped = v_shaped; a.ws = ws; a.verts = verts;
+    a.vf_begin = vf_begin; a.vf_list = reinterpret_cast<const int4*>(vf_list);
+    a.d_center = d_center; a.d_R = d_orien_mat; a.d_scaling = d_scaling; a.d_quat = d_orien_quat; a.g_verts = dL_dverts;
+    a.g_vs = g_vs;
+    gab::ChainArgs ch;
+    ch.Mmat = prepared + gab::prep_joint_offset(rig.V) + 16;
+    ch.rotation = rotation; ch.neck = neck; ch.jaw = jaw; ch.eyes = eyes;
+    ch.d_rotation = d_rotation; ch.d_neck = d_neck; ch.d_jaw = d_jaw; ch.d_eyes = d_eyes; ch.d_translation = d_translation; ch.d_expr = d_expr;
+    ch.ticket = counters + F;
+    ch.acc = reinterpret_cast<float*>(counters + F + 1);
+    hipStream_t st = (hipStream_t)stream_;
+    const bool flame_tree = rig.parents[1] == 0 && rig.parents[2] == 1 && rig.parents[3] == 1 && rig.parents[4] == 1;
+    if (flame_tree)
+        PROF_LAUNCH(gab::k_gather_skin_bwd<3>, dim3((rig.V + GAB_MESH_VPB - 1) / GAB_MESH_VPB), dim3(256), 0, st, rig, a, zs, ch);
+    else
+        PROF_LAUNCH(gab::k_gather_skin_bwd<2>, dim3((rig.V + GAB_MESH_VPB - 1) / GAB_MESH_VPB), dim3(256), 0, st, rig, a, zs, ch);
+    LAUNCH_CHECK("k_gather_skin_bwd");
     return GAB_OK;
 }
 
diff --git a/include/gab.h b/include/gab.h
--- a/include/gab.h
+++ b/include/gab.h
@@ -8,7 +8,7 @@
 extern "C" {
 #endif
 
-#define GAB_ABI_VERSION 5
+#define GAB_ABI_VERSION 6
 #define GAB_OK 0
 #define GAB_E_ARG (-1)
 #define GAB_E_HIP (-2)
@@ -69,6 +69,8 @@
                                float* scratch, int32_t zero_count, float* const* zero_buffers_host, const int32_t* zero_sizes_host,
                                void* stream);
 
+#include "gab_mesh.h"
+
 int gab_face_frames_forward(int32_t V, int32_t F, const float* verts, const void* faces , int32_t index_is_i64,
                             float* center , float* orien_mat , float* scaling ,
                             float* orien_quat , float* d_verts_zeroed, void* stream);
diff --git a/include/gab_mesh.h b/include/gab_mesh.h
--- /dev/null
+++ b/include/gab_mesh.h
@@ -0,0 +1,23 @@
+#ifndef GAB_MESH_H
+#define GAB_MESH_H
+#ifndef GAB_H
+#error "include gab.h, which includes this header"
+#endif
+
+int64_t gab_mesh_counter_words(const GabRig* rig, int32_t F);
+int gab_stream_is_capturing(void* stream);
+int gab_mesh_forward_prepared(const GabRig* rig, const float* prepared, const float* expr, const float* rotation, const float* neck,
+                              const float* jaw, const float* eyes , const float* translation,
+                              float* verts , float* v_shaped , float* ws ,
+                              int32_t F, const int32_t* vf_begin, const int32_t* vf_list,
+                              float* center , float* orien_mat , float* scaling , float* orien_quat ,
+                              int32_t* counters, void* stream);
+int gab_mesh_backward_fused(const GabRig* rig, const float* prepared, const float* rotation, const float* neck, const float* jaw,
+                            const float* eyes, const float* v_shaped, float* ws, const float* verts , int32_t F,
+                            const int32_t* vf_begin, const int32_t* vf_list, const float* d_center, const float* d_orien_mat,
+                            const float* d_scaling, const float* d_orien_quat, const float* dL_dverts ,
+                            float* d_expr, float* d_rotation, float* d_neck, float* d_jaw, float* d_eyes, float* d_translation,
+                            float* g_vs , int32_t zero_count, float* const* zero_buffers_host,
+                            const int32_t* zero_sizes_host, int32_t* counters, void* stream);
+
+#endif
```

Result: slower. 3526 frames/s (-8.0%).
